# tbepler/topaz

Hardware: AMD Instinct MI355X
Metric: micrographs/sec (4096x4096 fp32) denoise+score, NMS parity (higher is better)
Workload: dtype f32 (convs: fp32 operands carried as two f16 halves on the f16 MFMA, three exact products per multiply-add accumulated in f32 -- fp32-level error, fp32-MFMA re-run on f16-range overflow; NMS in fp32; the exact-fp32-multiply rate is reported as exact_fp32)

## Files before the change

### topaz_amd/csrc/conv_split.h

```cpp
#pragma once
#include <hip/hip_runtime.h>
#include <stdint.h>
#include <vector>

#include "conv_mfma.h"
#include "split_fmt.h"

namespace tpz {

struct SplitArgs {
    const uint4* in;
    const uint4* in2;
    const uint4* wpk;
    const float* wscale;
    const float* bias;
    uint4* out;
    float* out_f32;
    const uint4* res;
    const float* post_scale;
    const float* post_shift;
    const float* head_w;
    float* head_out;
    const void* zeros;
    unsigned* flag;
    float head_b, slope;
    int cells_in, Hin, Win;
    int cells_in1, H1, W1;
    int Cout, cells_out, Hout, Wout;
    int pad_x, pad_y;
    int os, ooy, oox, Hfull, Wfull;
    int Hres, Wres, res_crop;
    int KZ, pad_z, Din, Dout, ooz, Dfull, Dres;
    int ncz;
    int nphase, phase_k, ws_phase_stride;
    size_t w_phase_bytes;
    int subpix_cout;
    int issuer_half;
    int n_chunks;
    int cog_inner;
    int tiles_x, tiles_y;
    int n_tiles;
    int vol_srcmajor;
    int xcd_swizzle;
    int wy0, wx0, wy1, wx1;
    int wz0, Dlat;
    int fold_cells, fold_tap, in2_H, in2_W, in2_oy, in2_ox;
    const struct SplitStep* plan;
};

struct SplitStep {
    uint16_t bofs[4];
    uint32_t dma;
    uint32_t cidx;
    uint32_t cell[4];
};
enum : uint32_t {
    SPLIT_DMA_ROUNDS = 0xffu,
    SPLIT_DMA_BUF = 1u << 8,
    SPLIT_DMA_NCELL_SHIFT = 9,
    SPLIT_DMA_SWITCH = 1u << 12,
    SPLIT_DMA_SRC2 = 1u << 13,
    SPLIT_DMA_NEXT = 1u << 14,
    SPLIT_DMA_ANY = 1u << 31,
};

struct SplitSlot {
    int ky, kx, c;
};

template <int K_, int D_, int MT_, int TH_, int TW_, int CC_, int WAVES_ = 8, int KX_ = K_, int SPS_ = 1>
struct SplitCfg {
    static constexpr int K = K_, KX = KX_, D = D_, MT = MT_, TH = TH_, TW = TW_, CC = CC_;
    static constexpr int WAVES = WAVES_, THREADS = 64 * WAVES_, WGS_PER_CU = WAVES_ == 8 ? 1 : 2;
    static constexpr bool UNIFORM_DMA = (MT_ >= 128 && WAVES_ == 8);
    static constexpr bool ISSUER_HALF = (MT_ >= 96 && WAVES_ == 8);
    static constexpr int MW = MT / 16;
    static constexpr int RPW = TH / WAVES;
    static constexpr int NFC = TW / 16;
    static constexpr int NW = RPW * NFC;
    static constexpr int ITH = TH + K - 1;
    static constexpr int ITW = (CC == 1) ? (TW + (KX - 1) * D + 15) / 16 * 16 : TW + (KX - 1) * D;
    static constexpr int CELL_STRIDE = (ITH * ITW + 15) / 16 * 16;
    static constexpr int NPC = CC * CELL_STRIDE;
    static constexpr int PLANE_BYTES = NPC * 16;
    static constexpr int IN_BUF = 2 * PLANE_BYTES;
    static constexpr int NR = (NPC + THREADS - 1) / THREADS;
    static constexpr bool ROWPAIR = (K == 5) && (KX == 5) && ((4 * D) % 16 == 0);
    static constexpr int PV = KX * (K / 2);
    static constexpr int PAIRS1 = PV + ((K % 2) ? (ROWPAIR ? KX - 1 : KX) : 0);
    static constexpr int NSTEP = (CC == 1) ? (PAIRS1 + 1) / 2 : (K * KX * CC + 3) / 4;
    static constexpr bool CONT = (CC % 2 == 0);
    static constexpr int Q = K * KX * CC;
    static constexpr int TAPS = K * KX;
    __host__ __device__ static constexpr int cont_slots(int cells) { return TAPS * cells; }
    __host__ __device__ static constexpr int cont_stages(int cells) { return (TAPS * cells + 3) / 4; }
    __host__ __device__ static constexpr SplitSlot cont_slot(int q) { return SplitSlot{(q / CC) / KX, (q / CC) % KX, q % CC}; }
    __host__ __device__ static constexpr SplitSlot slot(int step, int kb) {
        if (CC != 1) {
            const int q = step * 4 + kb, t = q / CC;
            return t < K * KX ? SplitSlot{t / KX, t % KX, q % CC} : SplitSlot{-1, 0, 0};
        }
        const int p = step * 2 + (kb >> 1), j = kb & 1;
        if (p < PV) return SplitSlot{2 * (p % (K / 2)) + j, p / (K / 2), 0};
        const int e = p - PV;
        if (K % 2 == 0) return SplitSlot{-1, 0, 0};
        if (ROWPAIR) {
            if (e == 0) return SplitSlot{K - 1, j ? 4 : 0, 0};
            return (e < KX - 1 && j == 0) ? SplitSlot{K - 1, e, 0} : SplitSlot{-1, 0, 0};
        }
        return (e < KX && j == 0) ? SplitSlot{K - 1, e, 0} : SplitSlot{-1, 0, 0};
    }
    __host__ __device__ static constexpr int slot_lds_off(int step, int kb) {
        SplitSlot s = slot(step, kb);
        if (s.ky < 0) s = slot(step, kb & ~1);
        if (s.ky < 0) return 0;
        return (s.c * CELL_STRIDE + s.ky * ITW + s.kx * D) * 16;
    }
    static constexpr int W_STEP_BYTES = 2 * MW * 1024;
    static constexpr int SPS = SPS_;
    static constexpr int W_STAGE_BYTES = SPS * W_STEP_BYTES;
    static constexpr int WR = (W_STAGE_BYTES + THREADS * 16 - 1) / (THREADS * 16);
    static constexpr int OFF_W = 2 * IN_BUF;
    static constexpr int OFF_TAB = OFF_W + 2 * W_STAGE_BYTES;
    static constexpr int LDS_BYTES = OFF_TAB + (NPC * 4 + 15) / 16 * 16;
    static_assert(NR <= 8, "the plan carries the DMA rounds of a step as a byte mask");
    static_assert(TH % WAVES == 0 && TW % 16 == 0 && MT % 16 == 0, "tile shape");
    static_assert(PLANE_BYTES + (RPW * ITW + TW) * 16 < 65536, "ds_read immediates are 16 bit");
    static_assert(LDS_BYTES <= 160 * 1024 / WGS_PER_CU, "LDS per workgroup");
    static_assert(WAVES == 8 || WAVES == 4, "waves per workgroup");
    static_assert(SPS == 1 || (CONT && Q >= 8 * SPS), "multi-step stages: continuous slot stream, chunks of >= 2 * SPS steps");
};

struct SplitPlanKey {
    int cells_in, cells_in1, n_chunks, has_in2, vol, KZ, fold_cells, fold_tap, srcmajor;
};

template <class C>
void split_make_plan(const SplitPlanKey& k, std::vector<SplitStep>& out) {
    const bool vol = k.vol != 0;
    const bool folded = C::CONT && C::SPS == 1 && k.fold_cells > 0;
    const int vcells = (folded ? k.cells_in1 : k.cells_in) * (vol ? k.KZ : 1);
    const int n_full = vcells / C::CC, n_rem = vcells - n_full * C::CC;
    const int n_stages_a = C::CONT ? C::cont_stages(vcells) : k.n_chunks * C::NSTEP;
    const int n_stages = n_stages_a + (folded ? k.fold_cells / C::CC : 0);
    const int chunks1 = (k.has_in2 && !vol) ? k.cells_in1 / C::CC : k.n_chunks;
    auto cont_off = [](int q) {
        const SplitSlot sl = C::cont_slot(q);
        return (sl.c * C::CELL_STRIDE + sl.ky * C::ITW + sl.kx * C::D) * 16;
    };
    auto fetch = [&](SplitStep& e, int pf, unsigned rmask, bool sw) {
        e.dma = SPLIT_DMA_ANY | (rmask & SPLIT_DMA_ROUNDS) | ((pf & 1) ? SPLIT_DMA_BUF : 0u) | (sw ? SPLIT_DMA_SWITCH : 0u);
        if (!vol) {
            const bool second = pf >= chunks1;
            if (second) e.dma |= SPLIT_DMA_SRC2;
            e.cidx = (uint32_t)(second ? pf - chunks1 : pf);
            const int have = k.cells_in - pf * C::CC;
            if (have < C::CC) e.dma |= (uint32_t)(have > 1 ? have : 1) << SPLIT_DMA_NCELL_SHIFT;
        } else {
            bool any2 = false, any1 = false;
            for (int j = 0; j < C::CC && j < 4; ++j) {
                const int v = pf * C::CC + j;
                int kz, c;
                if (!k.srcmajor) {
                    kz = v / k.cells_in; c = v - kz * k.cells_in;
                } else if (v < k.KZ * k.cells_in1) {
                    kz = v / k.cells_in1; c = v - kz * k.cells_in1;
                } else {
                    const int vv = v - k.KZ * k.cells_in1, c2n = k.cells_in - k.cells_in1;
                    kz = vv / c2n; c = k.cells_in1 + (vv - kz * c2n);
                }
                if (kz >= k.KZ) { e.cell[j] = 0; continue; }
                const bool l2 = c >= k.cells_in1;
                (l2 ? any2 : any1) = true;
                e.cell[j] = 1u | (l2 ? 2u : 0u) | (uint32_t)kz << 2 | (uint32_t)(l2 ? c - k.cells_in1 : c) << 8;
            }
            if (k.srcmajor && any2 && !any1) e.dma |= SPLIT_DMA_SRC2;
        }
    };
    out.assign((size_t)n_stages + 1, SplitStep{});
    fetch(out[0], 0, (1u << C::NR) - 1, false);
    unsigned next_rounds = 0;
    for (int s = 0; s < n_stages; ++s) {
        SplitStep& e = out[(size_t)s + 1];
        for (int l4 = 0; l4 < 4; ++l4) {
            int off;
            if (C::CONT) {
                if (folded && s >= n_stages_a) {
                    off = ((chunks1 + s - n_stages_a) & 1) * C::IN_BUF + cont_off(k.fold_tap * C::CC + l4);
                } else {
                    int G = 4 * s + l4, cg = G / C::Q, q = G - cg * C::Q;
                    if (cg >= n_full) {
                        const int q2 = G - n_full * C::Q;
                        cg = n_full < k.n_chunks ? n_full : k.n_chunks - 1;
                        q = (n_rem > 0 && q2 < C::TAPS * n_rem) ? (q2 / n_rem) * C::CC + (q2 % n_rem) : 0;
                    }
                    off = (cg & 1) * C::IN_BUF + cont_off(q);
                }
            } else {
                const int ch = s / C::NSTEP;
                off = (ch & 1) * C::IN_BUF + C::slot_lds_off(s - ch * C::NSTEP, l4);
            }
            e.bofs[l4] = (uint16_t)(off / 16);
        }
        const int stage = s / C::SPS;
        if (s % C::SPS != 0) continue;
        int pf, r0, rstride;
        if (C::CONT) {
            const int ch = (4 * s) / C::Q;
            pf = ch + 1;
            const int ws = pf >= 2 ? (C::Q * (pf - 1) - 1) / 4 + 1 : 0;
            const int we = (C::Q * pf) / 4 - 1;
            const int gs = (ws + C::SPS - 1) / C::SPS, ge = (we + 1) / C::SPS - 1;
            r0 = (stage >= gs && stage <= ge) ? stage - gs : C::NR;
            rstride = ge - gs + 1;
            if (folded && s >= n_stages_a) {
                pf = chunks1 + (s - n_stages_a) + 1;
                r0 = 0;
                rstride = 1;
            }
        } else {
            const int ch = s / C::NSTEP;
            pf = ch + 1;
            r0 = s - ch * C::NSTEP;
            rstride = C::NSTEP;
        }
        if (pf < k.n_chunks) {
            if (r0 >= C::NR) continue;
            unsigned rmask = 0;
            for (int r = r0; r < C::NR; r += rstride) rmask |= 1u << r;
            fetch(e, pf, rmask, r0 == 0 && pf == chunks1);
        } else if (pf == k.n_chunks && !folded && !vol && !k.has_in2) {
            if (C::CONT) {
                const int ws = pf >= 2 ? (C::Q * (pf - 1) - 1) / 4 + 1 : 0;
                const int we = n_stages - 1;
                const int gs = (ws + C::SPS - 1) / C::SPS, ge = (we + 1) / C::SPS - 1;
                if (stage < gs || stage > ge) continue;
                r0 = stage - gs;
                rstride = ge - gs + 1;
            }
            if (r0 >= C::NR) continue;
            unsigned rmask = 0;
            for (int r = r0; r < C::NR; r += rstride) rmask |= 1u << r;
            fetch(e, 0, rmask, r0 == 0);
            e.dma |= SPLIT_DMA_NEXT;
            if (k.n_chunks & 1) e.dma |= SPLIT_DMA_BUF;
            next_rounds |= rmask;
        }
    }
    if (next_rounds == (1u << C::NR) - 1u) out[0].dma |= SPLIT_DMA_NEXT;
    const size_t n = out.size();
    out.resize(2 * n);
    for (size_t i = 0; i < n; ++i) {
        SplitStep e = out[i];
        for (int l4 = 0; l4 < 4; ++l4) {
            const int off = e.bofs[l4] * 16;
            e.bofs[l4] = (uint16_t)((off >= C::IN_BUF ? off - C::IN_BUF : off + C::IN_BUF) / 16);
        }
        if (e.dma & SPLIT_DMA_ANY) e.dma ^= SPLIT_DMA_BUF;
        out[n + i] = e;
    }
}

enum { EPI_PLAIN_F32 = 5, EPI_POOL = 6 };
template <class C, int EPI, int ABL, int MODE>
__device__ __forceinline__ void conv_split_body(const SplitArgs& a, const unsigned bid_x, const unsigned bid_y, const unsigned bid_z,
                                                const unsigned grid_x, const unsigned grid_y) {
    constexpr int D = C::D, MW = C::MW, NW = C::NW, NFC = C::NFC;
    constexpr bool HAS2 = (MODE & 1) != 0, VOLM = (MODE & 2) != 0;
    constexpr bool UNI2 = (MODE & 8) != 0;
    static_assert(!UNI2 || (HAS2 && VOLM), "MODE 11 = two sources, plane-stacked, chunk-uniform");
    constexpr bool PERSIST = (MODE & 4) != 0;
    static_assert(!PERSIST || (MODE == 4 && EPI != EPI_HEAD), "persistent tiles: plain single-source layers");
    const uint4* const in2 = HAS2 ? a.in2 : nullptr;
    const int fold_cells = HAS2 ? a.fold_cells : 0;
    extern __shared__ __attribute__((aligned(16))) unsigned char lds[];
    unsigned* lds_tab = reinterpret_cast<unsigned*>(lds + C::OFF_TAB);

    const int tid = threadIdx.x;
    unsigned long long probe_c0 = 0, probe_r0 = 0, probe_pro = 0, probe_loop = 0;
    unsigned long long seg[4] = {0, 0, 0, 0}, seg_t = 0;
    auto seg_mark = [&](int i) {
        if constexpr ((ABL & 4096) != 0) {
            const unsigned long long t = __builtin_readcyclecounter();
            if (i >= 0) seg[i] += t - seg_t;
            seg_t = t;
        }
    };
    if constexpr ((ABL & 2048) != 0) {
        probe_c0 = __builtin_readcyclecounter();
        probe_r0 = __builtin_amdgcn_s_memrealtime();
    }
    const int lane = tid & 63;
    const int wave = __builtin_amdgcn_readfirstlane(tid >> 6);
    const int l15 = lane & 15, l4 = lane >> 4;

    int y0, x0, cogz, oz, pad_x, pad_y, pad_z, oox, ooy, ooz, phase, ybase, xbase;
    auto set_tile = [&](int bx, int by, int bz) {
        y0 = a.wy0 + (by / D) * (C::TH * D) + (by % D);
        x0 = a.wx0 + bx * C::TW;
        cogz = bz % a.ncz;
        oz = bz / a.ncz;
        pad_x = a.pad_x; pad_y = a.pad_y; pad_z = a.pad_z; oox = a.oox; ooy = a.ooy; ooz = a.ooz; phase = 0;
        if (a.nphase > 0) {
            phase = oz % a.nphase;
            oz /= a.nphase;
            oox = phase & 1; ooy = (phase >> 1) & 1; ooz = (phase >> 2) & 1;
            pad_x = (a.phase_k / 2 - oox + 1) / 2;
            pad_y = (a.phase_k / 2 - ooy + 1) / 2;
            pad_z = (a.phase_k / 2 - ooz + 1) / 2;
        }
        oz += a.wz0;
        ybase = y0 - pad_y; xbase = x0 - pad_x;
    };
    auto set_tile_linear = [&](unsigned L) {
        const unsigned txy = (unsigned)(a.tiles_x * a.tiles_y);
        const unsigned bz = L / txy, rem = L - bz * txy, by = rem / (unsigned)a.tiles_x;
        set_tile((int)(rem - by * (unsigned)a.tiles_x), (int)by, (int)bz);
    };
    unsigned tile_L = 0, tile_end = 0, tile_stride = 1;
    if constexpr (PERSIST) {
        const unsigned nt = (unsigned)a.n_tiles;
        const unsigned xcd = bid_x & 7u, j = bid_x >> 3, q = nt / 8, r = nt % 8;
        const unsigned start = xcd < r ? xcd * (q + 1) : r * (q + 1) + (xcd - r) * q;
        tile_end = start + q + (xcd < r ? 1u : 0u);
        tile_stride = grid_x >> 3;
        tile_L = start + j;
        if (tile_L >= tile_end) return;
        set_tile_linear(tile_L);
    } else {
        int bx = (int)bid_x, by = (int)bid_y;
        if (a.xcd_swizzle) {
            const unsigned nwg = grid_x * grid_y, orig = bid_x + grid_x * bid_y;
            const unsigned q = nwg / 8, r = nwg % 8, xcd = orig % 8;
            const unsigned wgid = (xcd < r ? xcd * (q + 1) : r * (q + 1) + (xcd - r) * q) + orig / 8;
            if (a.xcd_swizzle == 2) {
                const unsigned blk = wgid >> 5, in = wgid & 31u, nbx = grid_x >> 3;
                const unsigned byb = blk / nbx, tr = byb * 4 + (in >> 3), bands = (unsigned)a.tiles_y / (unsigned)D;
                bx = (int)((blk - byb * nbx) * 8 + (in & 7u));
                if (bx >= a.tiles_x || tr >= (unsigned)a.tiles_y) return;
                const unsigned ph = tr / bands;
                by = (int)((tr - ph * bands) * (unsigned)D + ph);
            } else {
                bx = (int)(wgid % grid_x);
                by = (int)(wgid / grid_x);
            }
        }
        set_tile(bx, by, (int)bid_z);
    }
    const bool vol = VOLM && (a.KZ > 1 || a.Din > 1);

    constexpr unsigned OOB = 0xfffffff0u;
    constexpr bool BUFDMA = (ABL & 65536) == 0;
    const bool ups = (a.H1 != a.Hin) || (a.W1 != a.Win);
    auto compute_offsets = [&](bool second, int tid, int H1, int W1, int Hup, int Wup, int ybase, int xbase) {
        const bool fold2 = second && fold_cells > 0;
        const int Hs = fold2 ? a.in2_H : second ? a.Hin : H1, Ws = fold2 ? a.in2_W : second ? a.Win : W1;
        const int Hv = fold2 ? a.in2_H : a.Hin, Wv = fold2 ? a.in2_W : a.Win;
#pragma unroll 1
        for (int i = 0; i < C::NR; ++i) {
            const int g = i * C::THREADS + tid;
            if (g < C::NPC) {
                const int c = g / C::CELL_STRIDE;
                const int rem = g - c * C::CELL_STRIDE;
                const int r = rem / C::ITW, x = rem - r * C::ITW;
                const int gy = ybase + r * D + (fold2 ? a.in2_oy : 0), gx = xbase + x + (fold2 ? a.in2_ox : 0);
                unsigned off = OOB;
                if ((unsigned)gy < (unsigned)Hv && (unsigned)gx < (unsigned)Wv) {
                    int sy = gy, sx = gx;
                    if (!second && ups) { sy = nearest_src(gy, H1, Hup); sx = nearest_src(gx, W1, Wup); }
                    off = vol ? (unsigned)(((size_t)sy * Ws + sx) * 16) : (unsigned)((((size_t)c * Hs + sy) * Ws + sx) * 16);
                }
                lds_tab[g] = off;
            }
        }
    };
    const size_t plane1 = (size_t)a.cells_in1 * a.H1 * a.W1 * (vol ? a.Din : 1);
    const size_t hw2 = fold_cells > 0 ? (size_t)a.in2_H * a.in2_W : (size_t)a.Hin * a.Win;
    const size_t plane2 = (size_t)(a.cells_in - a.cells_in1) * hw2 * (vol ? a.Din : 1);
    const unsigned lds_base = (unsigned)(size_t)(lptr_t)lds;
    const void* zsrc = uniform_ptr(a.zeros);
    typedef uint32_t StepW __attribute__((ext_vector_type(8)));
    typedef const __attribute__((address_space(4))) StepW* plan_ptr_t;
    const plan_ptr_t plan0 = (plan_ptr_t)a.plan;

    auto glds16 = [&](const void* src, unsigned lds_addr) {
        __builtin_amdgcn_global_load_lds((__attribute__((address_space(1))) const void*)src,
                                         (__attribute__((address_space(3))) void*)(size_t)lds_addr, 16, 0, 0);
    };
    auto make_srd = [&](const void* base, size_t bytes) {
        return __builtin_amdgcn_make_buffer_rsrc(const_cast<void*>(uniform_ptr(base)), 0,
                                                 (int)__builtin_amdgcn_readfirstlane((unsigned)bytes), 0x00020000);
    };
    auto bdma16 = [&](__amdgpu_buffer_rsrc_t srd, unsigned voff, unsigned soff, unsigned lds_addr) {
        __builtin_amdgcn_raw_ptr_buffer_load_lds(srd, (__attribute__((address_space(3))) void*)(size_t)lds_addr, 16, voff, soff, 0, 0);
    };
    auto fetch = [&](const StepW& P, unsigned rounds, int tid, int wave) {
        const unsigned d = P[2];
        const int buf = (d & SPLIT_DMA_BUF) ? 1 : 0;
        const bool second = HAS2 && (d & SPLIT_DMA_SRC2) != 0;
        const unsigned ncell = (d >> SPLIT_DMA_NCELL_SHIFT) & 7u;
        const uint4* chunk = second ? in2 + (size_t)P[3] * (C::CC * hw2) : a.in + (size_t)P[3] * (C::CC * (size_t)a.H1 * a.W1);
        const unsigned char* bhi = reinterpret_cast<const unsigned char*>(uniform_ptr(vol ? ((UNI2 && second) ? in2 : a.in) : chunk));
        const size_t lo_delta0 = ((second && (!vol || UNI2)) ? plane2 : plane1) * 16;
        const size_t ext = vol ? ((UNI2 && second) ? plane2 : plane1) * 16 : (second ? (size_t)C::CC * hw2 : (size_t)C::CC * a.H1 * a.W1) * 16;
        const __amdgpu_buffer_rsrc_t srd_hi = make_srd(bhi, ext), srd_lo = make_srd(bhi + lo_delta0, ext);
        constexpr int CCV = C::CC < 4 ? C::CC : 4;
        unsigned coff[CCV], cflag[CCV];
        if (vol) {
#pragma unroll
            for (int j = 0; j < CCV; ++j) {
                const unsigned cv = P[4 + j];
                const int iz = oz + (int)((cv >> 2) & 63u) * D - pad_z;
                const bool ok = (cv & 1u) && (unsigned)iz < (unsigned)a.Din;
                coff[j] = (unsigned)((((size_t)(cv >> 8) * a.Din + iz) * a.Hin) * a.Win * 16);
                cflag[j] = (ok ? 1u : 0u) | ((HAS2 && !UNI2) ? (cv & 2u) : 0u);
            }
        }
#pragma unroll
        for (int r = 0; r < C::NR; ++r) {
            if (!((rounds >> r) & 1u)) continue;
            const int g = r * C::THREADS + tid;
            if ((r + 1) * C::THREADS <= C::NPC || g < C::NPC) {
                unsigned off = lds_tab[g];
                size_t lo_delta = lo_delta0;
                bool lane2 = false;
                if (!vol) {
                    if (ncell != 0 && g >= (int)ncell * C::CELL_STRIDE) off = OOB;
                } else {
                    unsigned co = coff[0], cf = cflag[0];
#pragma unroll
                    for (int j = 1; j < CCV; ++j)
                        if (g >= j * C::CELL_STRIDE) { co = coff[j]; cf = cflag[j]; }
                    if (!(cf & 1u)) off = OOB;
                    else if (off != OOB) { off += co; lane2 = HAS2 && !UNI2 && (cf & 2u) != 0; }
                }
                const unsigned dst = __builtin_amdgcn_readfirstlane(lds_base + (unsigned)(buf * C::IN_BUF + (r * C::THREADS + wave * 64) * 16));
                if constexpr (BUFDMA) {
                    if (VOLM && HAS2 && !UNI2 && __any(lane2)) {
                        if (lane2) {
                            const __amdgpu_buffer_rsrc_t s2h = make_srd(in2, plane2 * 16), s2l = make_srd(in2 + plane2, plane2 * 16);
                            bdma16(s2h, off, 0, dst);
                            bdma16(s2l, off, 0, dst + C::PLANE_BYTES);
                        } else {
                            bdma16(srd_hi, off, 0, dst);
                            bdma16(srd_lo, off, 0, dst + C::PLANE_BYTES);
                        }
                    } else {
                        bdma16(srd_hi, off, 0, dst);
                        bdma16(srd_lo, off, 0, dst + C::PLANE_BYTES);
                    }
                } else if constexpr (C::UNIFORM_DMA) {
                    const void* blo = bhi + lo_delta;
                    if (!__any(off == OOB || lane2)) {
                        glds_b128(off, bhi, dst);
                        glds_b128(off, blo, dst + C::PLANE_BYTES);
                    } else {
                        if (off == OOB) {
                            glds_b128(0u, zsrc, dst);
                            glds_b128(0u, zsrc, dst + C::PLANE_BYTES);
                        } else if (lane2) {
                            const void* b2 = uniform_ptr(in2);
                            const void* b2lo = uniform_ptr(in2 + plane2);
                            glds_b128(off, b2, dst);
                            glds_b128(off, b2lo, dst + C::PLANE_BYTES);
                        } else {
                            glds_b128(off, bhi, dst);
                            glds_b128(off, blo, dst + C::PLANE_BYTES);
                        }
                    }
                } else {
                    const unsigned char* src = bhi;
                    if (lane2) { src = reinterpret_cast<const unsigned char*>(in2); lo_delta = plane2 * 16; }
                    const bool oob = off == OOB;
                    const unsigned char* shi = oob ? reinterpret_cast<const unsigned char*>(zsrc) : src + off;
                    const unsigned char* slo = oob ? reinterpret_cast<const unsigned char*>(zsrc) : src + off + lo_delta;
                    glds16(shi, dst);
                    glds16(slo, dst + C::PLANE_BYTES);
                }
            }
        }
    };
    auto issue_weights = [&](const unsigned char* wcog, int stg, int bytes, int buf, int tid, int wave) {
        const unsigned char* base = reinterpret_cast<const unsigned char*>(uniform_ptr(wcog + (size_t)stg * C::W_STAGE_BYTES));
        const unsigned dst = __builtin_amdgcn_readfirstlane(lds_base + (unsigned)(C::OFF_W + buf * C::W_STAGE_BYTES + wave * 1024));
        if constexpr (BUFDMA) {
            const __amdgpu_buffer_rsrc_t srd = make_srd(base, (size_t)bytes);
#pragma unroll
            for (int i = 0; i < C::WR; ++i)
                if ((i * C::WAVES + wave) * 1024 < bytes) bdma16(srd, (unsigned)tid * 16u, (unsigned)(i * C::THREADS * 16), dst + i * C::THREADS * 16);
            return;
        }
#pragma unroll
        for (int i = 0; i < C::WR; ++i)
            if ((i * C::WAVES + wave) * 1024 < bytes) {
                if constexpr (C::UNIFORM_DMA) glds_b128((unsigned)(i * C::THREADS + tid) * 16u, base, dst + i * C::THREADS * 16);
                else glds16(base + (unsigned)(i * C::THREADS + tid) * 16u, dst + i * C::THREADS * 16);
            }
    };

    const unsigned b_lane = (unsigned)(((wave * C::RPW) * C::ITW + l15) * 16);
    const unsigned a_lane = (unsigned)(C::OFF_W + lane * 16);
    auto b_frag_base = [&](const StepW& P, int l4) -> const unsigned char* {
        const unsigned w = (l4 & 2) ? P[1] : P[0];
        return lds + b_lane + (((w >> ((l4 & 1) * 16)) & 0xffffu) << 4);
    };

    float hsum[NW];
#pragma unroll
    for (int n = 0; n < NW; ++n) hsum[n] = 0.f;
    bool big = false;

    const bool folded = C::CONT && C::SPS == 1 && fold_cells > 0;
    const int vcells = (folded ? a.cells_in1 : a.cells_in) * (vol ? a.KZ : 1);
    const int n_stages_a = C::CONT ? C::cont_stages(vcells) : a.n_chunks * C::NSTEP;
    const int n_stages = n_stages_a + (folded ? fold_cells / C::CC : 0);
    const size_t w_cog_bytes = (size_t)n_stages * C::W_STEP_BYTES;

    const int n_wstages = (n_stages + C::SPS - 1) / C::SPS;
    int par_in = 0, par_w = 0;
    bool prefetched = false;
    auto wcog_of = [&](int phase, int cog) {
        return reinterpret_cast<const unsigned char*>(a.wpk) + (size_t)phase * a.w_phase_bytes + (size_t)cog * w_cog_bytes;
    };
    for (;;) {
    const bool has_next = PERSIST && tile_L + tile_stride < tile_end;
    int n_ybase = 0, n_xbase = 0, n_phase = 0, n_cog = 0;
    if (PERSIST && has_next) {
        const int sy0 = y0, sx0 = x0, scogz = cogz, soz = oz, spx = pad_x, spy = pad_y, spz = pad_z, sox = oox, soy = ooy,
                  soz2 = ooz, sph = phase, syb = ybase, sxb = xbase;
        set_tile_linear(tile_L + tile_stride);
        n_ybase = ybase; n_xbase = xbase; n_phase = phase; n_cog = cogz;
        y0 = sy0; x0 = sx0; cogz = scogz; oz = soz; pad_x = spx; pad_y = spy; pad_z = spz; oox = sox; ooy = soy; ooz = soz2;
        phase = sph; ybase = syb; xbase = sxb;
    }
    const plan_ptr_t plan = plan0 + (PERSIST && par_in ? n_stages + 1 : 0);
    for (int cg = 0; cg < a.cog_inner; ++cg) {
        const int cog = cogz * a.cog_inner + cg;
        const unsigned char* wcog = wcog_of(phase, cog);
        const float* wscale = a.wscale + (size_t)phase * a.ws_phase_stride;
        f32x4 acc[MW][NW];
#pragma unroll
        for (int m = 0; m < MW; ++m)
#pragma unroll
            for (int n = 0; n < NW; ++n) acc[m][n] = (f32x4){0.f, 0.f, 0.f, 0.f};

        unsigned long long probe_t0 = 0;
        if constexpr ((ABL & 2048) != 0) probe_t0 = (cg == 0 && !prefetched) ? probe_c0 : __builtin_readcyclecounter();
        __syncthreads();
        int tid_p = tid, H1_p = a.H1, W1_p = a.W1, Hup_p = a.Hin, Wup_p = a.Win;
        asm volatile("" : "+v"(tid_p), "+s"(H1_p), "+s"(W1_p), "+s"(Hup_p), "+s"(Wup_p));
        const int wave_p = __builtin_amdgcn_readfirstlane(tid_p >> 6), l4_p = (tid_p & 63) >> 4;
        StepW P = plan[1];
        if (!(PERSIST && prefetched)) {
            const StepW P0 = plan0[0];
            compute_offsets((P0[2] & SPLIT_DMA_SRC2) != 0, tid_p, H1_p, W1_p, Hup_p, Wup_p, ybase, xbase);
            fetch(P0, (1u << C::NR) - 1u, tid_p, wave_p);
            issue_weights(wcog, 0, (n_stages < C::SPS ? n_stages : C::SPS) * C::W_STEP_BYTES, 0, tid_p, wave_p);
            asm volatile("s_waitcnt vmcnt(0)" ::: "memory");
            __syncthreads();
        }

        f16x8 bh[NW], bo[NW], ah[2], ao[2];
        auto b_off = [&](int n) { return ((n / NFC) * C::ITW + (n % NFC) * 16) * 16; };
        {
            const unsigned char* bl = b_frag_base(P, l4_p);
#pragma unroll
            for (int n = 0; n < NW; ++n) {
                bh[n] = *reinterpret_cast<const f16x8*>(bl + b_off(n));
                bo[n] = *reinterpret_cast<const f16x8*>(bl + b_off(n) + C::PLANE_BYTES);
            }
            const unsigned a_lane_p = (unsigned)(C::OFF_W + (tid_p & 63) * 16 + (PERSIST ? par_w * C::W_STAGE_BYTES : 0));
            ah[0] = *reinterpret_cast<const f16x8*>(lds + a_lane_p);
            ao[0] = *reinterpret_cast<const f16x8*>(lds + a_lane_p + MW * 1024);
        }

        unsigned long long probe_t1 = 0;
        if constexpr ((ABL & 2048) != 0) probe_t1 = __builtin_readcyclecounter();
        if constexpr ((ABL & 524288) != 0) { if (C::WAVES == 8 && wave >= 4) __builtin_amdgcn_s_setprio(1); }
        if constexpr ((ABL & 1048576) != 0) { if (C::WAVES == 8 && wave < 4) __builtin_amdgcn_s_setprio(1); }
#pragma unroll 1
        for (int s = 0; s < n_stages; ++s) {
            const int stage = s / C::SPS, sub = s - stage * C::SPS;
            const bool stage_end = sub == C::SPS - 1 || s == n_stages - 1;
            const StepW Pn = plan[1 + (s + 1 < n_stages ? s + 1 : s)];
            auto step_dma = [&]() {
            if (!(ABL & 2) && sub == 0) {
                const bool iss = C::ISSUER_HALF && a.issuer_half && (!in2 || folded);
                const int reps = iss ? (wave >= 4 ? 2 : 0) : 1;
                if constexpr (!(ABL & 128)) {
                    for (int rep = 0; rep < reps; ++rep) {
                        const int vw = iss ? wave - 4 * (1 - rep) : wave, vt = iss ? tid - 256 * (1 - rep) : tid;
                        const int left = n_stages - (stage + 1) * C::SPS;
                        const int wb = PERSIST ? (stage + 1 + par_w) & 1 : (stage + 1) & 1;
                        if (left > 0) issue_weights(wcog, stage + 1, (left < C::SPS ? left : C::SPS) * C::W_STEP_BYTES, wb, vt, vw);
                        else if (PERSIST && has_next)
                            issue_weights(wcog_of(n_phase, n_cog), 0, (n_stages < C::SPS ? n_stages : C::SPS) * C::W_STEP_BYTES, wb, vt, vw);
                    }
                }
                const bool next_fetch = (P[2] & SPLIT_DMA_NEXT) != 0;
                if (!(ABL & 256) && (P[2] & SPLIT_DMA_ANY) && (!next_fetch || (PERSIST && has_next))) {
                    if (HAS2 && (P[2] & SPLIT_DMA_SWITCH)) {
                        compute_offsets(true, tid, a.H1, a.W1, a.Hin, a.Win, ybase, xbase);
                        if (iss) __syncthreads();
                    }
                    if (PERSIST && next_fetch && (P[2] & SPLIT_DMA_SWITCH)) {
                        compute_offsets(false, tid, a.H1, a.W1, a.Hin, a.Win, n_ybase, n_xbase);
                        if (iss) __syncthreads();
                    }
                    for (int rep = 0; rep < reps; ++rep) {
                        const int vw = iss ? wave - 4 * (1 - rep) : wave, vt = iss ? tid - 256 * (1 - rep) : tid;
                        fetch(P, P[2] & SPLIT_DMA_ROUNDS, vt, vw);
                    }
                }
            }
            };
            seg_mark(s == 0 ? -1 : 3);
            step_dma();
            seg_mark(0);
            constexpr bool MFMA_FIRST = (ABL & 131072) == 0;
            const int wpar = PERSIST ? par_w : 0;
            const unsigned char* al = lds + a_lane + ((stage + wpar) & 1) * C::W_STAGE_BYTES + sub * C::W_STEP_BYTES;
            const int stage_n = (s + 1) / C::SPS;
            const unsigned char* al_next = lds + a_lane + ((stage_n + wpar) & 1) * C::W_STAGE_BYTES + (s + 1 - stage_n * C::SPS) * C::W_STEP_BYTES;
            const unsigned char* bl_next = nullptr;
            constexpr bool A0_EARLY = (MW % 2 == 0);
#pragma unroll
            for (int m = 0; m < MW; ++m) {
                const int t = m & 1;
                if (m + 1 < MW) {
                    if constexpr (!(ABL & 8)) {
                        ah[t ^ 1] = *reinterpret_cast<const f16x8*>(al + (m + 1) * 1024);
                        ao[t ^ 1] = *reinterpret_cast<const f16x8*>(al + (MW + m + 1) * 1024);
                    } else {
                        ah[t ^ 1] = ah[t];
                        ao[t ^ 1] = ao[t];
                    }
                } else {
                    if constexpr (!(ABL & 16) && !(ABL & 8)) {
#pragma unroll
                        for (int mm = 0; mm + 1 < MW; ++mm) {
                            if (mm == 0 && MFMA_FIRST) {
                                __builtin_amdgcn_sched_group_barrier(0x008, NW, 0);
                                __builtin_amdgcn_sched_group_barrier(0x100, 2, 0);
                                __builtin_amdgcn_sched_group_barrier(0x008, 2 * NW, 0);
                            } else {
                                __builtin_amdgcn_sched_group_barrier(0x100, 2, 0);
                                __builtin_amdgcn_sched_group_barrier(0x008, 3 * NW, 0);
                            }
                        }
                    }
                    __builtin_amdgcn_sched_barrier(0);
                    seg_mark(1);
                    if (C::SPS == 1 || stage_end) {
                        if constexpr (!(ABL & 16384))
                            asm volatile("s_waitcnt vmcnt(0)" ::: "memory");
                        if constexpr (!(ABL & 4)) __syncthreads();
                    }
                    seg_mark(2);
                    bl_next = b_frag_base(Pn, l4);
                    __builtin_amdgcn_sched_barrier(0);
                }
                const bool last = m + 1 == MW;
                f16x8 a_hi = ah[t], a_lo = ao[t];
                if (last && A0_EARLY) {
                    ah[0] = *reinterpret_cast<const f16x8*>(al_next);
                    ao[0] = *reinterpret_cast<const f16x8*>(al_next + MW * 1024);
                }
                if constexpr (!(ABL & 16)) {
#pragma unroll
                    for (int n = 0; n < NW; ++n)
                        acc[m][n] = __builtin_amdgcn_mfma_f32_16x16x32_f16(a_hi, bo[n], acc[m][n], 0, 0, 0);
                    if (last) {
#pragma unroll
                        for (int n = 0; n < NW; ++n) bo[n] = *reinterpret_cast<const f16x8*>(bl_next + b_off(n) + C::PLANE_BYTES);
                    }
#pragma unroll
                    for (int n = 0; n < NW; ++n)
                        acc[m][n] = __builtin_amdgcn_mfma_f32_16x16x32_f16(a_hi, bh[n], acc[m][n], 0, 0, 0);
#pragma unroll
                    for (int n = 0; n < NW; ++n)
                        acc[m][n] = __builtin_amdgcn_mfma_f32_16x16x32_f16(a_lo, bh[n], acc[m][n], 0, 0, 0);
                } else {
#pragma unroll
                    for (int n = 0; n < NW; ++n) acc[m][n][0] += (float)a_hi[0] * (float)bh[n][0] + (float)a_lo[1] * (float)bo[n][1];
                    if (last) {
#pragma unroll
                        for (int n = 0; n < NW; ++n) bo[n] = *reinterpret_cast<const f16x8*>(bl_next + b_off(n) + C::PLANE_BYTES);
                    }
                }
                if (last) {
#pragma unroll
                    for (int n = 0; n < NW; ++n) bh[n] = *reinterpret_cast<const f16x8*>(bl_next + b_off(n));
                    if (!A0_EARLY) {
                        ah[0] = *reinterpret_cast<const f16x8*>(al_next);
                        ao[0] = *reinterpret_cast<const f16x8*>(al_next + MW * 1024);
                    }
                    if constexpr (!(ABL & 16) && !(ABL & 8)) {
                        if (A0_EARLY) __builtin_amdgcn_sched_group_barrier(0x100, 2, 1);
                        __builtin_amdgcn_sched_group_barrier(0x008, NW, 1);
                        __builtin_amdgcn_sched_group_barrier(0x100, NW, 1);
                        __builtin_amdgcn_sched_group_barrier(0x008, 2 * NW, 1);
                        __builtin_amdgcn_sched_group_barrier(0x100, A0_EARLY ? NW : NW + 2, 1);
                    }
                    __builtin_amdgcn_sched_barrier(0);
                }
            }
            P = Pn;
        }
        if constexpr ((ABL & 2048) != 0) {
            probe_loop += __builtin_readcyclecounter() - probe_t1;
            probe_pro += probe_t1 - probe_t0;
        }

        if constexpr ((ABL & (524288 | 1048576)) != 0) __builtin_amdgcn_s_setprio(0);
        int tid_e = threadIdx.x;
        asm volatile("" : "+v"(tid_e));
        const int l15 = tid_e & 15, l4 = (tid_e >> 4) & 3;
        const int wave = __builtin_amdgcn_readfirstlane(tid_e >> 6);
        const int fz = oz * a.os + ooz;
        const size_t cplane_out = (size_t)a.Dfull * a.Hfull * a.Wfull, cplane_res = (size_t)a.Dres * a.Hres * a.Wres;
        const size_t plane_out = (size_t)a.cells_out * cplane_out;
        const size_t plane_res = (size_t)a.cells_out * cplane_res;
        const size_t zoff_out = (size_t)fz * a.Hfull * a.Wfull;
        const size_t zoff_res = (size_t)(fz + (a.Dres > 1 ? a.res_crop : 0)) * a.Hres * a.Wres;
        const bool has_bias = a.bias != nullptr;
        unsigned opix[NW], rpix[NW], ovo[NW], rvo[NW];
        bool okv[NW];
        if constexpr (EPI != EPI_HEAD) {
#pragma unroll
            for (int n = 0; n < NW; ++n) {
                const int oy = y0 + (wave * C::RPW + n / NFC) * D;
                const int ox = x0 + (n % NFC) * 16 + l15;
                okv[n] = oy < a.wy1 && ox < a.wx1;
                if constexpr ((ABL & 1) != 0 || (ABL & 64) != 0) okv[n] = okv[n] && (a.slope == 12345.f);
                const int cy = oy < a.Hout ? oy : a.Hout - 1, cx = ox < a.Wout ? ox : a.Wout - 1;
                const int fy = cy * a.os + ooy, fx = cx * a.os + oox;
                if constexpr (EPI == EPI_POOL) opix[n] = (unsigned)((cy >> 1) * a.Wfull + (cx >> 1));
                else opix[n] = (unsigned)(fy * a.Wfull + fx);
                rpix[n] = (unsigned)((fy + a.res_crop) * a.Wres + fx + a.res_crop);
                if constexpr (EPI == EPI_POOL) {
                    okv[n] = (l15 & 1) == 0 && oy < a.wy1 && ox < a.wx1 && oy + 1 < a.Hout && ox + 1 < a.Wout;
                }
                const unsigned lane_o = (unsigned)(l4 >> 1) * (unsigned)(cplane_out * 16) + (unsigned)(l4 & 1) * 8u;
                const unsigned lane_r = (unsigned)(l4 >> 1) * (unsigned)(cplane_res * 16) + (unsigned)(l4 & 1) * 8u;
                ovo[n] = okv[n] ? opix[n] * 16u + lane_o : OOB;
                rvo[n] = rpix[n] * 16u + lane_r;
            }
        }
        const unsigned cp16_o = (unsigned)(cplane_out * 16), cp16_r = (unsigned)(cplane_res * 16);
        constexpr bool WIDE = (NW % 2 == 0) && EPI != EPI_HEAD && EPI != EPI_PLAIN_F32 && EPI != EPI_POOL && (ABL & 262144) == 0;
        constexpr int NP = WIDE ? NW / 2 : 1;
        unsigned ovw[NP], rvw[NP];
        if constexpr (WIDE) {
            const int odd = l4 & 1;
#pragma unroll
            for (int q = 0; q < NP; ++q) {
                const int fr = odd ? (2 * q + 1) / NFC : (2 * q) / NFC, fc = odd ? (2 * q + 1) % NFC : (2 * q) % NFC;
                const int oy = y0 + (wave * C::RPW + fr) * D;
                const int ox = x0 + fc * 16 + l15;
                bool ok = oy < a.wy1 && ox < a.wx1;
                if constexpr ((ABL & 1) != 0 || (ABL & 64) != 0) ok = ok && (a.slope == 12345.f);
                const int cy = oy < a.Hout ? oy : a.Hout - 1, cx = ox < a.Wout ? ox : a.Wout - 1;
                const int fy = cy * a.os + ooy, fx = cx * a.os + oox;
                const unsigned po = (unsigned)(fy * a.Wfull + fx), pr = (unsigned)((fy + a.res_crop) * a.Wres + fx + a.res_crop);
                ovw[q] = ok ? po * 16u + (unsigned)(l4 >> 1) * (unsigned)(cplane_out * 16) : OOB;
                rvw[q] = pr * 16u + (unsigned)(l4 >> 1) * (unsigned)(cplane_res * 16);
            }
        }
        const unsigned zo16 = (unsigned)(zoff_out * 16), zr16 = (unsigned)(zoff_res * 16);
        const size_t pl16_o = plane_out * 16, pl16_r = plane_res * 16;
        const unsigned char* const out8 = reinterpret_cast<const unsigned char*>(a.out);
        const unsigned char* const res8 = reinterpret_cast<const unsigned char*>(a.res);
        const float slope = a.slope;
        u16x2 bigacc = {0, 0};
        unsigned okmask[NW];
#pragma unroll
        for (int n = 0; n < NW; ++n) okmask[n] = (EPI != EPI_HEAD && okv[n]) ? 0x7fff7fffu : 0u;
        struct Frag { int cb, sy, sx, cell0, ncell; bool ok; };
        auto frag_of = [&](int m) {
            Frag f;
            const int covb = cog * C::MT + m * 16;
            f.cb = covb; f.sy = 0; f.sx = 0; f.ok = true;
            if (a.subpix_cout > 0) {
                const int par = covb / a.subpix_cout;
                f.cb = covb - par * a.subpix_cout;
                f.sx = par & 1; f.sy = (par >> 1) & 1;
                f.ok = par <= 3;
            }
            f.cell0 = f.cb >> 3;
            const int nc = f.ok ? a.cells_out - f.cell0 : 0;
            f.ncell = nc < 0 ? 0 : nc > 2 ? 2 : nc;
            return f;
        };
        constexpr bool RESID = (EPI == EPI_RES || EPI == EPI_RES_POST) && !(ABL & 1) && !(ABL & 32);
        u32x2 rhb[2][NW], rlb[2][NW];
        auto load_res = [&](int m, u32x2 (&rh)[NW], u32x2 (&rl)[NW]) {
            const Frag f = frag_of(m);
            const unsigned ex16 = zr16 + (unsigned)(f.sy * a.Wres + f.sx) * 16u;
            const unsigned nrec = f.ncell > 0 ? (unsigned)f.ncell * cp16_r - ex16 : 0u;
            const unsigned char* rb8 = res8 + ((size_t)((unsigned)f.cell0 * (unsigned long long)cp16_r) + ex16);
            const __amdgpu_buffer_rsrc_t srd_rh = make_srd(rb8, nrec);
            const __amdgpu_buffer_rsrc_t srd_rl = make_srd(rb8 + pl16_r, nrec);
            if constexpr (WIDE) {
#pragma unroll
                for (int q = 0; q < NP; ++q) {
                    const u32x4 ch = __builtin_amdgcn_raw_buffer_load_b128(srd_rh, (int)rvw[q], 0, 0);
                    const u32x4 cl = __builtin_amdgcn_raw_buffer_load_b128(srd_rl, (int)rvw[q], 0, 0);
                    rh[2 * q] = (u32x2){ch[0], ch[1]}; rh[2 * q + 1] = (u32x2){ch[2], ch[3]};
                    rl[2 * q] = (u32x2){cl[0], cl[1]}; rl[2 * q + 1] = (u32x2){cl[2], cl[3]};
                }
            } else {
#pragma unroll
                for (int n = 0; n < NW; ++n) {
                    rh[n] = __builtin_amdgcn_raw_buffer_load_b64(srd_rh, (int)rvo[n], 0, 0);
                    rl[n] = __builtin_amdgcn_raw_buffer_load_b64(srd_rl, (int)rvo[n], 0, 0);
                }
            }
        };
        auto unswap_res = [&](u32x2 (&r)[NW], int q) {
            const auto s0 = __builtin_amdgcn_permlane16_swap(r[2 * q].x, r[2 * q + 1].x, false, false);
            const auto s1 = __builtin_amdgcn_permlane16_swap(r[2 * q].y, r[2 * q + 1].y, false, false);
            r[2 * q] = (u32x2){s0[0], s1[0]};
            r[2 * q + 1] = (u32x2){s0[1], s1[1]};
        };
        if constexpr (RESID) load_res(0, rhb[0], rlb[0]);
#pragma unroll
        for (int m = 0; m < MW; ++m) {
            const Frag f = frag_of(m);
            const int cov0 = cog * C::MT + m * 16 + l4 * 4;
            const int sy = f.sy, sx = f.sx, cell0 = f.cell0, ncell = f.ncell;
            const int co0 = f.ok ? f.cb + l4 * 4 : a.Cout;
            if constexpr (RESID) { if (m + 1 < MW) load_res(m + 1, rhb[(m + 1) & 1], rlb[(m + 1) & 1]); }
            u32x2 (&rh)[NW] = rhb[m & 1];
            u32x2 (&rl)[NW] = rlb[m & 1];
            f32x2 sc[2], bi[2], psc[2], psh[2], hw[2];
            {
                const float4 s4 = *reinterpret_cast<const float4*>(wscale + cov0);
                sc[0] = (f32x2){s4.x, s4.y}; sc[1] = (f32x2){s4.z, s4.w};
                float4 b4 = make_float4(0.f, 0.f, 0.f, 0.f);
                if (has_bias) b4 = *reinterpret_cast<const float4*>(a.bias + co0);
                bi[0] = (f32x2){b4.x, b4.y}; bi[1] = (f32x2){b4.z, b4.w};
                if constexpr (EPI == EPI_RES_POST) {
                    const float4 p4 = *reinterpret_cast<const float4*>(a.post_scale + co0);
                    const float4 q4 = *reinterpret_cast<const float4*>(a.post_shift + co0);
                    psc[0] = (f32x2){p4.x, p4.y}; psc[1] = (f32x2){p4.z, p4.w};
                    psh[0] = (f32x2){q4.x, q4.y}; psh[1] = (f32x2){q4.z, q4.w};
                }
                if constexpr (EPI == EPI_HEAD) {
                    const float4 h4 = *reinterpret_cast<const float4*>(a.head_w + co0);
                    hw[0] = (f32x2){h4.x, h4.y}; hw[1] = (f32x2){h4.z, h4.w};
                }
            }
            const f32x2 slope2 = {slope, slope};
            __amdgpu_buffer_rsrc_t srd_oh, srd_ol;
            if constexpr (EPI != EPI_HEAD && EPI != EPI_PLAIN_F32) {
                const unsigned ex16 = zo16 + (unsigned)(sy * a.Wfull + sx) * 16u;
                const unsigned nrec = ncell > 0 ? (unsigned)ncell * cp16_o - ex16 : 0u;
                const unsigned char* ob8 = out8 + ((size_t)((unsigned)cell0 * (unsigned long long)cp16_o) + ex16);
                srd_oh = make_srd(ob8, nrec);
                srd_ol = make_srd(ob8 + pl16_o, nrec);
            }
            if constexpr (EPI == EPI_POOL) {
                static_assert(EPI != EPI_POOL || (C::RPW % 2 == 0 && C::D == 1), "pooling pairs tile rows inside a wave");
#pragma unroll
                for (int n = 0; n < NW; ++n) {
                    if ((n / NFC) % 2 != 0) continue;
                    f32x2 v[2];
#pragma unroll
                    for (int h = 0; h < 2; ++h) {
                        f32x2 t0 = (f32x2){acc[m][n][2 * h], acc[m][n][2 * h + 1]} * sc[h] + bi[h];
                        f32x2 t1 = (f32x2){acc[m][n + NFC][2 * h], acc[m][n + NFC][2 * h + 1]} * sc[h] + bi[h];
                        t0 = __builtin_elementwise_max(t0, t0 * slope2);
                        t1 = __builtin_elementwise_max(t1, t1 * slope2);
                        const f32x2 t = __builtin_elementwise_max(t0, t1);
                        v[h] = __builtin_elementwise_max(t, (f32x2){__shfl_xor(t[0], 1, 64), __shfl_xor(t[1], 1, 64)});
                    }
                    unsigned h0, l0, h1, l1;
                    split2m(v[0], h0, l0);
                    split2m(v[1], h1, l1);
                    const u32x2 hi = {h0, h1}, lo = {l0, l1};
                    bigacc = __builtin_elementwise_max(bigacc, __builtin_bit_cast(u16x2, h0 & okmask[n]));
                    bigacc = __builtin_elementwise_max(bigacc, __builtin_bit_cast(u16x2, h1 & okmask[n]));
                    __builtin_amdgcn_raw_buffer_store_b64(hi, srd_oh, (int)ovo[n], 0, 0);
                    __builtin_amdgcn_raw_buffer_store_b64(lo, srd_ol, (int)ovo[n], 0, 0);
                }
                continue;
            }
            unsigned keep_h[2] = {0u, 0u}, keep_l[2] = {0u, 0u};
#pragma unroll
            for (int n = 0; n < NW; ++n) {
                if constexpr (WIDE && RESID) {
                    if ((n & 1) == 0) { unswap_res(rh, n >> 1); unswap_res(rl, n >> 1); }
                }
                f32x2 v[2];
#pragma unroll
                for (int h = 0; h < 2; ++h) {
                    f32x2 addend = bi[h];
                    if constexpr (RESID)
                        addend = add_halves(add_halves(addend, h ? rl[n].y : rl[n].x), h ? rh[n].y : rh[n].x);
                    v[h] = (f32x2){acc[m][n][2 * h], acc[m][n][2 * h + 1]} * sc[h] + addend;
                    if constexpr (EPI == EPI_RES_POST) v[h] = v[h] * psc[h] + psh[h];
                    v[h] = __builtin_elementwise_max(v[h], v[h] * slope2);
                    if constexpr (EPI == EPI_HEAD) v[h] *= hw[h];
                }
                if constexpr (EPI == EPI_HEAD) {
                    const f32x2 t = v[0] + v[1];
                    hsum[n] += t[0] + t[1];
                } else if constexpr (EPI == EPI_PLAIN_F32) {
                    const size_t cs = cplane_out;
                    float* const fb = a.out_f32 + ((size_t)co0 * cplane_out + zoff_out + (unsigned)(sy * a.Wfull + sx)) + opix[n];
#pragma unroll
                    for (int r = 0; r < 4; ++r)
                        if (okv[n] && co0 + r < a.Cout) fb[r * cs] = v[r >> 1][r & 1];
                } else {
                    unsigned h0, l0, h1, l1;
                    split2m(v[0], h0, l0);
                    split2m(v[1], h1, l1);
                    const u32x2 hi = {h0, h1}, lo = {l0, l1};
                    bigacc = __builtin_elementwise_max(bigacc, __builtin_bit_cast(u16x2, h0 & okmask[n]));
                    bigacc = __builtin_elementwise_max(bigacc, __builtin_bit_cast(u16x2, h1 & okmask[n]));
                    if constexpr (WIDE) {
                        if ((n & 1) == 0) {
                            keep_h[0] = h0; keep_h[1] = h1; keep_l[0] = l0; keep_l[1] = l1;
                        } else {
                            const auto sh0 = __builtin_amdgcn_permlane16_swap(keep_h[0], h0, false, false);
                            const auto sh1 = __builtin_amdgcn_permlane16_swap(keep_h[1], h1, false, false);
                            const auto sl0 = __builtin_amdgcn_permlane16_swap(keep_l[0], l0, false, false);
                            const auto sl1 = __builtin_amdgcn_permlane16_swap(keep_l[1], l1, false, false);
                            const u32x4 chi = {sh0[0], sh1[0], sh0[1], sh1[1]}, clo = {sl0[0], sl1[0], sl0[1], sl1[1]};
                            __builtin_amdgcn_raw_buffer_store_b128(chi, srd_oh, (int)ovw[n >> 1], 0, 0);
                            __builtin_amdgcn_raw_buffer_store_b128(clo, srd_ol, (int)ovw[n >> 1], 0, 0);
                        }
                    } else {
                        __builtin_amdgcn_raw_buffer_store_b64(hi, srd_oh, (int)ovo[n], 0, 0);
                        __builtin_amdgcn_raw_buffer_store_b64(lo, srd_ol, (int)ovo[n], 0, 0);
                    }
                }
            }
        }
        big = big || bigacc[0] >= 0x7c00 || bigacc[1] >= 0x7c00;
    }
    if (!(PERSIST && has_next)) break;
    tile_L += tile_stride;
    set_tile_linear(tile_L);
    par_in ^= a.n_chunks & 1;
    par_w ^= n_wstages & 1;
    prefetched = true;
    }

    if constexpr ((ABL & 2048) != 0) {
        if (threadIdx.x == 0) {
            unsigned long long* ctr = reinterpret_cast<unsigned long long*>(a.flag) + 1;
            atomicAdd(ctr, __builtin_readcyclecounter() - probe_c0);
            atomicAdd(ctr + 1, __builtin_amdgcn_s_memrealtime() - probe_r0);
            atomicAdd(ctr + 2, probe_pro);
            atomicAdd(ctr + 3, probe_loop);
        }
        if constexpr ((ABL & 4096) != 0) {
            if ((threadIdx.x & 63) == 0 && (wave == 0 || wave == C::WAVES / 2)) {
                unsigned long long* ctr = reinterpret_cast<unsigned long long*>(a.flag) + 5 + (wave == 0 ? 0 : 4);
                for (int i = 0; i < 4; ++i) atomicAdd(ctr + i, seg[i]);
            }
        }
    }
    if constexpr (EPI == EPI_HEAD) {
        int tid_e = threadIdx.x;
        asm volatile("" : "+v"(tid_e));
        const int l15 = tid_e & 15, l4 = (tid_e >> 4) & 3;
        const int wave = __builtin_amdgcn_readfirstlane(tid_e >> 6);
#pragma unroll
        for (int n = 0; n < NW; ++n) {
            const int trow = wave * C::RPW + n / NFC;
            const int oy = y0 + trow * D;
            const int ox = x0 + (n % NFC) * 16 + l15;
            float h = hsum[n];
            h += __shfl_xor(h, 16, 64);
            h += __shfl_xor(h, 32, 64);
            if (l4 == 0 && oy < a.wy1 && ox < a.wx1) a.head_out[((size_t)oz * a.Hout + oy) * a.Wout + ox] = h + a.head_b;
        }
    } else if constexpr (EPI != EPI_PLAIN_F32) {
        if (__any(big) && lane == 0) atomicOr(a.flag, 1u);
    }
}

template <class C, int EPI, int ABL = 0, int MODE = 3>
__global__ __launch_bounds__(C::THREADS, C::WGS_PER_CU) void conv_split_kernel(const SplitArgs a) {
    conv_split_body<C, EPI, ABL, MODE>(a, blockIdx.x, blockIdx.y, blockIdx.z, gridDim.x, gridDim.y);
}

enum { SPLIT_MULTI_MAX = 8 };
struct SplitMulti {
    unsigned n, first[SPLIT_MULTI_MAX + 1];
    unsigned pad_[6];
    SplitArgs a[SPLIT_MULTI_MAX];
};
static_assert(sizeof(SplitMulti) <= 4096, "kernel-argument segment");

template <class C, int EPI, int MODE>
__global__ __launch_bounds__(C::THREADS, C::WGS_PER_CU) void conv_split_multi_kernel(const SplitMulti) {
    typedef const __attribute__((address_space(4))) SplitMulti* multi_ptr_t;
    const multi_ptr_t m = (multi_ptr_t)__builtin_amdgcn_kernarg_segment_ptr();
    const unsigned b = blockIdx.x;
    unsigned j = 0;
#pragma unroll
    for (unsigned i = 1; i < SPLIT_MULTI_MAX; ++i) j += b >= m->first[i] ? 1u : 0u;
    const unsigned l = b - m->first[j];
    const SplitArgs& a = *(const SplitArgs*)&m->a[j];
    const unsigned gx = (unsigned)a.tiles_x, gy = (unsigned)a.tiles_y, gxy = gx * gy;
    const unsigned bz = l / gxy, rem = l - bz * gxy, by = rem / gx;
    if (l >= (unsigned)a.n_tiles) return;
    conv_split_body<C, EPI, 0, MODE>(a, rem - by * gx, by, bz, gx, gy);
}

}
```

### topaz_amd/csrc/conv_split_registry.h

```cpp
#pragma once
#include <hip/hip_runtime.h>
#include "conv_split.h"
#include "conv_registry.h"

namespace tpz {

struct SplitKernelInfo {
    int K, D, MT, epi;
    int KX, TH, TW, CC, WAVES, NSTEP, W_STEP_BYTES, lds_bytes, SPS;
    int cont, Q;
    SplitSlot (*slot)(int step, int kb);
    SplitSlot (*cont_slot)(int q);
    int stages(int cells) const { return cont ? ((Q / CC) * cells + 3) / 4 : (cells + CC - 1) / CC * NSTEP; }
    hipError_t (*launch)(const SplitArgs&, dim3 grid, hipStream_t);
    hipError_t (*launch_multi)(const SplitArgs* const* list, int n, hipStream_t);
    void (*make_plan)(const SplitPlanKey&, std::vector<SplitStep>&);
    char name[160];
};

void register_split(const SplitKernelInfo& info);
const SplitKernelInfo* find_split(int K, int D, int MT, int epi, int KX = 0, int sps = 0);

template <class C, int EPI>
hipError_t launch_split_cfg(const SplitArgs& a, dim3 grid, hipStream_t s) {
    static bool attr_set = false;
    if (!attr_set) {
        hipError_t e = hipFuncSetAttribute(reinterpret_cast<const void*>(&conv_split_kernel<C, EPI, 0, 0>),
                                           hipFuncAttributeMaxDynamicSharedMemorySize, C::LDS_BYTES);
        if (e == hipSuccess)
            e = hipFuncSetAttribute(reinterpret_cast<const void*>(&conv_split_kernel<C, EPI, 0, 1>),
                                    hipFuncAttributeMaxDynamicSharedMemorySize, C::LDS_BYTES);
        if (e == hipSuccess)
            e = hipFuncSetAttribute(reinterpret_cast<const void*>(&conv_split_kernel<C, EPI, 0, 2>),
                                    hipFuncAttributeMaxDynamicSharedMemorySize, C::LDS_BYTES);
        if (e == hipSuccess)
            e = hipFuncSetAttribute(reinterpret_cast<const void*>(&conv_split_kernel<C, EPI, 0, 11>),
                                    hipFuncAttributeMaxDynamicSharedMemorySize, C::LDS_BYTES);
        if (e == hipSuccess)
            e = hipFuncSetAttribute(reinterpret_cast<const void*>(&conv_split_kernel<C, EPI, 0, 3>),
                                    hipFuncAttributeMaxDynamicSharedMemorySize, C::LDS_BYTES);
        if constexpr (EPI != EPI_HEAD)
            if (e == hipSuccess)
                e = hipFuncSetAttribute(reinterpret_cast<const void*>(&conv_split_kernel<C, EPI, 0, 4>),
                                        hipFuncAttributeMaxDynamicSharedMemorySize, C::LDS_BYTES);
        if (e != hipSuccess) return e;
        attr_set = true;
    }
    const bool plain = !a.in2 && a.KZ <= 1 && a.Din <= 1;
    if (a.n_tiles > 0) {
        if constexpr (EPI != EPI_HEAD) {
            if (!plain) return hipErrorInvalidValue;
            hipLaunchKernelGGL((conv_split_kernel<C, EPI, 0, 4>), grid, dim3(C::THREADS), C::LDS_BYTES, s, a);
        } else {
            return hipErrorInvalidValue;
        }
    } else if (plain) {
        hipLaunchKernelGGL((conv_split_kernel<C, EPI, 0, 0>), grid, dim3(C::THREADS), C::LDS_BYTES, s, a);
    } else if (a.KZ <= 1 && a.Din <= 1) {
        hipLaunchKernelGGL((conv_split_kernel<C, EPI, 0, 1>), grid, dim3(C::THREADS), C::LDS_BYTES, s, a);
    } else if (!a.in2) {
        hipLaunchKernelGGL((conv_split_kernel<C, EPI, 0, 2>), grid, dim3(C::THREADS), C::LDS_BYTES, s, a);
    } else if (a.vol_srcmajor) {
        hipLaunchKernelGGL((conv_split_kernel<C, EPI, 0, 11>), grid, dim3(C::THREADS), C::LDS_BYTES, s, a);
    } else {
        hipLaunchKernelGGL((conv_split_kernel<C, EPI, 0, 3>), grid, dim3(C::THREADS), C::LDS_BYTES, s, a);
    }
    return hipGetLastError();
}

inline int split_mode_of(const SplitArgs& a) {
    if (!a.in2 && a.KZ <= 1 && a.Din <= 1) return 0;
    if (a.KZ <= 1 && a.Din <= 1) return 1;
    if (!a.in2) return 2;
    return a.vol_srcmajor ? 11 : 3;
}

template <class C, int EPI>
hipError_t launch_split_multi_cfg(const SplitArgs* const* list, int n, hipStream_t s) {
    static bool attr_set = false;
    if (!attr_set) {
        hipError_t e = hipFuncSetAttribute(reinterpret_cast<const void*>(&conv_split_multi_kernel<C, EPI, 0>),
                                           hipFuncAttributeMaxDynamicSharedMemorySize, C::LDS_BYTES);
        if (e == hipSuccess)
            e = hipFuncSetAttribute(reinterpret_cast<const void*>(&conv_split_multi_kernel<C, EPI, 1>),
                                    hipFuncAttributeMaxDynamicSharedMemorySize, C::LDS_BYTES);
        if (e == hipSuccess)
            e = hipFuncSetAttribute(reinterpret_cast<const void*>(&conv_split_multi_kernel<C, EPI, 2>),
                                    hipFuncAttributeMaxDynamicSharedMemorySize, C::LDS_BYTES);
        if (e == hipSuccess)
            e = hipFuncSetAttribute(reinterpret_cast<const void*>(&conv_split_multi_kernel<C, EPI, 11>),
                                    hipFuncAttributeMaxDynamicSharedMemorySize, C::LDS_BYTES);
        if (e != hipSuccess) return e;
        attr_set = true;
    }
    if (n < 1 || n > SPLIT_MULTI_MAX) return hipErrorInvalidValue;
    SplitMulti m;
    m.n = (unsigned)n;
    unsigned total = 0;
    const int mode = split_mode_of(*list[0]);
    for (int i = 0; i < n; ++i) {
        if (split_mode_of(*list[i]) != mode || list[i]->n_tiles < 1) return hipErrorInvalidValue;
        m.first[i] = total;
        m.a[i] = *list[i];
        total = (total + (unsigned)list[i]->n_tiles + 7u) & ~7u;
    }
    for (int i = n; i <= SPLIT_MULTI_MAX; ++i) m.first[i] = total;
    const dim3 grid(total, 1, 1);
    if (mode == 0) hipLaunchKernelGGL((conv_split_multi_kernel<C, EPI, 0>), grid, dim3(C::THREADS), C::LDS_BYTES, s, m);
    else if (mode == 1) hipLaunchKernelGGL((conv_split_multi_kernel<C, EPI, 1>), grid, dim3(C::THREADS), C::LDS_BYTES, s, m);
    else if (mode == 2) hipLaunchKernelGGL((conv_split_multi_kernel<C, EPI, 2>), grid, dim3(C::THREADS), C::LDS_BYTES, s, m);
    else if (mode == 11) hipLaunchKernelGGL((conv_split_multi_kernel<C, EPI, 11>), grid, dim3(C::THREADS), C::LDS_BYTES, s, m);
    else return hipErrorInvalidValue;
    return hipGetLastError();
}

template <class C>
SplitSlot split_slot_of(int step, int kb) { return C::slot(step, kb); }
template <class C>
SplitSlot split_cont_slot_of(int q) { return C::cont_slot(q); }

template <class C, int EPI>
struct SplitRegistrar {
    SplitRegistrar() {
        SplitKernelInfo i;
        i.K = C::K; i.KX = C::KX; i.D = C::D; i.MT = C::MT; i.epi = EPI;
        i.TH = C::TH; i.TW = C::TW; i.CC = C::CC; i.WAVES = C::WAVES; i.NSTEP = C::NSTEP; i.W_STEP_BYTES = C::W_STEP_BYTES;
        i.lds_bytes = C::LDS_BYTES;
        i.SPS = C::SPS;
        i.slot = &split_slot_of<C>;
        i.cont = C::CONT ? 1 : 0; i.Q = C::Q;
        i.cont_slot = &split_cont_slot_of<C>;
        i.launch = &launch_split_cfg<C, EPI>;
        i.launch_multi = nullptr;
        if constexpr (C::WAVES == 4 && EPI != EPI_HEAD) i.launch_multi = &launch_split_multi_cfg<C, EPI>;
        i.make_plan = &split_make_plan<C>;
        if (C::SPS == 1)
            snprintf(i.name, sizeof i.name, "conv_split_kernel<K=%dx%d,D=%d,MT=%d,TH=%d,TW=%d,CC=%d,W=%d,EPI=%d>", i.K, i.KX,
                     i.D, i.MT, i.TH, i.TW, i.CC, i.WAVES, i.epi);
        else
            snprintf(i.name, sizeof i.name, "conv_split_kernel<K=%dx%d,D=%d,MT=%d,TH=%d,TW=%d,CC=%d,W=%d,S=%d,EPI=%d>", i.K,
                     i.KX, i.D, i.MT, i.TH, i.TW, i.CC, i.WAVES, i.SPS, i.epi);
        register_split(i);
    }
};

#define TPZ_SPLIT(K, D, MT, TH, TW, CC, EPI) \
    static ::tpz::SplitRegistrar<::tpz::SplitCfg<K, D, MT, TH, TW, CC>, EPI> TPZ_CAT(tpz_sreg_, __COUNTER__);
#define TPZ_SPLIT_S(K, D, MT, TH, TW, CC, S, EPI) \
    static ::tpz::SplitRegistrar<::tpz::SplitCfg<K, D, MT, TH, TW, CC, 8, K, S>, EPI> TPZ_CAT(tpz_sreg_, __COUNTER__);
#define TPZ_SPLIT4_S(K, D, MT, TH, TW, CC, S, EPI) \
    static ::tpz::SplitRegistrar<::tpz::SplitCfg<K, D, MT, TH, TW, CC, 4, K, S>, EPI> TPZ_CAT(tpz_sreg_, __COUNTER__);
#define TPZ_SPLIT4_COL(K, D, MT, TH, TW, CC, EPI) \
    static ::tpz::SplitRegistrar<::tpz::SplitCfg<K, D, MT, TH, TW, CC, 4, 1>, EPI> TPZ_CAT(tpz_sreg_, __COUNTER__);
#define TPZ_SPLIT4(K, D, MT, TH, TW, CC, EPI) \
    static ::tpz::SplitRegistrar<::tpz::SplitCfg<K, D, MT, TH, TW, CC, 4>, EPI> TPZ_CAT(tpz_sreg_, __COUNTER__);
#define TPZ_SPLIT_RESID_S(K, D, MT, TH, TW, CC, S)        \
    TPZ_SPLIT_S(K, D, MT, TH, TW, CC, S, ::tpz::EPI_PLAIN) \
    TPZ_SPLIT_S(K, D, MT, TH, TW, CC, S, ::tpz::EPI_RES)   \
    TPZ_SPLIT_S(K, D, MT, TH, TW, CC, S, ::tpz::EPI_RES_POST)
#define TPZ_SPLIT4_RESID(K, D, MT, TH, TW, CC)        \
    TPZ_SPLIT4(K, D, MT, TH, TW, CC, ::tpz::EPI_PLAIN) \
    TPZ_SPLIT4(K, D, MT, TH, TW, CC, ::tpz::EPI_RES)   \
    TPZ_SPLIT4(K, D, MT, TH, TW, CC, ::tpz::EPI_RES_POST)
#define TPZ_SPLIT4_RESID_S(K, D, MT, TH, TW, CC, S)        \
    TPZ_SPLIT4_S(K, D, MT, TH, TW, CC, S, ::tpz::EPI_PLAIN) \
    TPZ_SPLIT4_S(K, D, MT, TH, TW, CC, S, ::tpz::EPI_RES)   \
    TPZ_SPLIT4_S(K, D, MT, TH, TW, CC, S, ::tpz::EPI_RES_POST)
#define TPZ_SPLIT_RESID(K, D, MT, TH, TW, CC)        \
    TPZ_SPLIT(K, D, MT, TH, TW, CC, ::tpz::EPI_PLAIN) \
    TPZ_SPLIT(K, D, MT, TH, TW, CC, ::tpz::EPI_RES)   \
    TPZ_SPLIT(K, D, MT, TH, TW, CC, ::tpz::EPI_RES_POST)

}
```

### topaz_amd/csrc/rt_core.hip

```cpp
#include "rt_internal.h"

namespace tpz {
namespace {
std::vector<ConvKernelInfo>& registry() {
    static std::vector<ConvKernelInfo> r;
    return r;
}
std::vector<SplitKernelInfo>& split_registry() {
    static std::vector<SplitKernelInfo> r;
    return r;
}
}
void register_conv(const ConvKernelInfo& info) { registry().push_back(info); }
const ConvKernelInfo* find_conv(int dims, int K, int D, int MT, bool cin1, int epi) {
    for (const auto& k : registry())
        if (k.dims == dims && k.K == K && k.D == D && k.MT == MT && k.cin1 == (cin1 ? 1 : 0) && k.epi == epi) return &k;
    return nullptr;
}
void register_split(const SplitKernelInfo& info) { split_registry().push_back(info); }
const SplitKernelInfo* find_split(int K, int D, int MT, int epi, int KX, int sps) {
    if (KX <= 0) KX = K;
    const SplitKernelInfo* best = nullptr;
    for (const auto& k : split_registry())
        if (k.K == K && k.KX == KX && k.D == D && k.MT == MT && k.epi == epi && (sps <= 0 || k.SPS == sps) &&
            (!best || k.SPS > best->SPS)) best = &k;
    return best;
}
}

namespace tpz::rt {
namespace {
std::string g_last_error;
}
const std::string& last_global_error() { return g_last_error; }
void restore_errors(tpz_ctx* ctx, const std::string& ctx_err, const std::string& global_err) {
    if (ctx) ctx->err = ctx_err;
    g_last_error = global_err;
}

DebugEnv debug_env() {
    DebugEnv d;
    const char* on = getenv("TPZ_DEBUG");
    if (!on || !*on || !strcmp(on, "0")) return d;
    d.on = true;
    auto flag = [](const char* name) { const char* e = getenv(name); return e != nullptr && *e && strcmp(e, "0") != 0; };
    d.no_phase = flag("TPZ_NO_PHASE");
    d.exact_fp32 = flag("TPZ_EXACT_FP32");
    d.no_issuer = flag("TPZ_NO_ISSUER");
    d.no_lanes = flag("TPZ_NO_LANES");
    d.no_roi = flag("TPZ_NO_ROI");
    d.no_persist = flag("TPZ_NO_PERSIST");
    d.trace_host = flag("TPZ_TRACE_HOST");
    d.no_range = flag("TPZ_NO_RANGE");
    d.no_raster = flag("TPZ_NO_RASTER");
    d.no_srcmajor = flag("TPZ_NO_SRCMAJOR");
    d.no_valu_last = flag("TPZ_NO_VALU_LAST");
    d.no_rw = flag("TPZ_NO_RW");
    d.no_pool3d = flag("TPZ_NO_POOL3D");
    d.no_fold = flag("TPZ_NO_FOLD");
    d.no_widen = flag("TPZ_NO_WIDEN");
    if (flag("TPZ_NO_BATCH")) d.batch = 0;
    else if (const char* e = getenv("TPZ_BATCH")) {
        const int n = atoi(e);
        d.batch = n < 0 ? 0 : n > (int)tpz::SPLIT_MULTI_MAX ? (int)tpz::SPLIT_MULTI_MAX : n;
    }
    if (const char* e = getenv("TPZ_LANES")) d.lanes = atoi(e);
    return d;
}

int fail(tpz_ctx* ctx, const char* fmt, ...) {
    char buf[1024];
    va_list ap;
    va_start(ap, fmt);
    vsnprintf(buf, sizeof buf, fmt, ap);
    va_end(ap);
    g_last_error = buf;
    if (ctx) ctx->err = buf;
    return 1;
}

void* pool_alloc(tpz_ctx* ctx, size_t bytes) {
    if (bytes == 0) bytes = 16;
    std::vector<tpz_ctx::Buf>& pool = *ctx->pool_cur;
    int best = -1;
    for (int i = 0; i < (int)pool.size(); ++i) {
        auto& b = pool[i];
        if (!b.used && b.bytes >= bytes && (best < 0 || b.bytes < pool[best].bytes)) best = i;
    }
    if (best >= 0) {
        pool[best].used = true;
        return pool[best].p;
    }
    void* p = nullptr;
    size_t rounded = (bytes + (1u << 20) - 1) & ~((size_t)(1u << 20) - 1);
    if (hipMalloc(&p, rounded) != hipSuccess) {
        auto trim = [](std::vector<tpz_ctx::Buf>& pl) {
            for (auto it = pl.begin(); it != pl.end();) {
                if (!it->used) { (void)hipFree(it->p); it = pl.erase(it); }
                else ++it;
            }
        };
        auto recording = [&](const std::vector<tpz_ctx::Buf>* pl) {
            if (!ctx->rec_on) return false;
            for (const auto& rp : ctx->rec_pools[ctx->rec_lane])
                if (&rp == pl) return true;
            return false;
        };
        (void)hipGetLastError();
        if (!recording(&pool)) trim(pool);
        if (recording(&pool) || hipMalloc(&p, rounded) != hipSuccess) {
            (void)hipGetLastError();
            (void)hipDeviceSynchronize();
            trim(ctx->pool);
            for (auto& ln : ctx->lanes) trim(ln.pool);
            for (auto& lane_pools : ctx->rec_pools)
                for (auto& pl : lane_pools)
                    if (!recording(&pl)) trim(pl);
            if (hipMalloc(&p, rounded) != hipSuccess) { (void)hipGetLastError(); return nullptr; }
        }
    }
    pool.push_back({p, rounded, true});
    return p;
}
void pool_release(tpz_ctx* ctx, void* p) {
    for (auto& b : *ctx->pool_cur)
        if (b.p == p) { b.used = false; return; }
}

hipError_t flag_clear(tpz_ctx* ctx) { return hipMemsetAsync(ctx->d_flag, 0, sizeof(unsigned), ctx->stream); }
hipError_t flag_read(tpz_ctx* ctx, unsigned* flag, bool check_copy) {
    const hipError_t copied = hipMemcpyAsync(ctx->h_flag, ctx->d_flag, sizeof(unsigned), hipMemcpyDeviceToHost, ctx->stream);
    const hipError_t drained = hipStreamSynchronize(ctx->stream);
    *flag = *ctx->h_flag;
    return check_copy && copied != hipSuccess ? copied : drained;
}

float* next_nrm(tpz_ctx* ctx) {
    if (ctx->nrm_next >= NRM_RING) {
        if (ctx->lanes_on) (void)hipDeviceSynchronize();
        else (void)hipStreamSynchronize(ctx->stream);
        ctx->nrm_next = 0;
    }
    return ctx->d_nrm + 4 * (ctx->nrm_next++);
}

int lanes_begin(tpz_ctx* ctx) {
    if (!ctx->lanes_enabled || ctx->lanes_on) return 0;
    if (!ctx->lanes_fork) {
        if (hipEventCreateWithFlags(&ctx->lanes_fork, hipEventDisableTiming) != hipSuccess) return fail(ctx, "hipEventCreate failed");
        for (auto& ln : ctx->lanes) {
            if (hipStreamCreateWithFlags(&ln.stream, hipStreamNonBlocking) != hipSuccess ||
                hipEventCreateWithFlags(&ln.done, hipEventDisableTiming) != hipSuccess ||
                hipMalloc((void**)&ln.d_part, 2 * PART_BLOCKS * sizeof(double)) != hipSuccess)
                return fail(ctx, "patch lanes: stream / event / scratch creation failed");
        }
    }
    HIPCHK(ctx, hipEventRecord(ctx->lanes_fork, ctx->stream));
    for (auto& ln : ctx->lanes) HIPCHK(ctx, hipStreamWaitEvent(ln.stream, ctx->lanes_fork, 0));
    ctx->lanes_saved_stream = ctx->stream;
    ctx->lanes_saved_part = ctx->d_part;
    ctx->lanes_on = true;
    ctx->lanes_live = ctx->n_lanes;
    return 0;
}
void lane_enter(tpz_ctx* ctx, int k) {
    if (!ctx->lanes_on) return;
    tpz_ctx::Lane& ln = ctx->lanes[k % ctx->lanes_live];
    ctx->stream = ln.stream;
    ctx->pool_cur = &ln.pool;
    ctx->d_part = ln.d_part;
}
int lanes_end(tpz_ctx* ctx) {
    if (!ctx->lanes_on) return 0;
    ctx->stream = ctx->lanes_saved_stream;
    ctx->pool_cur = &ctx->pool;
    ctx->d_part = ctx->lanes_saved_part;
    ctx->lanes_on = false;
    for (auto& ln : ctx->lanes) {
        HIPCHK(ctx, hipEventRecord(ln.done, ln.stream));
        HIPCHK(ctx, hipStreamWaitEvent(ctx->stream, ln.done, 0));
    }
    return 0;
}

void prof_begin(tpz_ctx* ctx, int cls, double flops, const void* key, double bytes) {
    ctx->prof_open = false;
    if (!ctx->prof) return;
    if (ctx->prof == 2 && (cls != 0 || flops < 2e10)) return;
    ctx->prof_open = true;
    ProfRec r;
    r.cls = cls;
    r.flops = flops;
    r.bytes = bytes;
    r.key = key;
    auto get = [&]() {
        hipEvent_t e;
        if (!ctx->free_events.empty()) { e = ctx->free_events.back(); ctx->free_events.pop_back(); }
        else (void)hipEventCreate(&e);
        return e;
    };
    r.e0 = get();
    r.e1 = get();
    (void)hipEventRecord(r.e0, ctx->stream);
    ctx->recs.push_back(r);
}
void prof_end(tpz_ctx* ctx) {
    if (!ctx->prof_open || ctx->recs.empty()) return;
    ctx->prof_open = false;
    (void)hipEventRecord(ctx->recs.back().e1, ctx->stream);
}
void prof_flush(tpz_ctx* ctx) {
    if (ctx->recs.empty()) return;
    (void)hipStreamSynchronize(ctx->stream);
    for (auto& r : ctx->recs) {
        float ms = 0.f;
        (void)hipEventElapsedTime(&ms, r.e0, r.e1);
        ctx->acc_ms[r.cls] += ms;
        ctx->acc_n[r.cls] += 1;
        ctx->acc_flops[r.cls] += r.flops;
        if (r.key) {
            ProfAcc* a = nullptr;
            for (auto& kv : ctx->per_kernel)
                if (kv.first == r.key) a = &kv.second;
            if (!a) { ctx->per_kernel.push_back({r.key, ProfAcc()}); a = &ctx->per_kernel.back().second; }
            a->ms += ms; a->flops += r.flops; a->bytes += r.bytes; a->n += 1;
        }
        ctx->free_events.push_back(r.e0);
        ctx->free_events.push_back(r.e1);
    }
    ctx->recs.clear();
}

int rec_begin(tpz_ctx* ctx, int batch_no) {
    if (ctx->dbg.trace_host) ctx->rec_t0 = host_now_ms();
    for (auto& r : ctx->rec) r.clear();
    lane_enter(ctx, batch_no);
    ctx->rec_lane = ctx->lanes_on ? batch_no % ctx->lanes_live : 0;
    ctx->rec_on = true;
    ctx->rec_cur = 0;
    ctx->pool_cur = &ctx->rec_pools[ctx->rec_lane][0];
    return 0;
}
void rec_select(tpz_ctx* ctx, int i) {
    ctx->rec_cur = i;
    ctx->pool_cur = &ctx->rec_pools[ctx->rec_lane][i];
}
void rec_abort(tpz_ctx* ctx) {
    ctx->rec_on = false;
    ctx->pool_cur = &ctx->pool;
    for (auto& r : ctx->rec) r.clear();
}
int rec_flush(tpz_ctx* ctx) {
    ctx->rec_on = false;
    ctx->pool_cur = &ctx->pool;
    const double t_flush0 = ctx->dbg.trace_host ? host_now_ms() : 0.0;
    long long n_issued = 0;
    const int n = (int)tpz::SPLIT_MULTI_MAX;
    size_t cur[tpz::SPLIT_MULTI_MAX] = {};
    int rc = 0;
    for (;;) {
        bool any = false;
        for (int i = 0; i < n && !rc; ++i) {
            auto& L = ctx->rec[i];
            while (cur[i] < L.size() && !L[cur[i]].ks && !rc) {
                RecOp& op = L[cur[i]++];
                prof_begin(ctx, op.cls, op.flops, op.key, op.bytes);
                const hipError_t e = op.fn(ctx->stream);
                prof_end(ctx);
                ++ctx->n_launches;
                ++n_issued;
                if (e != hipSuccess) rc = fail(ctx, "launch failed: %s", hipGetErrorString(e));
            }
            if (cur[i] < L.size()) any = true;
        }
        if (rc || !any) break;
        int lead = -1;
        for (int i = 0; i < n; ++i)
            if (cur[i] < ctx->rec[i].size()) { lead = i; break; }
        const RecOp& o0 = ctx->rec[lead][cur[lead]];
        const SplitArgs* list[tpz::SPLIT_MULTI_MAX];
        int who[tpz::SPLIT_MULTI_MAX], m = 0;
        double flops = 0, bytes = 0;
        for (int i = lead; i < n; ++i) {
            if (cur[i] >= ctx->rec[i].size()) continue;
            const RecOp& o = ctx->rec[i][cur[i]];
            if (o.ks != o0.ks || o.a.plan != o0.a.plan || split_mode_of(o.a) != split_mode_of(o0.a)) continue;
            if (i != lead && (!o0.ks->launch_multi || split_mode_of(o0.a) == 3)) continue;
            list[m] = &o.a; who[m++] = i;
            flops += o.flops; bytes += o.bytes;
        }
        prof_begin(ctx, 0, flops, o0.ks->name, bytes);
        hipError_t e;
        if (m == 1) {
            SplitArgs a1 = o0.a;
            a1.n_tiles = 0;
            e = o0.ks->launch(a1, o0.grid, ctx->stream);
        } else {
            e = o0.ks->launch_multi(list, m, ctx->stream);
        }
        prof_end(ctx);
        ++ctx->n_launches;
        ++n_issued;
        if (e != hipSuccess) rc = fail(ctx, "conv_split launch failed: %s", hipGetErrorString(e));
        for (int k = 0; k < m; ++k) ++cur[who[k]];
    }
    if (ctx->dbg.trace_host) {
        size_t n_ops = 0;
        int n_img = 0;
        for (auto& r : ctx->rec) { n_ops += r.size(); n_img += r.empty() ? 0 : 1; }
        fprintf(stderr, "[tpz host] batch of %d images: %zu launches recorded in %.3f ms, issued as %lld in %.3f ms\n", n_img, n_ops,
                t_flush0 - ctx->rec_t0, n_issued, host_now_ms() - t_flush0);
    }
    for (auto& r : ctx->rec) r.clear();
    return rc;
}

}

using namespace tpz;
using namespace tpz::rt;

int tpz_debug_switches(char* buf, int buf_len) {
    const DebugEnv d = debug_env();
    std::string s;
    int n = 0;
    auto add = [&](bool on, const char* name) { if (on) { if (!s.empty()) s += ' '; s += name; ++n; } };
    add(d.no_phase, "no_phase"); add(d.exact_fp32, "exact_fp32"); add(d.no_issuer, "no_issuer"); add(d.no_lanes, "no_lanes");
    add(d.no_roi, "no_roi"); add(d.no_persist, "no_persist"); add(d.trace_host, "trace_host"); add(d.no_range, "no_range");
    add(d.no_raster, "no_raster"); add(d.no_srcmajor, "no_srcmajor"); add(d.no_valu_last, "no_valu_last"); add(d.no_rw, "no_rw");
    add(d.no_pool3d, "no_pool3d"); add(d.no_fold, "no_fold"); add(d.no_widen, "no_widen"); add(d.batch >= 0, "batch");
    add(d.lanes != 0, "lanes");
    if (buf && buf_len > 0) snprintf(buf, (size_t)buf_len, "%s", s.c_str());
    return n;
}

const char* tpz_version(void) { return "topaz_hip 0.1 (gfx950)"; }

const char* tpz_last_error(tpz_ctx* ctx) { return ctx ? ctx->err.c_str() : g_last_error.c_str(); }

int tpz_ctx_create(int device_id, tpz_ctx** out) {
    if (!out) return fail(nullptr, "tpz_ctx_create: out is NULL");
    *out = nullptr;
    int ndev = 0;
    if (hipGetDeviceCount(&ndev) != hipSuccess || ndev == 0)
        return fail(nullptr, "tpz_ctx_create: no HIP device visible (this library has no CPU fallback)");
    if (device_id < 0 || device_id >= ndev) return fail(nullptr, "tpz_ctx_create: device %d of %d", device_id, ndev);
    tpz_ctx* ctx = new tpz_ctx();
    ctx->device = device_id;
    if (hipSetDevice(device_id) != hipSuccess) { delete ctx; return fail(nullptr, "hipSetDevice(%d) failed", device_id); }
    hipDeviceProp_t prop;
    if (hipGetDeviceProperties(&prop, device_id) == hipSuccess) {
        if (strncmp(prop.gcnArchName, "gfx950", 6) != 0) {
            delete ctx;
            return fail(nullptr, "device %d is %s; this library is built for gfx950 (MI355X) only", device_id,
                        prop.gcnArchName);
        }
        if (prop.multiProcessorCount > 0) ctx->n_cus = prop.multiProcessorCount;
    }
    ctx->dbg = debug_env();
    ctx->lanes_enabled = !ctx->dbg.no_lanes;
    ctx->roi_enabled = !ctx->dbg.no_roi;
    ctx->persist_mode = ctx->dbg.no_persist ? 0 : 1;
    ctx->range_scaling = !ctx->dbg.no_range;
    ctx->raster = !ctx->dbg.no_raster;
    ctx->exact = ctx->dbg.exact_fp32;
    if (ctx->dbg.batch >= 0) ctx->batch = ctx->dbg.batch;
    if (ctx->dbg.lanes >= 2 && ctx->dbg.lanes <= N_LANES) ctx->n_lanes = ctx->dbg.lanes;
    if (hipStreamCreate(&ctx->own_stream) != hipSuccess) { delete ctx; return fail(nullptr, "hipStreamCreate failed"); }
    ctx->stream = ctx->own_stream;
    if (hipMalloc((void**)&ctx->d_part, 2 * PART_BLOCKS * sizeof(double)) != hipSuccess ||
        hipMalloc((void**)&ctx->d_nrm, 4 * NRM_RING * sizeof(float)) != hipSuccess ||
        hipMalloc((void**)&ctx->d_counters, NMS_COUNTERS * sizeof(unsigned int)) != hipSuccess ||
        hipMalloc((void**)&ctx->d_flag, 16) != hipSuccess || hipHostMalloc((void**)&ctx->h_flag, 16) != hipSuccess ||
        hipMalloc((void**)&ctx->d_absmax, 1024) != hipSuccess || hipMemset(ctx->d_absmax, 0, 1024) != hipSuccess ||
        hipMalloc((void**)&ctx->d_zeros, 256) != hipSuccess || hipMemset(ctx->d_zeros, 0, 256) != hipSuccess) {
        delete ctx;
        return fail(nullptr, "tpz_ctx_create: hipMalloc failed");
    }
    *out = ctx;
    return 0;
}

void tpz_ctx_destroy(tpz_ctx* ctx) {
    if (!ctx) return;
    (void)hipSetDevice(ctx->device);
    (void)hipStreamSynchronize(ctx->stream);
    (void)hipDeviceSynchronize();
    if (ctx->io_stage) tpz_stage_free(ctx->io_stage);
    for (auto& b : ctx->pool) (void)hipFree(b.p);
    for (auto& lane_pools : ctx->rec_pools)
        for (auto& rp : lane_pools)
            for (auto& b : rp) (void)hipFree(b.p);
    for (auto& ln : ctx->lanes) {
        for (auto& b : ln.pool) (void)hipFree(b.p);
        if (ln.d_part) (void)hipFree(ln.d_part);
        if (ln.done) (void)hipEventDestroy(ln.done);
        if (ln.stream) (void)hipStreamDestroy(ln.stream);
    }
    if (ctx->lanes_fork) (void)hipEventDestroy(ctx->lanes_fork);
    (void)hipFree(ctx->d_part);
    (void)hipFree(ctx->d_nrm);
    (void)hipFree(ctx->d_counters);
    (void)hipFree(ctx->d_zeros);
    (void)hipFree(ctx->d_flag);
    (void)hipFree(ctx->d_absmax);
    (void)hipHostFree(ctx->h_flag);
    for (auto& e : ctx->split_plans) (void)hipFree(e.d);
    for (auto e : ctx->free_events) (void)hipEventDestroy(e);
    if (ctx->own_stream) (void)hipStreamDestroy(ctx->own_stream);
    delete ctx;
}

int tpz_ctx_set_stream(tpz_ctx* ctx, void* hip_stream) {
    if (!ctx) return fail(nullptr, "ctx is NULL");
    (void)hipStreamSynchronize(ctx->stream);
    ctx->stream = hip_stream ? (hipStream_t)hip_stream : ctx->own_stream;
    return 0;
}

int tpz_ctx_sync(tpz_ctx* ctx) {
    if (!ctx) return fail(nullptr, "ctx is NULL");
    HIPCHK(ctx, hipStreamSynchronize(ctx->stream));
    return 0;
}

int tpz_ctx_set_lanes(tpz_ctx* ctx, int on) {
    if (!ctx) return fail(nullptr, "ctx is NULL");
    if (on < 0 || on > N_LANES) return fail(ctx, "tpz_ctx_set_lanes: 0 (off), 1 (on, two lanes) or a lane count up to %d", (int)N_LANES);
    ctx->lanes_enabled = on != 0;
    if (on >= 1) ctx->n_lanes = on == 1 ? 2 : on;
    return 0;
}

int tpz_ctx_set_batch(tpz_ctx* ctx, int n) {
    if (!ctx) return fail(nullptr, "ctx is NULL");
    if (n < 0 || n > (int)SPLIT_MULTI_MAX) return fail(ctx, "tpz_ctx_set_batch: 0 (off) or up to %d images per launch", (int)SPLIT_MULTI_MAX);
    ctx->batch = n == 1 ? 0 : n;
    return 0;
}
int tpz_ctx_set_batch_memory(tpz_ctx* ctx, long long bytes) {
    if (!ctx || bytes < 0) return fail(ctx, "tpz_ctx_set_batch_memory: bytes >= 0 (0: 90 %% of the free device memory)");
    ctx->batch_mem = bytes;
    return 0;
}
long long tpz_prof_launches(tpz_ctx* ctx) { return ctx ? ctx->n_launches : 0; }

int tpz_ctx_set_persist(tpz_ctx* ctx, int mode, int workgroups) {
    if (!ctx || mode < 0 || mode > 2 || workgroups < 0) return fail(ctx, "tpz_ctx_set_persist: bad arguments");
    ctx->persist_mode = mode;
    ctx->persist_wgs = workgroups;
    return 0;
}
int tpz_ctx_set_roi(tpz_ctx* ctx, int on) {
    if (!ctx) return 1;
    ctx->roi_enabled = on != 0;
    return 0;
}

int tpz_ctx_set_tiling(tpz_ctx* ctx, long long limit_px, int tile) {
    if (!ctx || limit_px < 1 || tile < 16) return fail(ctx, "tpz_ctx_set_tiling: limit_px >= 1, tile >= 16");
    ctx->tile_limit_px = limit_px;
    ctx->tile_size = tile;
    return 0;
}

int tpz_ctx_set_raster(tpz_ctx* ctx, int on) {
    if (!ctx) return fail(nullptr, "ctx is NULL");
    ctx->raster = on != 0;
    return 0;
}

int tpz_ctx_set_rw(tpz_ctx* ctx, int on) {
    if (!ctx) return fail(nullptr, "ctx is NULL");
    ctx->rw_enabled = on != 0;
    return 0;
}
int tpz_ctx_set_range(tpz_ctx* ctx, int on) {
    if (!ctx) return fail(nullptr, "ctx is NULL");
    ctx->range_scaling = on != 0;
    return 0;
}

int tpz_ctx_set_exact(tpz_ctx* ctx, int on) {
// ... 128 lines not shown
```

### topaz_amd/csrc/rt_forward.hip

```cpp
#include "rt_internal.h"

namespace tpz::rt {
namespace {

bool split_volume_fits(const tpz_model* m, int D, int H, int W) {
    if (D <= 1) return true;
    size_t cmax = 1;
    for (const LayerRT& rt : m->layers)
        if (rt.L.op == TPZ_OP_CONV) cmax = std::max(cmax, (size_t)std::max(rt.L.cin, rt.L.cout));
    return split_cells((int)cmax) * (size_t)D * H * W * 16 < ((size_t)1 << 32) - 16;
}

int model_halo(const tpz_model* m) {
    int h = 0;
    for (const LayerRT& rt : m->layers) {
        const tpz_layer& L = rt.L;
        if (L.op != TPZ_OP_CONV && L.op != TPZ_OP_MAXPOOL && L.op != TPZ_OP_AVGPOOL) return -1;
        h += std::max(L.pad, L.dil * (L.k - 1) - L.pad);
    }
    return (h + 1) & ~1;
}

bool has_padded_pool(const tpz_model* m) {
    for (const LayerRT& rt : m->layers)
// ... 35 lines not shown
            if (!rc) {
                const float* src = ot + (size_t)(ty - y0) * ww + (tx - x0);
                float* dst = out + (size_t)ty * W + tx;
                const hipError_t e = enqueue(ctx, [=](hipStream_t st) {
                    return launch_copy_box(src, (long long)wh * ww, ww, dst, (long long)H * W, W, Co, th, tw, st);
                });
                if (e != hipSuccess) rc = fail(ctx, "copy_box failed: %s", hipGetErrorString(e));
            }
            if (xt) pool_release(ctx, xt);
            if (ot) pool_release(ctx, ot);
            if (rc) return rc;
        }
    return 0;
}

enum PassMode {
    PASS_DEFAULT,
    PASS_SPLIT,
    PASS_FP32,
};

bool split_path_open(const tpz_model* m, int D, int H, int W) { return m->split_ok && split_volume_fits(m, D, H, W); }

int forward_image(tpz_model* m, float* x, int D, int H, int W, float* out_b, int Co, int Do, int Ho, int Wo, PassMode mode,
                  unsigned* overflow_out = nullptr) {
    tpz_ctx* ctx = m->ctx;
    bool done = false;
    if (mode == PASS_SPLIT || (mode == PASS_DEFAULT && !ctx->exact && !m->exact && split_path_open(m, D, H, W))) {
        HIPCHK(ctx, flag_clear(ctx));
        float* x_b = x;
        const bool scaled = ctx->range_scaling && m->layers.back().L.op == TPZ_OP_CONV && m->layers.back().L.head &&
                            m->d_bias_scaled != nullptr;
        float *xs = nullptr, *rng = nullptr;
        if (scaled) {
            const size_t n_in = (size_t)D * H * W;
            rng = next_nrm(ctx);
            xs = (float*)pool_alloc(ctx, n_in * sizeof(float));
            if (!xs) return fail(ctx, "out of device memory");
            hipError_t e = enqueue(ctx, [=](hipStream_t st) {
                return launch_range_fit(x_b, n_in, ctx->d_absmax, rng, m->d_bias_arena, m->d_bias_scaled, m->n_bias_arena, st);
            });
            if (e == hipSuccess) e = enqueue(ctx, [=](hipStream_t st) { return launch_affine_dev(x_b, D, H, W, (long long)H * W, W, rng, xs, st); });
            if (e != hipSuccess) { pool_release(ctx, xs); return fail(ctx, "range scaling failed: %s", hipGetErrorString(e)); }
            x_b = xs;
            ctx->bias_shift = m->d_bias_scaled - m->d_bias_arena;
            ctx->scaled_pass = true;
        }
        const int rc = run_image(m, x_b, D, H, W, out_b, Co, Do, Ho, Wo, true);
        ctx->bias_shift = 0;
        ctx->scaled_pass = false;
        if (xs) pool_release(ctx, xs);
        if (rc) return 1;
        if (scaled) {
            const size_t n_out = (size_t)Co * Do * Ho * Wo;
            const float hb = m->layers.back().head_b;
            HIPCHK(ctx, enqueue(ctx, [=](hipStream_t st) { return launch_unscale(out_b, n_out, rng, hb, st); }));
        }
        unsigned overflow = 0;
        HIPCHK(ctx, flag_read(ctx, &overflow));
        if (mode == PASS_SPLIT) {
            if (overflow_out) *overflow_out = overflow;
            return 0;
        }
        done = (overflow == 0);
        if (done) ++m->n_split; else ++m->n_fallback;
    }
    if (!done && run_image(m, x, D, H, W, out_b, Co, Do, Ho, Wo, false)) return 1;
    return 0;
}

}

}

using namespace tpz;
using namespace tpz::rt;

int tpz_model_forward(tpz_model* m, const float* d_in, int n, int D, int H, int W, float* d_out) {
    if (!m || !d_in || !d_out) return fail(m ? m->ctx : nullptr, "tpz_model_forward: NULL argument");
    tpz_ctx* ctx = m->ctx;
    HIPCHK(ctx, hipSetDevice(ctx->device));
    int Do, Ho, Wo;
    tpz_model_out_shape(m, D, H, W, &Do, &Ho, &Wo);
    if (Do < 1 || Ho < 1 || Wo < 1) return fail(ctx, "input %dx%dx%d too small for this model", D, H, W);
    int Co = 1;
    tpz_model_out_channels(m, &Co);
    for (int b = 0; b < n; ++b)
        if (forward_image(m, const_cast<float*>(d_in) + (size_t)b * D * H * W, D, H, W, d_out + (size_t)b * Co * Do * Ho * Wo, Co, Do,
                          Ho, Wo, PASS_DEFAULT))
            return 1;
    return 0;
}

int tpz_model_calibrate(tpz_model* m, const float* d_in, int D, int H, int W, float bar, tpz_calibration* out) {
    if (!m || !d_in || !out) return fail(m ? m->ctx : nullptr, "tpz_model_calibrate: NULL argument");
    tpz_ctx* ctx = m->ctx;
    HIPCHK(ctx, hipSetDevice(ctx->device));
    memset(out, 0, sizeof *out);
    int Do, Ho, Wo;
    tpz_model_out_shape(m, D, H, W, &Do, &Ho, &Wo);
    if (Do < 1 || Ho < 1 || Wo < 1) return fail(ctx, "tpz_model_calibrate: input %dx%dx%d too small for this model", D, H, W);
    if (!split_path_open(m, D, H, W)) return 0;
    out->eligible = 1;
    int Co = 1;
    tpz_model_out_channels(m, &Co);
    const size_t n_out = (size_t)Co * Do * Ho * Wo;
    float* x = const_cast<float*>(d_in);
    float* y_split = (float*)pool_alloc(ctx, n_out * sizeof(float));
    float* y_exact = (float*)pool_alloc(ctx, n_out * sizeof(float));
    int rc = (!y_split || !y_exact) ? fail(ctx, "out of device memory") : 0;
    unsigned overflow = 0;
    if (!rc) rc = forward_image(m, x, D, H, W, y_split, Co, Do, Ho, Wo, PASS_SPLIT, &overflow);
    if (!rc && overflow) out->overflow = 1;
    if (!rc && !overflow) rc = forward_image(m, x, D, H, W, y_exact, Co, Do, Ho, Wo, PASS_FP32);
    if (!rc && !overflow) rc = delta_stats(ctx, y_split, y_exact, n_out, &out->d);
    if (y_split) pool_release(ctx, y_split);
    if (y_exact) pool_release(ctx, y_exact);
    if (rc || overflow) return rc;
    out->rms_delta = std::sqrt(out->d.sum_sq / (double)n_out);
    if (bar > 0.f && !(out->d.max_abs_delta <= bar)) {
        m->exact = true;
        out->tripped = 1;
    }
    return 0;
}

int tpz_model_set_exact(tpz_model* m, int on) {
    if (!m) return fail(nullptr, "tpz_model_set_exact: model is NULL");
    m->exact = on != 0;
    return 0;
}

int tpz_model_get_exact(tpz_model* m, int* on) {
    if (!m || !on) return fail(m ? m->ctx : nullptr, "tpz_model_get_exact: NULL argument");
    *on = m->exact ? 1 : 0;
    return 0;
}

int tpz_conv_split_2d(tpz_ctx* ctx, const float* d_in, int cin, int H, int W, const float* h_w, const float* h_b,
                      int cout, int k, int dil, int pad, float slope, const float* d_res, int res_crop,
                      const float* h_post_scale, const float* h_post_shift, const float* h_head_w, float head_b,
                      float* d_out, int* overflow) {
    if (!ctx || !d_in || !h_w || !d_out) return fail(ctx, "tpz_conv_split_2d: NULL argument");
    if (slope > 1.f) return fail(ctx, "tpz_conv_split_2d: the 2xf16 epilogue applies max(v, slope * v): slope must be <= 1 (%g)", slope);
    HIPCHK(ctx, hipSetDevice(ctx->device));
    int epi = EPI_PLAIN;
    if (h_head_w) epi = EPI_HEAD;
    else if (d_res) epi = h_post_scale ? EPI_RES_POST : EPI_RES;
    LayerRT rt;
    tpz_layer& L = rt.L;
    memset(&L, 0, sizeof L);
    L.op = TPZ_OP_CONV; L.dims = 2; L.cin = cin; L.cout = cout; L.k = k; L.dil = dil; L.pad = pad; L.slope = slope;
    L.res = d_res ? 1 : -1; L.res_crop = res_crop; L.head = h_head_w ? 1 : 0; L.src2 = -1;
    rt.ks = pick_split(k, dil, cout, epi);
    if (!rt.ks) return fail(ctx, "tpz_conv_split_2d: no 2xf16 kernel for k=%d dil=%d cout=%d epi=%d", k, dil, cout, epi);
    const int span = dil * (k - 1);
    const int Ho = H + 2 * pad - span, Wo = W + 2 * pad - span;
    if (Ho < 1 || Wo < 1) return fail(ctx, "tpz_conv_split_2d: input too small");
    tpz_model tmp;
    tmp.ctx = ctx;
    rt.s_n_cog = (cout + rt.ks->MT - 1) / rt.ks->MT;
    rt.s_n_chunks = (int)((split_cells(cin) + rt.ks->CC - 1) / rt.ks->CC);
    std::vector<uint16_t> packed;
    std::vector<float> inv;
    pack_weights_split(*rt.ks, h_w, cout, cin, rt.s_n_cog, rt.s_n_chunks, packed, inv);
    int rc = upload_halfs(ctx, &tmp, packed, &rt.d_wsplit);
    if (!rc) rc = upload_chan(ctx, &tmp, inv.data(), inv.size(), &rt.d_wscale);
    if (!rc && h_b) rc = upload_chan(ctx, &tmp, h_b, cout, &rt.d_bias);
    if (!rc && h_post_scale) rc = upload_chan(ctx, &tmp, h_post_scale, cout, &rt.d_post_scale);
    if (!rc && h_post_shift) rc = upload_chan(ctx, &tmp, h_post_shift, cout, &rt.d_post_shift);
    if (!rc && h_head_w) { rc = upload_chan(ctx, &tmp, h_head_w, cout, &rt.d_head_w); rt.head_b = head_b; }
    Slot s1, sres, dst;
    float *x_s = nullptr, *r_s = nullptr, *y_s = nullptr;
    const int Hr = Ho + 2 * res_crop, Wr = Wo + 2 * res_crop;
    if (!rc) {
        x_s = (float*)pool_alloc(ctx, split_cells(cin) * 8 * (size_t)H * W * 4);
        y_s = (float*)pool_alloc(ctx, split_cells(cout) * 8 * (size_t)Ho * Wo * 4);
        if (d_res) r_s = (float*)pool_alloc(ctx, split_cells(cout) * 8 * (size_t)Hr * Wr * 4);
        if (!x_s || !y_s || (d_res && !r_s)) rc = fail(ctx, "out of device memory");
    }
    if (!rc) {
        (void)flag_clear(ctx);
        (void)launch_to_split(d_in, x_s, cin, H, W, ctx->d_flag, ctx->stream);
        set_dense(s1, x_s, cin, 1, H, W); s1.split = true;
        if (d_res) { (void)launch_to_split(d_res, r_s, cout, Hr, Wr, ctx->d_flag, ctx->stream); set_dense(sres, r_s, cout, 1, Hr, Wr); sres.split = true; }
        set_dense(dst, L.head ? d_out : y_s, L.head ? 1 : cout, 1, Ho, Wo);
        rc = run_conv_split(ctx, rt, s1, d_res ? &sres : nullptr, dst);
        if (!rc && !L.head) (void)launch_from_split(y_s, d_out, cout, Ho, Wo, ctx->stream);
        unsigned flag = 0;
        if (flag_read(ctx, &flag, false) != hipSuccess) rc = fail(ctx, "tpz_conv_split_2d: kernel failed");
        if (overflow) *overflow = (int)flag;
    }
    if (x_s) pool_release(ctx, x_s);
    if (y_s) pool_release(ctx, y_s);
    if (r_s) pool_release(ctx, r_s);
    for (void* p_ : tmp.dev_allocs) (void)hipFree(p_);
    return rc;
}

int tpz_conv(tpz_ctx* ctx, int dims, const float* d_in, int cin1, int D1, int H1, int W1, const float* d_in2, int cin,
             int D, int H, int W, const float* h_w, const float* h_b, int cout, int k, int dil, int pad, float slope,
             const float* d_res, int res_crop, const float* h_post_scale, const float* h_post_shift,
             const float* h_head_w, float head_b, float* d_out) {
    if (!ctx || !d_in || !h_w || !d_out) return fail(ctx, "tpz_conv: NULL argument");
    HIPCHK(ctx, hipSetDevice(ctx->device));
    const size_t taps = dims == 3 ? (size_t)k * k * k : (size_t)k * k;
    std::vector<float> blob;
    tpz_layer L;
    memset(&L, 0, sizeof L);
    L.op = TPZ_OP_CONV; L.dims = dims; L.src = 0; L.src2 = d_in2 ? 1 : -1; L.dst = 3;
    L.cin = cin; L.cout = cout; L.k = k; L.dil = dil; L.pad = pad; L.slope = slope;
    L.res = d_res ? 2 : -1; L.res_crop = res_crop;
    L.w_off = 0;
    blob.insert(blob.end(), h_w, h_w + (size_t)cout * cin * taps);
    L.b_off = -1;
    if (h_b) { L.b_off = (int64_t)blob.size(); blob.insert(blob.end(), h_b, h_b + cout); }
    L.post_scale_off = L.post_shift_off = -1;
    if (h_post_scale && h_post_shift) {
        L.post_scale_off = (int64_t)blob.size(); blob.insert(blob.end(), h_post_scale, h_post_scale + cout);
        L.post_shift_off = (int64_t)blob.size(); blob.insert(blob.end(), h_post_shift, h_post_shift + cout);
    }
    L.head = h_head_w ? 1 : 0;
    if (h_head_w) {
        L.head_w_off = (int64_t)blob.size(); blob.insert(blob.end(), h_head_w, h_head_w + cout);
        L.head_b_off = (int64_t)blob.size(); blob.push_back(head_b);
    }
    tpz_model* m = nullptr;
    if (model_load(ctx, &L, 1, blob.data(), blob.size(), {cin1, d_in2 ? cin - cin1 : 0, cout}, &m)) return 1;
    std::vector<Slot> slots(4);
    set_dense(slots[0], const_cast<float*>(d_in), cin1, D1, H1, W1);
    if (d_in2) set_dense(slots[1], const_cast<float*>(d_in2), cin - cin1, D, H, W);
    if (d_res) {
        const int span = dil * (k - 1);
        const int Ho = H + 2 * pad - span, Wo = W + 2 * pad - span, Do = dims == 3 ? D + 2 * pad - span : 1;
        set_dense(slots[2], const_cast<float*>(d_res), cout, dims == 3 ? Do + 2 * res_crop : 1, Ho + 2 * res_crop,
                  Wo + 2 * res_crop);
    }
    m->n_slots = 4;
    m->last_use.assign(4, 0);
    int rc = run_program(m, slots, d_out, nullptr);
    if (rc == 0 && hipStreamSynchronize(ctx->stream) != hipSuccess) rc = fail(ctx, "tpz_conv: kernel failed");
    tpz_model_free(m);
    return rc;
}

int tpz_maxpool2(tpz_ctx* ctx, int dims, const float* d_in, int C, int D, int H, int W, float* d_out) {
    if (!ctx || !d_in || !d_out) return fail(ctx, "tpz_maxpool2: NULL argument");
    HIPCHK(ctx, hipSetDevice(ctx->device));
    HIPCHK(ctx, launch_maxpool2(d_in, d_out, C, D, H, W, dims, ctx->stream));
    return 0;
}

int tpz_pool(tpz_ctx* ctx, int op, int dims, const float* d_in, int C, int D, int H, int W, int dil, int pad, int split,
             float* d_out, int* overflow) {
    if (!ctx || !d_in || !d_out) return fail(ctx, "tpz_pool: NULL argument");
    if (overflow) *overflow = 0;
    if (op != TPZ_OP_MAXPOOL && op != TPZ_OP_AVGPOOL) return fail(ctx, "tpz_pool: op must be TPZ_OP_MAXPOOL or TPZ_OP_AVGPOOL");
    if ((dims != 2 && dims != 3) || C < 1 || H < 1 || W < 1 || (dims == 3 && D < 1)) return fail(ctx, "tpz_pool: bad shape");
    if (dil < 1 || pad < 0 || pad > dil) return fail(ctx, "tpz_pool: needs 0 <= pad <= dil");
    if (op == TPZ_OP_AVGPOOL && (dil != 1 || pad != 1)) return fail(ctx, "tpz_pool: the mean takes dil = 1, pad = 1");
    if (dims == 2) D = 1;
    const int grow = 2 * pad - 2 * dil;
    const int Do = dims == 3 ? D + grow : 1, Ho = H + grow, Wo = W + grow;
    if (Do < 1 || Ho < 1 || Wo < 1) return fail(ctx, "tpz_pool: input too small");
    HIPCHK(ctx, hipSetDevice(ctx->device));
    const bool mean = op == TPZ_OP_AVGPOOL;
    int rc = 0;
    if (!split) {
        HIPCHK(ctx, launch_pool_pad(d_in, d_out, C, D, H, W, dil, pad, dims, mean, false, ctx->stream));
    } else {
        float* x_s = (float*)pool_alloc(ctx, split_cells(C) * 8 * (size_t)D * H * W * 4);
        float* y_s = (float*)pool_alloc(ctx, split_cells(C) * 8 * (size_t)Do * Ho * Wo * 4);
        if (!x_s || !y_s) rc = fail(ctx, "out of device memory");
        if (!rc) {
            hipError_t e = flag_clear(ctx);
            if (e == hipSuccess) e = launch_to_split(d_in, x_s, C, D * H, W, ctx->d_flag, ctx->stream);
            if (e == hipSuccess) e = launch_pool_pad(x_s, y_s, C, D, H, W, dil, pad, dims, mean, true, ctx->stream);
            if (e == hipSuccess) e = launch_from_split(y_s, d_out, C, Do * Ho, Wo, ctx->stream);
            if (e != hipSuccess) rc = fail(ctx, "tpz_pool: launch failed: %s", hipGetErrorString(e));
        }
        unsigned flag = 0;
        if (flag_read(ctx, &flag) != hipSuccess) rc = fail(ctx, "tpz_pool: kernel failed");
        if (!rc && overflow) *overflow = (int)flag;
        if (x_s) pool_release(ctx, x_s);
        if (y_s) pool_release(ctx, y_s);
        return rc;
    }
    if (hipStreamSynchronize(ctx->stream) != hipSuccess) rc = fail(ctx, "tpz_pool: kernel failed");
    return rc;
}

int tpz_transpose_2d(tpz_ctx* ctx, const float* d_in, int rows, int cols, float* d_out) {
    if (!ctx || !d_in || !d_out) return fail(ctx, "tpz_transpose_2d: NULL argument");
    HIPCHK(ctx, hipSetDevice(ctx->device));
    prof_begin(ctx, 2, 0);
    hipError_t e = launch_transpose(d_in, d_out, rows, cols, ctx->stream);
    prof_end(ctx);
    HIPCHK(ctx, e);
    return 0;
}

int tpz_filter_2d(tpz_ctx* ctx, const float* d_in, int H, int W, const float* h_w, int k, float bias, float* d_out) {
    if (!ctx || !d_in || !h_w || !d_out || k < 1 || (k & 1) == 0) return fail(ctx, "tpz_filter_2d: bad arguments");
    return tpz_conv(ctx, 2, d_in, 1, 1, H, W, nullptr, 1, 1, H, W, h_w, &bias, 1, k, 1, k / 2, 1.0f, nullptr, 0, nullptr,
                    nullptr, nullptr, 0.f, d_out);
}
```

### topaz_amd/csrc/rt_internal.h

```cpp
#pragma once
#include <hip/hip_runtime.h>
#include <stdarg.h>
#include <stdio.h>
#include <string.h>
#include <algorithm>
#include <chrono>
#include <cmath>
#include <functional>
#include <string>
#include <vector>

#include "../../include/topaz_hip.h"
#include "conv_registry.h"
#include "conv_split_registry.h"
#include "conv_rw.h"
#include "kernels_misc.h"

namespace tpz::rt {

struct DebugEnv {
    bool on = false;
    bool no_phase = false;
    bool exact_fp32 = false;
    bool no_issuer = false;
    bool no_lanes = false;
    bool no_roi = false;
    bool no_persist = false;
    bool trace_host = false;
    bool no_range = false;
    bool no_raster = false;
    bool no_srcmajor = false;
    bool no_valu_last = false;
    bool no_rw = false;
    bool no_pool3d = false;
    bool no_fold = false;
    bool no_widen = false;
    int batch = -1;
    int lanes = 0;
};
DebugEnv debug_env();

static inline double host_now_ms() {
    return std::chrono::duration<double, std::milli>(std::chrono::steady_clock::now().time_since_epoch()).count();
}

#ifndef TPZ_N_LANES
#define TPZ_N_LANES 4
#endif
enum { N_LANES = TPZ_N_LANES };
enum { NMS_BATCH = 4, NMS_VER = 5, NMS_SNAP = 9, NMS_PICKS = 15, NMS_COUNTERS = 16 };

struct ProfRec {
    int cls;
    hipEvent_t e0, e1;
    double flops, bytes;
    const void* key;
};
struct ProfAcc {
    double ms = 0, flops = 0, bytes = 0;
    long long n = 0;
};

struct RecOp {
    const SplitKernelInfo* ks = nullptr;
    SplitArgs a;
    dim3 grid;
    std::function<hipError_t(hipStream_t)> fn;
    int cls = 2;
    double flops = 0, bytes = 0;
    const void* key = nullptr;
};

}

struct tpz_ctx {
    int device = 0;
    tpz::rt::DebugEnv dbg;
    int n_cus = 256;
    hipStream_t own_stream = nullptr;
    hipStream_t stream = nullptr;
    std::string err;
    struct Buf {
        void* p;
        size_t bytes;
        bool used;
    };
    std::vector<Buf> pool;
    std::vector<Buf>* pool_cur = &pool;
    struct Lane {
        hipStream_t stream = nullptr;
        hipEvent_t done = nullptr;
        std::vector<Buf> pool;
        double* d_part = nullptr;
    };
    Lane lanes[tpz::rt::N_LANES];
    struct tpz_stage* io_stage = nullptr;
    hipEvent_t lanes_fork = nullptr;
    hipStream_t lanes_saved_stream = nullptr;
    double* lanes_saved_part = nullptr;
    bool lanes_on = false;
    int lanes_live = 2;
    int n_lanes = 2;
    bool lanes_enabled = true;
    bool roi_enabled = true;
    int persist_mode = 1;
    int persist_wgs = 0;
    int batch = (int)tpz::SPLIT_MULTI_MAX;
    bool rec_on = false;
    double rec_t0 = 0;
    int rec_cur = 0;
    std::vector<tpz::rt::RecOp> rec[tpz::SPLIT_MULTI_MAX];
    std::vector<Buf> rec_pools[TPZ_N_LANES][tpz::SPLIT_MULTI_MAX];
    int rec_lane = 0;
    long long batch_mem = 0;
    long long n_launches = 0;
    long long resample_upload_bytes = 0;
    double* d_part = nullptr;
    float* d_nrm = nullptr;
    int nrm_next = 0;
    unsigned int* d_counters = nullptr;
    float* d_zeros = nullptr;
    ptrdiff_t bias_shift = 0;
    bool scaled_pass = false;
    unsigned* d_absmax = nullptr;
    bool range_scaling = true;
    bool raster = true;
    bool rw_enabled = true;
    long long tile_limit_px = 40LL << 20;
    int tile_size = 4096;
    unsigned* d_flag = nullptr;
    unsigned* h_flag = nullptr;
    bool exact = false;
    struct SplitPlan {
        const tpz::SplitKernelInfo* ks;
        tpz::SplitPlanKey key;
        tpz::SplitStep* d;
        bool next_ok;
    };
    std::vector<SplitPlan> split_plans;
    int prof = 0;
    bool prof_open = false;
    std::vector<tpz::rt::ProfRec> recs;
    std::vector<hipEvent_t> free_events;
    std::vector<std::pair<const void*, tpz::rt::ProfAcc>> per_kernel;
    double acc_ms[4] = {0, 0, 0, 0};
    long long acc_n[4] = {0, 0, 0, 0};
    double acc_flops[4] = {0, 0, 0, 0};
};

namespace tpz::rt {

static const int PART_BLOCKS = 1024;
static const int NRM_RING = 4096;

int fail(tpz_ctx* ctx, const char* fmt, ...);

#define HIPCHK(ctx, expr)                                                                        \
    do {                                                                                         \
        hipError_t e__ = (expr);                                                                 \
        if (e__ != hipSuccess)                                                                   \
            return ::tpz::rt::fail(ctx, "%s failed: %s (%s:%d)", #expr, hipGetErrorString(e__), __FILE__, __LINE__); \
    } while (0)

void* pool_alloc(tpz_ctx* ctx, size_t bytes);
void pool_release(tpz_ctx* ctx, void* p);
hipError_t flag_clear(tpz_ctx* ctx);
hipError_t flag_read(tpz_ctx* ctx, unsigned* flag, bool check_copy = true);
float* next_nrm(tpz_ctx* ctx);
int lanes_begin(tpz_ctx* ctx);
void lane_enter(tpz_ctx* ctx, int k);
int lanes_end(tpz_ctx* ctx);
void prof_begin(tpz_ctx* ctx, int cls, double flops, const void* key = nullptr, double bytes = 0);
void prof_end(tpz_ctx* ctx);
void prof_flush(tpz_ctx* ctx);
int rec_begin(tpz_ctx* ctx, int batch_no = 0);
void rec_select(tpz_ctx* ctx, int i);
void rec_abort(tpz_ctx* ctx);
int rec_flush(tpz_ctx* ctx);
const std::string& last_global_error();
void restore_errors(tpz_ctx* ctx, const std::string& ctx_err, const std::string& global_err);

template <class F>
static hipError_t enqueue(tpz_ctx* ctx, int cls, double flops, const void* key, double bytes, F&& fn) {
    if (ctx->rec_on) {
        RecOp op;
        op.fn = std::forward<F>(fn);
        op.cls = cls; op.flops = flops; op.key = key; op.bytes = bytes;
        ctx->rec[ctx->rec_cur].push_back(std::move(op));
        return hipSuccess;
// ... 1 lines not shown
    prof_begin(ctx, cls, flops, key, bytes);
    const hipError_t e = fn(ctx->stream);
    prof_end(ctx);
    ++ctx->n_launches;
    return e;
}
template <class F>
static hipError_t enqueue(tpz_ctx* ctx, F&& fn) { return enqueue(ctx, 2, 0.0, nullptr, 0.0, std::forward<F>(fn)); }

struct LayerRT {
    tpz_layer L;
    const ConvKernelInfo* ki = nullptr;
    int n_cog = 1, n_chunks = 1, cog_inner = 1;
    int c1 = 0, c2 = 0;
    float* d_wpk = nullptr;
    float* d_bias = nullptr;
    float* d_post_scale = nullptr;
    float* d_post_shift = nullptr;
    float* d_head_w = nullptr;
    float head_b = 0.f;
    float bias0 = 0.f;
    const SplitKernelInfo* ks = nullptr;
    const ConvKernelInfo* ki_stem_split = nullptr;
    void* d_wsplit = nullptr;
    float* d_wscale = nullptr;
    int s_n_cog = 1, s_n_chunks = 1;
    const SplitKernelInfo* ks_stem = nullptr;
    const SplitKernelInfo* ks_last = nullptr;
    float* d_wlast = nullptr;
    void* d_w_rw = nullptr;
    float* d_ws_rw = nullptr;
    const SplitKernelInfo* ks_pool = nullptr;
    int folded_into = -1;
    int fold_src = -1, fold_cells = 0, f_n_cog = 1, f_n_chunks = 1;
    const SplitKernelInfo* ks_fold = nullptr;
    void* d_wfold = nullptr;
    float* d_wscale_fold = nullptr;
    float* d_bias_fold = nullptr;
    struct SplitPhase {
        bool valid = false;
        const SplitKernelInfo* ks_low = nullptr;
        const SplitKernelInfo* ks_skip = nullptr;
        const ConvKernelInfo* ki_skip_stem = nullptr;
        int n_cog_low = 1, n_chunks_low = 1, n_cog_skip = 1, n_chunks_skip = 1;
        const SplitKernelInfo* ks_sub = nullptr;
        int n_cog_sub = 1;
        bool sub_with_skip = false;
        bool low_with_skip = false;
        bool srcmajor = false;
        const SplitKernelInfo* ks_low_plain = nullptr;
        void* d_w_low = nullptr;
        float* d_ws_low = nullptr;
        size_t w_phase_bytes = 0;
        void* d_w_skip = nullptr;
        float* d_ws_skip = nullptr;
    } sphase;
    struct Phase {
        bool valid = false;
        int c1 = 0, c2 = 0, k1 = 0;
        const ConvKernelInfo* ki_low = nullptr;
        const ConvKernelInfo* ki_skip = nullptr;
        int n_cog_low = 1, n_chunks_low = 1, n_cog_skip = 1, n_chunks_skip = 1;
        float* d_w_low[8] = {nullptr, nullptr, nullptr, nullptr, nullptr, nullptr, nullptr, nullptr};
        float* d_w_skip = nullptr;
    } phase;
};

}

struct tpz_model {
    tpz_ctx* ctx = nullptr;
    tpz::rt::DebugEnv dbg;
    std::vector<tpz::rt::LayerRT> layers;
    int n_slots = 0;
    std::vector<int> last_use;
    std::vector<void*> dev_allocs;
    float* d_bias_arena = nullptr;
    float* d_bias_scaled = nullptr;
    size_t n_bias_arena = 0;
    int n_conv = 0, n_conv_split = 0;
    std::string off_path;
    bool split_ok = false;
    bool widened = false;
    long long n_split = 0, n_fallback = 0;
    bool exact = false;
};

namespace tpz::rt {

struct Rect {
    int y0 = 0, x0 = 0, y1 = 0, x1 = 0;
    bool on = false;
    int z0 = 0, z1 = 1;
    void unite(const Rect& r) {
        if (!r.on) return;
        if (!on) { *this = r; return; }
        y0 = std::min(y0, r.y0); x0 = std::min(x0, r.x0); y1 = std::max(y1, r.y1); x1 = std::max(x1, r.x1);
        z0 = std::min(z0, r.z0); z1 = std::max(z1, r.z1);
    }
    long long area() const { return (long long)(y1 - y0) * (x1 - x0); }
};

struct Slot {
    Rect need;
    float* p = nullptr;
    int C = 0, D = 1, H = 0, W = 0;
    long long cs = 0, ps = 0;
    int pitch = 0;
    bool owned = false;
    bool set = false;
    bool split = false;
    bool pooled = false;
    float* alt = nullptr;
};

static void set_dense(Slot& s, float* p, int C, int D, int H, int W) {
    s.p = p; s.C = C; s.D = D; s.H = H; s.W = W;
    s.pitch = W; s.ps = (long long)H * W; s.cs = s.ps * D;
    s.set = true;
}

static inline const float* bias_view(const tpz_ctx* ctx, const float* p) { return p ? p + ctx->bias_shift : nullptr; }

enum ConvForm {
    FORM_FP32,
    FORM_FP32_STEM_SPLIT,
    FORM_SPLIT,
    FORM_SPLIT_FOLD,
    FORM_STEM,
    FORM_LAST,
    FORM_PARITY,
    FORM_FOLDED_AWAY,
};
struct ConvPlan {
    ConvForm form = FORM_FP32;
    bool fuse_pool = false;
    bool split_dst = false;
    bool split1 = false, split2 = false, split_res = false;
};
struct Dhw { int D = 1, H = 0, W = 0; };

static inline Dhw layer_out_dhw(const tpz_layer& L, const Dhw& g) {
    if (L.op == TPZ_OP_MAXPOOL2) return {L.dims == 3 ? g.D / 2 : 1, g.H / 2, g.W / 2};
    const int grow = 2 * L.pad - L.dil * (L.k - 1);
    return {L.dims == 3 ? g.D + grow : 1, g.H + grow, g.W + grow};
}
static inline bool is_padded_pool(const tpz_layer& L) { return L.op == TPZ_OP_AVGPOOL || (L.op == TPZ_OP_MAXPOOL && L.pad > 0); }

static inline size_t chan_pad(size_t n) { return (n + 127) / 128 * 128 + 128; }
static inline int phase_pad(int k, int p) { return (k / 2 - p + 1) / 2; }
int upload(tpz_ctx* ctx, tpz_model* m, const float* h, size_t n, float** out);
int upload_chan(tpz_ctx* ctx, tpz_model* m, const float* h, size_t n, float** out);
int upload_halfs(tpz_ctx* ctx, tpz_model* m, const std::vector<uint16_t>& h, void** out);
void pack_weights_split(const SplitKernelInfo& ki, const float* w, int cout, int cin, int n_cog, int n_chunks,
                        std::vector<uint16_t>& out, std::vector<float>& wscale_inv, const float* wp = nullptr, int cin_b = 0,
                        const float* mul = nullptr);
const SplitKernelInfo* pick_split(int k, int dil, int cout, int epi, int kx = 0);
int model_load(tpz_ctx* ctx, const tpz_layer* layers, int n_layers, const float* h_blob, size_t n_floats,
               const std::vector<int>& preset_chan, tpz_model** out);
unsigned split_forms(const tpz_model* m, int i);
ConvPlan conv_plan(const tpz_model* m, int i, bool split, const Dhw& g1, const Dhw* g2, bool split1, bool fold_set);
int run_conv_split(tpz_ctx* ctx, const LayerRT& rt, const Slot& s1, const Slot* sres, Slot& dst, const Slot* s2 = nullptr,
                   bool pooled = false, const Slot* fold = nullptr);
int run_program(tpz_model* m, std::vector<Slot>& slots, float* d_out, const float* d_nrm, bool split = false,
                const Rect* keep = nullptr);
tpz_ctx* resample_ctx(tpz_resample* plan);
int delta_stats(tpz_ctx* ctx, const float* d_a, const float* d_b, size_t n, tpz_delta* out);
static inline double beta_logpdf(double x, double a, double b) {
    const double t1 = (b - 1.0) == 0.0 ? 0.0 : (b - 1.0) * std::log1p(-x);
    const double t2 = (a - 1.0) == 0.0 ? 0.0 : (a - 1.0) * std::log(x);
    return t1 + t2 - (std::lgamma(a) + std::lgamma(b) - std::lgamma(a + b));
}
struct GmmMoments { double mu_all, var_unbiased; };
static inline GmmMoments gmm_moments(const double* S, double N) {
    const double mu_all = S[3] / N;
    return {mu_all, (S[5] - 2.0 * mu_all * S[3] + mu_all * mu_all * N) / (N - 1.0)};
}
static inline void gmm_single_component(const GmmMoments& M, double N, double alpha, double beta, double scale, double& logp,
                                        double& mu, double& sd, double& pi) {
    const double pdf1 = beta == 1.0 ? std::exp(-(std::lgamma(alpha) + std::lgamma(beta) - std::lgamma(alpha + beta)))
                                    : (beta > 1.0 ? 0.0 : INFINITY);
    logp = scale * (-(N - 1.0) / 2.0 - N * 0.5 * std::log(2.0 * M_PI * M.var_unbiased)) + pdf1;
    mu = M.mu_all;
    sd = std::sqrt(M.var_unbiased);
    pi = 1.0;
}
static inline void gmm_m_step(const double* T, double N, double mu_all, double& mu0, double& mu1, double& var) {
    mu0 = T[1] > 0 ? T[3] / T[1] : mu_all;
    mu1 = T[2] > 0 ? T[4] / T[2] : mu_all;
    var = ((T[5] - 2.0 * mu0 * T[3] + mu0 * mu0 * T[1]) + (T[6] - 2.0 * mu1 * T[4] + mu1 * mu1 * T[2])) / N;
}
static inline double gmm_map_pi(const double* S, double N, double alpha, double beta) {
    const double a_ = alpha + S[2], b_ = beta + N - S[2];
    return (a_ - 1.0) / (a_ + b_ - 2.0);
}
static inline void gmm_e_step_par(double mu0, double mu1, double var, double pi, double (&par)[6]) {
    par[0] = mu0; par[1] = mu1; par[2] = var; par[3] = var; par[4] = std::log1p(-pi); par[5] = std::log(pi);
}

hipError_t launch_mfma_spin(const void* src, float* out, int n_wg, int iters, unsigned long long* ticks, hipStream_t s);

}
```

### topaz_amd/csrc/rt_load.hip

```cpp
#include "rt_internal.h"

namespace tpz::rt {

int upload(tpz_ctx* ctx, tpz_model* m, const float* h, size_t n, float** out) {
    float* d = nullptr;
    HIPCHK(ctx, hipMalloc((void**)&d, std::max<size_t>(n, 4) * sizeof(float)));
    HIPCHK(ctx, hipMemcpy(d, h, n * sizeof(float), hipMemcpyHostToDevice));
    if (m) m->dev_allocs.push_back(d);
    *out = d;
    return 0;
}

int upload_chan(tpz_ctx* ctx, tpz_model* m, const float* h, size_t n, float** out) {
    std::vector<float> padded(chan_pad(n), 0.f);
    memcpy(padded.data(), h, n * sizeof(float));
    return upload(ctx, m, padded.data(), padded.size(), out);
}

namespace {

template <class Find>
auto pick_by_padded_width(int cout, Find find) -> decltype(find(0)) {
    decltype(find(0)) best = nullptr;
    int best_padded = 1 << 30;
// ... 14 lines not shown
}

const ConvKernelInfo* choose_kernel(const tpz_layer& L) {
    if (L.cout == 1 && !L.head) return nullptr;
    const bool cin1 = (L.cin == 1 && L.src2 < 0);
    int epi = EPI_PLAIN;
    if (L.head) epi = EPI_HEAD;
    else if (L.res >= 0) epi = L.post_scale_off >= 0 ? EPI_RES_POST : EPI_RES;
    if ((L.head && (L.res >= 0 || L.post_scale_off >= 0)) || (L.res < 0 && L.post_scale_off >= 0)) return nullptr;
    return pick_conv(L.dims, L.k, L.dil, L.cout, cin1, epi);
}

void pack_weights(const ConvKernelInfo& ki, const float* w, int cout, int cin, int n_cog, int n_chunks,
                  std::vector<float>& out) {
    const int K = ki.K, KZ = ki.dims == 3 ? K : 1, MW = ki.MT / 16;
    out.assign((size_t)n_cog * n_chunks * ki.W_CHUNK, 0.f);
    const size_t taps = (size_t)KZ * K * K;
    for (int cog = 0; cog < n_cog; ++cog)
        for (int ch = 0; ch < n_chunks; ++ch)
            for (int j = 0; j < ki.SPG; ++j) {
                float* blk = out.data() + ((size_t)cog * n_chunks + ch) * ki.W_CHUNK + (size_t)j * ki.W_STAGE;
                for (int step = 0; step < ki.STEPS; ++step)
                    for (int mf = 0; mf < MW; ++mf)
                        for (int k = 0; k < 4; ++k)
                            for (int i = 0; i < 16; ++i) {
                                const int co = cog * ki.MT + mf * 16 + i;
                                int ci, kx, row;
                                if (ki.cin1) {
                                    row = j * ki.RPS + step / ki.KXG;
                                    kx = (step % ki.KXG) * 4 + k;
                                    ci = 0;
                                } else {
                                    const int kg = step / (ki.RPS * K);
                                    row = j * ki.RPS + (step / K) % ki.RPS;
                                    kx = step % K;
                                    ci = ch * ki.NCH + kg * 4 + k;
                                }
                                const int kz = row / K, ky = row % K;
                                float v = 0.f;
                                if (co < cout && ci < cin && kx < K)
                                    v = w[((size_t)co * cin + ci) * taps + ((size_t)kz * K + ky) * K + kx];
                                blk[((size_t)step * MW + mf) * 64 + k * 16 + i] = v;
                            }
            }
}

int phase_tap(int k, int p, int ky) {
    const int v = p + ky - k / 2;
    return (v >= 0 ? v / 2 : -((-v + 1) / 2)) + phase_pad(k, p);
}

void phase_weights(const tpz_layer& L, const float* w, int c1, int p, std::vector<double>& acc) {
    const int k = L.k, k1 = k / 2 + 1, kz_n = L.dims == 3 ? k : 1;
    const size_t taps = (size_t)kz_n * k * k, taps1 = (size_t)(L.dims == 3 ? k1 : 1) * k1 * k1;
    const int px = p & 1, py = (p >> 1) & 1, pz = L.dims == 3 ? (p >> 2) & 1 : 0;
    acc.assign((size_t)L.cout * c1 * taps1, 0.0);
    for (int co = 0; co < L.cout; ++co)
        for (int ci = 0; ci < c1; ++ci)
            for (int kz = 0; kz < kz_n; ++kz)
                for (int ky = 0; ky < k; ++ky)
                    for (int kx = 0; kx < k; ++kx) {
                        const int tz = L.dims == 3 ? phase_tap(k, pz, kz) : 0;
                        acc[((size_t)co * c1 + ci) * taps1 + ((size_t)tz * k1 + phase_tap(k, py, ky)) * k1 + phase_tap(k, px, kx)] +=
                            (double)w[((size_t)co * L.cin + ci) * taps + ((size_t)kz * k + ky) * k + kx];
                    }
}

void skip_weights(const tpz_layer& L, const float* w, int c1, int c2, std::vector<float>& eff) {
    const size_t taps = L.dims == 3 ? (size_t)L.k * L.k * L.k : (size_t)L.k * L.k;
    eff.resize((size_t)L.cout * c2 * taps);
    for (int co = 0; co < L.cout; ++co)
        for (int ci = 0; ci < c2; ++ci)
            memcpy(&eff[((size_t)co * c2 + ci) * taps], &w[((size_t)co * L.cin + c1 + ci) * taps], taps * sizeof(float));
}

int prepare_phases(tpz_ctx* ctx, tpz_model* m, const tpz_layer& L, const float* w, int c1, int c2, LayerRT& rt) {
    LayerRT::Phase& ph = rt.phase;
    if (L.src2 < 0 || L.dil != 1 || (L.k != 3 && L.k != 5) || L.pad != L.k / 2 || L.res >= 0 || L.head ||
        L.post_scale_off >= 0 || c1 + c2 != L.cin || c1 < 1 || c2 < 1)
        return 0;
    const int k = L.k, k1 = k / 2 + 1, dims = L.dims;
    ph.ki_low = pick_conv(dims, k1, 1, L.cout, false, EPI_PLAIN);
    ph.ki_skip = pick_conv(dims, k, 1, L.cout, c2 == 1, EPI_RES);
    if (!ph.ki_low || !ph.ki_skip) return 0;
    ph.c1 = c1; ph.c2 = c2; ph.k1 = k1;
    ph.n_cog_low = (L.cout + ph.ki_low->MT - 1) / ph.ki_low->MT;
    ph.n_chunks_low = (c1 + ph.ki_low->NCH - 1) / ph.ki_low->NCH;
    ph.n_cog_skip = (L.cout + ph.ki_skip->MT - 1) / ph.ki_skip->MT;
    ph.n_chunks_skip = ph.ki_skip->cin1 ? 1 : (c2 + ph.ki_skip->NCH - 1) / ph.ki_skip->NCH;
    std::vector<double> acc;
    std::vector<float> eff, packed;
    for (int p = 0; p < (1 << dims); ++p) {
        phase_weights(L, w, c1, p, acc);
        eff.assign(acc.begin(), acc.end());
        pack_weights(*ph.ki_low, eff.data(), L.cout, c1, ph.n_cog_low, ph.n_chunks_low, packed);
        if (upload(ctx, m, packed.data(), packed.size(), &ph.d_w_low[p])) return 1;
    }
    skip_weights(L, w, c1, c2, eff);
    pack_weights(*ph.ki_skip, eff.data(), L.cout, c2, ph.n_cog_skip, ph.n_chunks_skip, packed);
    if (upload(ctx, m, packed.data(), packed.size(), &ph.d_w_skip)) return 1;
    ph.valid = true;
    return 0;
}

int prepare_layer(tpz_ctx* ctx, tpz_model* m, const tpz_layer& L, const float* blob, size_t n_floats, LayerRT& rt,
                  int c1 = 0, int c2 = 0) {
    rt.L = L;
    rt.c1 = c1; rt.c2 = c2;
    if (L.op == TPZ_OP_MAXPOOL && (L.pad < 0 || L.pad > L.dil || (L.pad > 0 && L.k != 3) || L.dil < 1 || L.k < 1))
        return fail(ctx, "maxpool: pad %d needs k = 3 and pad <= dil (k %d, dil %d)", L.pad, L.k, L.dil);
    if (L.op == TPZ_OP_AVGPOOL && (L.k != 3 || L.dil != 1 || L.pad != 1)) return fail(ctx, "avgpool: only k = 3, dil = 1, pad = 1");
    if (L.op != TPZ_OP_CONV && L.op != TPZ_OP_MAXPOOL2 && L.op != TPZ_OP_MAXPOOL && L.op != TPZ_OP_AVGPOOL) return fail(ctx, "unknown op %d", L.op);
    if (L.op != TPZ_OP_CONV && L.dims != 2 && L.dims != 3) return fail(ctx, "pool: dims must be 2 or 3");
    if (L.op != TPZ_OP_CONV) return 0;
    if (L.dims != 2 && L.dims != 3) return fail(ctx, "conv: dims must be 2 or 3");
    const size_t taps = (L.dims == 3 ? (size_t)L.k * L.k * L.k : (size_t)L.k * L.k);
    const size_t wn = (size_t)L.cout * L.cin * taps;
    if (L.w_off < 0 || (size_t)L.w_off + wn > n_floats) return fail(ctx, "conv: weight offset out of range");
    const float* w = blob + L.w_off;
    rt.ki = choose_kernel(L);
    if (rt.ki) {
        const ConvKernelInfo& ki = *rt.ki;
        rt.n_cog = (L.cout + ki.MT - 1) / ki.MT;
        rt.n_chunks = ki.cin1 ? 1 : (L.cin + ki.NCH - 1) / ki.NCH;
        rt.cog_inner = L.head ? rt.n_cog : 1;
        std::vector<float> packed;
        pack_weights(ki, w, L.cout, L.cin, rt.n_cog, rt.n_chunks, packed);
        if (upload(ctx, m, packed.data(), packed.size(), &rt.d_wpk)) return 1;
        if (!m->dbg.no_phase && prepare_phases(ctx, m, L, w, c1, c2, rt)) return 1;
    } else {
        if (L.src2 >= 0 || L.head || L.post_scale_off >= 0)
            return fail(ctx, "conv k=%d dil=%d cin=%d cout=%d dims=%d: no MFMA kernel compiled and the direct "
                        "kernel has no concat/head/affine epilogue", L.k, L.dil, L.cin, L.cout, L.dims);
        if (upload(ctx, m, w, wn, &rt.d_wpk)) return 1;
    }
    if (L.b_off >= 0) {
        if ((size_t)L.b_off + L.cout > n_floats) return fail(ctx, "conv: bias offset out of range");
        rt.bias0 = blob[L.b_off];
        if (upload_chan(ctx, m, blob + L.b_off, L.cout, &rt.d_bias)) return 1;
    }
    if (L.post_scale_off >= 0) {
        if (upload_chan(ctx, m, blob + L.post_scale_off, L.cout, &rt.d_post_scale)) return 1;
        if (upload_chan(ctx, m, blob + L.post_shift_off, L.cout, &rt.d_post_shift)) return 1;
    }
    if (L.head) {
        if (upload_chan(ctx, m, blob + L.head_w_off, L.cout, &rt.d_head_w)) return 1;
        rt.head_b = blob[L.head_b_off];
    }
    return 0;
}

}

void pack_weights_split(const SplitKernelInfo& ki, const float* w, int cout, int cin, int n_cog, int n_chunks,
                        std::vector<uint16_t>& out, std::vector<float>& wscale_inv, const float* wp, int cin_b, const float* mul) {
    const int K = ki.K, KX = ki.KX, MW = ki.MT / 16;
    const size_t taps = (size_t)K * KX;
    std::vector<float> scale(cout, 1.f);
    wscale_inv.assign(cout, 1.f);
    for (int co = 0; co < cout; ++co) {
        float mx = 0.f;
        const float f = mul ? std::fabs(mul[co]) : 1.f;
        for (size_t i = 0; i < (size_t)cin * taps; ++i) mx = std::max(mx, f * std::fabs(w[(size_t)co * cin * taps + i]));
        for (int i = 0; wp && i < cin_b; ++i) mx = std::max(mx, f * std::fabs(wp[(size_t)co * cin_b + i]));
        int e = 0;
        if (mx > 0.f && std::isfinite(mx)) e = std::min(60, std::max(-60, (int)std::floor(std::log2(16384.0 / mx))));
        scale[co] = std::ldexp(1.f, e);
        wscale_inv[co] = std::ldexp(1.f, -e);
    }
    const size_t step_halfs = (size_t)ki.W_STEP_BYTES / 2;
    const int cells = (int)split_cells(cin);
    const int n_stages_a = ki.stages(cells);
    const int n_stages = n_stages_a + (wp ? (int)split_cells(cin_b) / ki.CC : 0);
    const int n_full = cells / ki.CC, n_rem = cells - n_full * ki.CC, taps_n = ki.cont ? ki.Q / ki.CC : 0;
    out.assign((size_t)n_cog * n_stages * step_halfs, 0);
    auto put = [&](uint16_t* blk, int m, int kb, int i, int j, float v) {
        const _Float16 hi = (_Float16)v;
        const _Float16 lo = (_Float16)(v - (float)hi);
        uint16_t hb, lb;
        memcpy(&hb, &hi, 2);
        memcpy(&lb, &lo, 2);
        const size_t lane = (size_t)kb * 16 + i;
        blk[((size_t)(0 * MW + m) * 64 + lane) * 8 + j] = hb;
        blk[((size_t)(1 * MW + m) * 64 + lane) * 8 + j] = lb;
    };
    for (int cog = 0; cog < n_cog; ++cog)
        for (int st = 0; st < n_stages; ++st) {
            uint16_t* blk = out.data() + ((size_t)cog * n_stages + st) * step_halfs;
            if (st >= n_stages_a) {
                const int cb = st - n_stages_a;
                for (int kb = 0; kb < ki.CC; ++kb)
                    for (int m = 0; m < MW; ++m)
                        for (int i = 0; i < 16; ++i) {
                            const int co = cog * ki.MT + m * 16 + i;
                            if (co >= cout) continue;
                            for (int j = 0; j < 8; ++j) {
                                const int ci = (cb * ki.CC + kb) * 8 + j;
                                if (ci < cin_b) put(blk, m, kb, i, j, wp[(size_t)co * cin_b + ci] * scale[co] * (mul ? mul[co] : 1.f));
                            }
                        }
                continue;
            }
            for (int kb = 0; kb < 4; ++kb) {
                int ch;
                SplitSlot sl;
                if (ki.cont) {
                    const int G = 4 * st + kb;
                    ch = G / ki.Q;
                    if (ch < n_full) {
                        sl = ki.cont_slot(G % ki.Q);
                    } else {
                        const int q2 = G - n_full * ki.Q;
                        if (n_rem == 0 || q2 >= taps_n * n_rem) continue;
                        ch = n_full;
                        sl = ki.cont_slot((q2 / n_rem) * ki.CC + (q2 % n_rem));
                    }
                } else {
                    ch = st / ki.NSTEP;
                    sl = ki.slot(st % ki.NSTEP, kb);
                    if (sl.ky < 0) continue;
                }
                for (int m = 0; m < MW; ++m)
                    for (int i = 0; i < 16; ++i) {
                        const int co = cog * ki.MT + m * 16 + i;
                        if (co >= cout) continue;
                        for (int j = 0; j < 8; ++j) {
                            const int ci = (ch * ki.CC + sl.c) * 8 + j;
                            if (ci >= cin) continue;
                            put(blk, m, kb, i, j, w[((size_t)co * cin + ci) * taps + (size_t)sl.ky * KX + sl.kx] * scale[co] * (mul ? mul[co] : 1.f));
                        }
                    }
            }
        }
}

const SplitKernelInfo* pick_split(int k, int dil, int cout, int epi, int kx) {
    return pick_by_padded_width(cout, [&](int mt) { return find_split(k, dil, mt, epi, kx); });
}

int upload_halfs(tpz_ctx* ctx, tpz_model* m, const std::vector<uint16_t>& h, void** out) {
    float* d = nullptr;
    if (upload(ctx, m, reinterpret_cast<const float*>(h.data()), (h.size() + 1) / 2, &d)) return 1;
    *out = d;
    return 0;
}

namespace {

void pack_weights_split_stacked(const SplitKernelInfo& ks, const float* w, int cout, int cin, int* n_cog, int* n_chunks,
                                std::vector<uint16_t>& packed, std::vector<float>& inv, int kz_n = 1, int c1_major = 0) {
    std::vector<float> stacked;
    if (kz_n > 1) {
        const int c8 = (int)split_cells(cin) * 8, k = ks.K;
        const size_t taps2 = (size_t)k * ks.KX;
        stacked.assign((size_t)cout * kz_n * c8 * taps2, 0.f);
        for (int co = 0; co < cout; ++co)
            for (int ci = 0; ci < cin; ++ci)
                for (int kz = 0; kz < kz_n; ++kz) {
                    size_t vch = (size_t)kz * c8 + ci;
                    if (c1_major > 0)
                        vch = ci < c1_major ? (size_t)kz * c1_major + ci
                                            : (size_t)kz_n * c1_major + (size_t)kz * (c8 - c1_major) + (ci - c1_major);
                    memcpy(&stacked[((size_t)co * kz_n * c8 + vch) * taps2],
                           &w[(((size_t)co * cin + ci) * kz_n + kz) * taps2], taps2 * sizeof(float));
                }
        w = stacked.data();
        cin = kz_n * c8;
    }
    *n_cog = (cout + ks.MT - 1) / ks.MT;
    *n_chunks = (int)((split_cells(cin) + ks.CC - 1) / ks.CC);
    pack_weights_split(ks, w, cout, cin, *n_cog, *n_chunks, packed, inv);
}

int upload_split_weights(tpz_ctx* ctx, tpz_model* m, const SplitKernelInfo& ks, const float* w, int cout, int cin, int* n_cog,
                         int* n_chunks, void** d_w, float** d_ws, int kz_n = 1) {
    std::vector<uint16_t> packed;
    std::vector<float> inv;
    pack_weights_split_stacked(ks, w, cout, cin, n_cog, n_chunks, packed, inv, kz_n);
    if (upload_halfs(ctx, m, packed, d_w)) return 1;
    return upload_chan(ctx, m, inv.data(), inv.size(), d_ws);
}

int prepare_split_phases(tpz_ctx* ctx, tpz_model* m, const float* w, LayerRT& rt) {
    const tpz_layer& L = rt.L;
    const LayerRT::Phase& ph = rt.phase;
    LayerRT::SplitPhase& sp = rt.sphase;
    if (!ph.valid || ph.c1 % 8 != 0) return 0;
    const int k = L.k, k1 = ph.k1, c1 = ph.c1, c2 = ph.c2, dims = L.dims;
    const int kz_n = dims == 3 ? k : 1, k1z_n = dims == 3 ? k1 : 1;
    sp.ks_low = pick_split(k1, 1, L.cout, EPI_RES);
    if (!sp.ks_low) return 0;
    if (c2 == 1) {
        if (!ph.ki_skip->cin1) return 0;
        sp.ki_skip_stem = find_conv(dims, k, 1, ph.ki_skip->MT, true, EPI_SPLIT);
        if (!sp.ki_skip_stem || ph.n_cog_skip != 1) return 0;
    } else {
        sp.ks_skip = pick_split(k, 1, L.cout, EPI_PLAIN);
        if (!sp.ks_skip) return 0;
    }
    const size_t taps = (size_t)kz_n * k * k, taps1 = (size_t)k1z_n * k1 * k1;
    if (k == 3 && c2 == 1) {
        sp.ks_low_plain = find_split(k1, 1, sp.ks_low->MT, EPI_PLAIN);
        if (sp.ks_low_plain && sp.ks_low_plain->CC == sp.ks_low->CC && sp.ks_low_plain->WAVES == sp.ks_low->WAVES &&
            (dims == 3 || (c1 / 8) % sp.ks_low_plain->CC == 0))
            sp.low_with_skip = true;
    }
    const int c1e = sp.low_with_skip ? c1 + 8 : c1;
    std::vector<double> acc;
    std::vector<float> eff, all_s, sub_w, inv;
    std::vector<uint16_t> all_w, packed;
    for (int p = 0; p < (1 << dims); ++p) {
        const int px = p & 1, py = (p >> 1) & 1, pz = dims == 3 ? (p >> 2) & 1 : 0;
        phase_weights(L, w, c1, p, acc);
        eff.assign((size_t)L.cout * c1e * taps1, 0.f);
        for (int co = 0; co < L.cout; ++co)
            for (size_t i = 0; i < (size_t)c1 * taps1; ++i) eff[(size_t)co * c1e * taps1 + i] = (float)acc[(size_t)co * c1 * taps1 + i];
        if (sp.low_with_skip) {
            const int nq = 1 << dims;
            for (int co = 0; co < L.cout; ++co)
                for (int q = 0; q < nq; ++q) {
                    const int qx = q & 1, qy = (q >> 1) & 1, qz = dims == 3 ? (q >> 2) & 1 : 0;
                    for (int tz = 0; tz < k1z_n; ++tz)
                        for (int ty = 0; ty < k1; ++ty)
                            for (int tx = 0; tx < k1; ++tx) {
                                const int dz = dims == 3 ? 2 * (tz - phase_pad(k, pz)) + qz - pz : 0;
                                const int dy = 2 * (ty - phase_pad(k, py)) + qy - py, dx = 2 * (tx - phase_pad(k, px)) + qx - px;
                                if (dz < -1 || dz > 1 || dy < -1 || dy > 1 || dx < -1 || dx > 1) continue;
                                const int kz = dims == 3 ? dz + 1 : 0;
                                eff[((size_t)co * c1e + c1 + q) * taps1 + ((size_t)tz * k1 + ty) * k1 + tx] =
                                    w[((size_t)co * L.cin + c1) * taps + ((size_t)kz * k + (dy + 1)) * k + (dx + 1)];
                            }
                }
        }
        if (!sp.low_with_skip) sub_w.insert(sub_w.end(), eff.begin(), eff.end());
        const bool no_srcmajor = m->dbg.no_srcmajor;
        sp.srcmajor = dims == 3 && sp.low_with_skip && !no_srcmajor && (k1z_n * (c1 / 8)) % sp.ks_low_plain->CC == 0;
        pack_weights_split_stacked(sp.low_with_skip ? *sp.ks_low_plain : *sp.ks_low, eff.data(), L.cout, c1e, &sp.n_cog_low,
                                   &sp.n_chunks_low, packed, inv, k1z_n, sp.srcmajor ? c1 : 0);
        sp.w_phase_bytes = packed.size() * sizeof(uint16_t);
        all_w.insert(all_w.end(), packed.begin(), packed.end());
        inv.resize(chan_pad(L.cout), 0.f);
        all_s.insert(all_s.end(), inv.begin(), inv.end());
    }
    if (dims == 2 && k == 5 && L.cout % 16 == 0) sp.ks_sub = find_split(k1, 1, 128, EPI_RES);
    if (sp.ks_sub && c2 == 1) {
        const SplitKernelInfo* pl = find_split(k1, 1, 128, EPI_PLAIN);
        if (pl && pl->CC == sp.ks_sub->CC) {
            const int cin2 = c1 + 8;
            std::vector<float> w2((size_t)4 * L.cout * cin2 * taps1, 0.f);
            for (int p = 0; p < 4; ++p)
                for (int co = 0; co < L.cout; ++co) {
                    const size_t v = (size_t)p * L.cout + co;
                    memcpy(&w2[v * cin2 * taps1], &sub_w[v * c1 * taps1], (size_t)c1 * taps1 * sizeof(float));
                    const int px = p & 1, py = (p >> 1) & 1;
                    for (int q = 0; q < 4; ++q)
                        for (int ty = 0; ty < 3; ++ty)
                            for (int tx = 0; tx < 3; ++tx) {
                                const int ky = 2 * (ty - 1) + (q >> 1) - py + 2, kx = 2 * (tx - 1) + (q & 1) - px + 2;
                                if (ky < 0 || ky > 4 || kx < 0 || kx > 4) continue;
                                w2[(v * cin2 + c1 + q) * taps1 + (size_t)ty * 3 + tx] = w[((size_t)co * L.cin + c1) * taps + (size_t)ky * 5 + kx];
                            }
                }
            sub_w.swap(w2);
            sp.ks_sub = pl;
            sp.sub_with_skip = true;
        }
    }
    if (sp.ks_sub) {
        all_w.clear(); all_s.clear();
        if (upload_split_weights(ctx, m, *sp.ks_sub, sub_w.data(), 4 * L.cout, sp.sub_with_skip ? c1 + 8 : c1, &sp.n_cog_sub,
                                 &sp.n_chunks_low, &sp.d_w_low, &sp.d_ws_low)) return 1;
    } else {
        if (upload_halfs(ctx, m, all_w, &sp.d_w_low)) return 1;
        if (upload(ctx, m, all_s.data(), all_s.size(), &sp.d_ws_low)) return 1;
    }
    if (sp.ks_skip) {
        skip_weights(L, w, c1, c2, eff);
        if (upload_split_weights(ctx, m, *sp.ks_skip, eff.data(), L.cout, c2, &sp.n_cog_skip, &sp.n_chunks_skip,
                                 &sp.d_w_skip, &sp.d_ws_skip, kz_n)) return 1;
    }
    sp.valid = true;
    return 0;
}

int prepare_split(tpz_ctx* ctx, tpz_model* m, const float* blob) {
    const int nl = (int)m->layers.size();
    std::vector<int> reads(nl, 0);
    for (int i = 0; i < nl; ++i) {
        LayerRT& rt = m->layers[i];
        const tpz_layer& L = rt.L;
        if (L.op == TPZ_OP_CONV && L.slope > 1.f) continue;
        if (L.op == TPZ_OP_CONV && !rt.ki && L.cout == 1 && L.cin % 8 == 0 && L.src2 < 0 && (L.res < 0 || L.res_crop == 0) && !L.head &&
            L.post_scale_off < 0 && L.dil == 1 && L.pad == L.k / 2 && L.slope == 1.f && i == nl - 1) {
            rt.ks_last = find_split(L.k, 1, 16, EPI_PLAIN_F32, 1);
            reads[i] = rt.ks_last ? 1 : 0;
            continue;
        }
        if (L.op != TPZ_OP_CONV || !rt.ki || rt.ki->cin1) continue;
        if (L.src2 >= 0) {
            if (prepare_split_phases(ctx, m, blob + L.w_off, rt)) return 1;
            if (L.dims == 2 && rt.ki->epi == EPI_PLAIN && rt.c1 + rt.c2 == L.cin) {
                rt.ks = pick_split(L.k, L.dil, L.cout, EPI_PLAIN);
                if (rt.ks && rt.c1 % (8 * rt.ks->CC) != 0) rt.ks = nullptr;
            }
            reads[i] = (rt.sphase.valid || rt.ks) ? 1 : 0;
            continue;
        }
        rt.ks = pick_split(L.k, L.dil, L.cout, rt.ki->epi);
        if (!rt.ks && rt.ki->epi == EPI_PLAIN) rt.ks = pick_split(L.k, L.dil, L.cout, EPI_PLAIN_F32);
        reads[i] = rt.ks ? 1 : 0;
    }
    std::function<bool(int)> slot_read_split = [&](int slot) {
        bool any = false;
        for (int j = 0; j < nl; ++j) {
            const tpz_layer& Lj = m->layers[j].L;
            const bool uses = Lj.src == slot || Lj.src2 == slot || Lj.res == slot;
            if (!uses) continue;
            if (Lj.op == TPZ_OP_MAXPOOL2 || Lj.op == TPZ_OP_MAXPOOL || Lj.op == TPZ_OP_AVGPOOL) any |= slot_read_split(Lj.dst);
            else if (Lj.src2 == slot && m->layers[j].sphase.valid && m->layers[j].sphase.ki_skip_stem) continue;
            else any |= reads[j] != 0;
        }
        return any;
    };
    bool any_split = false;
    for (int i = 0; i < nl; ++i) {
        LayerRT& rt = m->layers[i];
        const tpz_layer& L = rt.L;
        if (L.op != TPZ_OP_CONV) continue;
        const bool wanted = slot_read_split(L.dst);
        if (rt.ki && rt.ki->cin1 && L.src2 < 0) {
            if (!(wanted && L.res < 0 && !L.head && L.post_scale_off < 0)) continue;
            if (L.dil == 1 && !(L.slope > 1.f)) rt.ks_stem = pick_split(L.k, 1, L.cout, EPI_PLAIN, 1);
            if (rt.ks_stem) {
                const int k = L.k, kz_n = L.dims == 3 ? k : 1, c8 = (k + 7) / 8 * 8;
                std::vector<float> w2((size_t)L.cout * c8 * kz_n * k, 0.f);
                const float* w = blob + L.w_off;
                for (int co = 0; co < L.cout; ++co)
                    for (int kz = 0; kz < kz_n; ++kz)
                        for (int ky = 0; ky < k; ++ky)
                            for (int kx = 0; kx < k; ++kx)
                                w2[(((size_t)co * c8 + kx) * kz_n + kz) * k + ky] = w[(((size_t)co * kz_n + kz) * k + ky) * k + kx];
                if (upload_split_weights(ctx, m, *rt.ks_stem, w2.data(), L.cout, c8, &rt.s_n_cog, &rt.s_n_chunks,
                                         &rt.d_wsplit, &rt.d_wscale, kz_n)) return 1;
                any_split = true;
            } else if (rt.n_cog == 1) {
                rt.ki_stem_split = find_conv(L.dims, L.k, L.dil, rt.ki->MT, true, EPI_SPLIT);
            }
            continue;
        }
        if (rt.ks_last) {
            const int k = L.k, kz_n = L.dims == 3 ? k : 1;
            const float* w = blob + L.w_off;
            const bool no_valu_last = m->dbg.no_valu_last;
            if (!no_valu_last && (k == 3 || k == 5) && (size_t)L.cin * k * k * kz_n <= 1024) {
                const int cells = (int)split_cells(L.cin);
                std::vector<float> wl((size_t)kz_n * cells * k * k * 8, 0.f);
                for (int ci = 0; ci < L.cin; ++ci)
                    for (int kz = 0; kz < kz_n; ++kz)
                        for (int ky = 0; ky < k; ++ky)
                            for (int kx = 0; kx < k; ++kx)
                                wl[((((size_t)kz * cells + ci / 8) * k + kx) * k + ky) * 8 + ci % 8] =
                                    w[(((size_t)ci * kz_n + kz) * k + ky) * k + kx];
                if (upload(ctx, m, wl.data(), wl.size(), &rt.d_wlast)) return 1;
            }
            std::vector<float> w2((size_t)k * L.cin * kz_n * k);
            for (int v = 0; v < k; ++v)
                for (int ci = 0; ci < L.cin; ++ci)
                    for (int kz = 0; kz < kz_n; ++kz)
                        for (int ky = 0; ky < k; ++ky)
                            w2[(((size_t)v * L.cin + ci) * kz_n + kz) * k + ky] = w[(((size_t)ci * kz_n + kz) * k + ky) * k + v];
            if (upload_split_weights(ctx, m, *rt.ks_last, w2.data(), k, L.cin, &rt.s_n_cog, &rt.s_n_chunks,
                                     &rt.d_wsplit, &rt.d_wscale, kz_n)) return 1;
            any_split = true;
            continue;
        }
        if (rt.ks) {
            if (!L.head && !wanted && rt.ks->epi == EPI_PLAIN && L.src2 < 0) {
                const SplitKernelInfo* f = find_split(L.k, L.dil, rt.ks->MT, EPI_PLAIN_F32);
                if (!f) f = pick_split(L.k, L.dil, L.cout, EPI_PLAIN_F32);
                if (f) rt.ks = f;
            }
            if (i == nl - 1 && !L.head && rt.ks->epi != EPI_PLAIN_F32) rt.ks = nullptr;
        }
        if (rt.ks) {
            if (upload_split_weights(ctx, m, *rt.ks, blob + L.w_off, L.cout, L.cin, &rt.s_n_cog, &rt.s_n_chunks,
                                     &rt.d_wsplit, &rt.d_wscale, L.dims == 3 ? L.k : 1)) return 1;
            any_split = true;
            const bool no_rw = m->dbg.no_rw;
            if (!no_rw && L.dims == 2 && L.k == 3 && L.cin == 32 && L.cout == 32 && L.src2 < 0 && !L.head &&
                (L.dil == 1 || L.dil == 2 || L.dil == 4) && rt.ks->epi <= EPI_RES_POST) {
                SplitKernelInfo rw;
                memset(&rw, 0, sizeof rw);
                rw.K = rw.KX = 3; rw.D = L.dil; rw.MT = 32; rw.CC = 4; rw.cont = 1; rw.Q = 36; rw.SPS = 1;
                rw.W_STEP_BYTES = 2 * (32 / 16) * 1024;
                rw.cont_slot = [](int q) { return SplitSlot{(q / 4) / 3, (q / 4) % 3, q % 4}; };
                int n_cog = 0, n_chunks = 0;
                if (upload_split_weights(ctx, m, rw, blob + L.w_off, L.cout, L.cin, &n_cog, &n_chunks, &rt.d_w_rw, &rt.d_ws_rw)) return 1;
            }
        }
        if (rt.sphase.valid) any_split = true;
    }
    for (int i = 0; i + 1 < nl; ++i) {
        LayerRT& rt = m->layers[i];
        const tpz_layer& L = rt.L;
        const bool no_pool3d = m->dbg.no_pool3d;
        if (L.op != TPZ_OP_CONV || L.dil != 1 || L.head || L.res >= 0 || L.post_scale_off >= 0 || (L.dims == 3 && no_pool3d)) continue;
        const SplitKernelInfo* base = rt.ks_stem ? rt.ks_stem : ((rt.ks && L.src2 < 0 && rt.ks->epi == EPI_PLAIN) ? rt.ks : nullptr);
        if (!base) continue;
        int readers = 0, pool = -1;
        for (int j = 0; j < nl; ++j) {
            const tpz_layer& Lj = m->layers[j].L;
            if (Lj.src == L.dst || Lj.src2 == L.dst || Lj.res == L.dst) { ++readers; if (Lj.op == TPZ_OP_MAXPOOL2 && Lj.src == L.dst) pool = j; }
        }
        if (readers != 1 || pool != i + 1) continue;
        const SplitKernelInfo* pk = find_split(base->K, base->D, base->MT, EPI_POOL, base->KX);
        if (pk && pk->CC == base->CC && pk->NSTEP == base->NSTEP && pk->cont == base->cont && pk->W_STEP_BYTES == base->W_STEP_BYTES) rt.ks_pool = pk;
    }
    const bool no_fold = m->dbg.no_fold;
    for (int i = 0; i < nl && !no_fold; ++i) {
        LayerRT& rt = m->layers[i];
        const tpz_layer& L = rt.L;
        if (L.op != TPZ_OP_CONV || L.dims != 2 || !rt.ks || L.res < 0 || L.src2 >= 0 || L.head || L.k % 2 == 0) continue;
        if (rt.ks->epi != EPI_RES && rt.ks->epi != EPI_RES_POST) continue;
        int j = -1, readers = 0;
        for (int t = 0; t < nl; ++t) {
            const tpz_layer& T = m->layers[t].L;
            if (T.dst == L.res && t < i) j = t;
            if (T.src == L.res || T.src2 == L.res || T.res == L.res) ++readers;
        }
        if (j < 0 || readers != 1) continue;
        LayerRT& pj = m->layers[j];
        const tpz_layer& P = pj.L;
        if (P.op != TPZ_OP_CONV || P.dims != 2 || P.k != 1 || P.pad != 0 || P.slope != 1.f || P.b_off >= 0 || P.res >= 0 ||
            P.src2 >= 0 || P.head || P.post_scale_off >= 0 || P.cout != L.cout || !pj.ks) continue;
        const SplitKernelInfo* kf = find_split(L.k, L.dil, rt.ks->MT, EPI_PLAIN, 0, 1);
        if (!kf || !kf->cont || kf->CC != 2 || L.cin % 16 != 0 || P.cin % 16 != 0) continue;
        std::vector<float> mul, bias(L.cout, 0.f);
        if (L.b_off >= 0) memcpy(bias.data(), blob + L.b_off, L.cout * sizeof(float));
        if (L.post_scale_off >= 0) {
            mul.assign(blob + L.post_scale_off, blob + L.post_scale_off + L.cout);
            for (int c = 0; c < L.cout; ++c) bias[c] = bias[c] * mul[c] + blob[L.post_shift_off + c];
        }
        rt.f_n_cog = (L.cout + kf->MT - 1) / kf->MT;
        rt.fold_cells = (int)split_cells(P.cin);
        rt.f_n_chunks = (int)split_cells(L.cin) / kf->CC + rt.fold_cells / kf->CC;
        std::vector<uint16_t> packed;
        std::vector<float> inv;
        pack_weights_split(*kf, blob + L.w_off, L.cout, L.cin, rt.f_n_cog, rt.f_n_chunks, packed, inv, blob + P.w_off, P.cin,
                           mul.empty() ? nullptr : mul.data());
        if (upload_halfs(ctx, m, packed, &rt.d_wfold)) return 1;
        if (upload_chan(ctx, m, inv.data(), inv.size(), &rt.d_wscale_fold)) return 1;
        if (upload_chan(ctx, m, bias.data(), bias.size(), &rt.d_bias_fold)) return 1;
        rt.ks_fold = kf;
        rt.fold_src = P.src;
        pj.folded_into = i;
        m->last_use[P.src] = std::max(m->last_use[P.src], i);
    }
    m->split_ok = any_split;
    m->n_conv = m->n_conv_split = 0;
    m->off_path.clear();
    for (int i = 0; i < nl; ++i) {
        const LayerRT& rt = m->layers[i];
        const tpz_layer& L = rt.L;
        if (L.op != TPZ_OP_CONV) continue;
        ++m->n_conv;
        if (split_forms(m, i)) { ++m->n_conv_split; continue; }
        char buf[96];
        snprintf(buf, sizeof buf, "%s#%d %dx%d d%d %d->%d", m->off_path.empty() ? "" : ", ", i, L.k, L.k, L.dil, L.cin, L.cout);
        if (m->off_path.size() < 400) m->off_path += buf;
    }
    return 0;
}

int build_bias_arena(tpz_ctx* ctx, tpz_model* m) {
    std::vector<std::pair<float**, size_t>> vecs;
    for (LayerRT& rt : m->layers) {
        if (rt.L.op != TPZ_OP_CONV) continue;
        const size_t n = chan_pad((size_t)rt.L.cout);
        if (rt.d_bias) vecs.push_back({&rt.d_bias, n});
        if (rt.d_post_shift) vecs.push_back({&rt.d_post_shift, n});
        if (rt.d_bias_fold) vecs.push_back({&rt.d_bias_fold, n});
    }
    size_t total = 0;
    for (auto& v : vecs) total += v.second;
    if (total == 0) return 0;
    float *arena = nullptr, *scaled = nullptr;
    HIPCHK(ctx, hipMalloc((void**)&arena, total * sizeof(float)));
    m->dev_allocs.push_back(arena);
    HIPCHK(ctx, hipMalloc((void**)&scaled, total * sizeof(float)));
    m->dev_allocs.push_back(scaled);
    size_t off = 0;
    for (auto& v : vecs) {
        HIPCHK(ctx, hipMemcpy(arena + off, *v.first, v.second * sizeof(float), hipMemcpyDeviceToDevice));
        *v.first = arena + off;
        off += v.second;
    }
    HIPCHK(ctx, hipMemcpy(scaled, arena, total * sizeof(float), hipMemcpyDeviceToDevice));
    m->d_bias_arena = arena; m->d_bias_scaled = scaled; m->n_bias_arena = total;
    return 0;
}

bool widen_program(const tpz_layer* layers, int n_layers, const float* blob, size_t n_floats, std::vector<tpz_layer>& out_l,
                   std::vector<float>& out_b) {
    int max_slot = 0;
    for (int i = 0; i < n_layers; ++i)
        max_slot = std::max(max_slot, std::max(std::max(layers[i].src, layers[i].src2), std::max(layers[i].dst, layers[i].res)));
    std::vector<int> chan(max_slot + 1, 0), pch(max_slot + 1, 0);
    chan[0] = pch[0] = 1;
    auto pad16 = [](int c) { return c <= 1 ? c : (c + 15) / 16 * 16; };
    bool any = false;
    out_l.assign(layers, layers + n_layers);
    out_b.assign(blob, blob + n_floats);
    std::vector<char> is_out(max_slot + 1, 0);
    is_out[layers[n_layers - 1].dst] = 1;
    for (int i = n_layers - 1; i >= 0 && layers[i].op != TPZ_OP_CONV; --i)
        if (layers[i].dst >= 0 && layers[i].dst <= max_slot && is_out[layers[i].dst] && layers[i].src >= 0 && layers[i].src <= max_slot)
            is_out[layers[i].src] = 1;
    for (int i = 0; i < n_layers; ++i) {
        tpz_layer& L = out_l[i];
        if (L.src < 0 || L.src > max_slot || L.dst <= 0) return false;
        const int c1 = chan[L.src], c2 = L.src2 >= 0 ? chan[L.src2] : 0;
        const int p1 = pch[L.src], p2 = L.src2 >= 0 ? pch[L.src2] : 0;
        if (L.op != TPZ_OP_CONV) { chan[L.dst] = c1; pch[L.dst] = p1; continue; }
        if (L.cin != c1 + c2 || L.w_off < 0) return false;
        const size_t taps = L.dims == 3 ? (size_t)L.k * L.k * L.k : (size_t)L.k * L.k;
        if ((size_t)L.w_off + (size_t)L.cout * L.cin * taps > n_floats) return false;
        const bool last = is_out[L.dst] != 0;
        const int pco = (last || L.cout == 1) ? L.cout : pad16(L.cout);
        chan[L.dst] = L.head ? 1 : L.cout;
        pch[L.dst] = L.head ? 1 : pco;
        if (pco == L.cout && p1 == c1 && p2 == c2) continue;
        any = true;
        const int pci = p1 + p2;
        const size_t w_new = out_b.size();
        out_b.resize(w_new + (size_t)pco * pci * taps, 0.f);
        for (int co = 0; co < L.cout; ++co) {
            memcpy(&out_b[w_new + ((size_t)co * pci) * taps], blob + L.w_off + ((size_t)co * L.cin) * taps, (size_t)c1 * taps * sizeof(float));
            if (c2 > 0)
                memcpy(&out_b[w_new + ((size_t)co * pci + p1) * taps], blob + L.w_off + ((size_t)co * L.cin + c1) * taps,
                       (size_t)c2 * taps * sizeof(float));
        }
        auto widen_vec = [&](int64_t& off) {
            if (off < 0 || pco == L.cout) return;
            const size_t o = out_b.size();
            out_b.resize(o + pco, 0.f);
            memcpy(&out_b[o], blob + off, (size_t)L.cout * sizeof(float));
            off = (int64_t)o;
        };
        widen_vec(L.b_off); widen_vec(L.post_scale_off); widen_vec(L.post_shift_off);
        if (L.head) widen_vec(L.head_w_off);
        L.w_off = (int64_t)w_new;
        L.cin = pci;
        L.cout = pco;
    }
    return any;
}

int model_load_one(tpz_ctx* ctx, const tpz_layer* layers, int n_layers, const float* h_blob, size_t n_floats,
                   const std::vector<int>& preset_chan, tpz_model** out) {
    if (!ctx || !layers || !out || n_layers < 1) return fail(ctx, "tpz_model_load: bad arguments");
    *out = nullptr;
    HIPCHK(ctx, hipSetDevice(ctx->device));
    tpz_model* m = new tpz_model();
    m->ctx = ctx;
    m->dbg = debug_env();
    int max_slot = 0;
    for (int i = 0; i < n_layers; ++i) {
        const tpz_layer& L = layers[i];
        max_slot = std::max(max_slot, std::max(std::max(L.src, L.src2), std::max(L.dst, L.res)));
// ... 87 lines not shown
```

Before: 8.861.

## Add ky-run slot ordering for 5x5 split convs to reuse B fragments across rows

Adds a KYRUN variant of the split-fp32 MFMA conv for 5x5 kernels. Each wave owns four output rows of one 16-column fragment, and the slot stream is ordered in runs over ky. Consecutive ky steps then reuse B fragments held in registers: each step loads only one new row instead of all NW fragments. This cuts LDS reads per MFMA. The cost is extra B registers (NW+K-1), a new DMA plan generator, new instantiations, and kernel selection that now prefers ky-run kernels for 2-D layers.

```diff
diff --git a/topaz_amd/csrc/conv_split.h b/topaz_amd/csrc/conv_split.h
--- a/topaz_amd/csrc/conv_split.h
+++ b/topaz_amd/csrc/conv_split.h
@@ -1,6 +1,7 @@
 #pragma once
 #include <hip/hip_runtime.h>
 #include <stdint.h>
+#include <type_traits>
 #include <vector>
 
 #include "conv_mfma.h"
@@ -67,16 +68,22 @@
 struct SplitSlot {
     int ky, kx, c;
 };
-
-template <int K_, int D_, int MT_, int TH_, int TW_, int CC_, int WAVES_ = 8, int KX_ = K_, int SPS_ = 1>
+struct SplitRunSlot {
+    int chunk;
+    SplitSlot sl;
+};
+
+template <int K_, int D_, int MT_, int TH_, int TW_, int CC_, int WAVES_ = 8, int KX_ = K_, int SPS_ = 1, bool KYRUN_ = false>
 struct SplitCfg {
     static constexpr int K = K_, KX = KX_, D = D_, MT = MT_, TH = TH_, TW = TW_, CC = CC_;
+    static constexpr bool KYRUN = KYRUN_;
     static constexpr int WAVES = WAVES_, THREADS = 64 * WAVES_, WGS_PER_CU = WAVES_ == 8 ? 1 : 2;
     static constexpr bool UNIFORM_DMA = (MT_ >= 128 && WAVES_ == 8);
     static constexpr bool ISSUER_HALF = (MT_ >= 96 && WAVES_ == 8);
     static constexpr int MW = MT / 16;
-    static constexpr int RPW = TH / WAVES;
-    static constexpr int NFC = TW / 16;
+    static constexpr int WCOLS = KYRUN ? TW / 16 : 1;
+    static constexpr int RPW = KYRUN ? 4 : TH / WAVES;
+    static constexpr int NFC = KYRUN ? 1 : TW / 16;
     static constexpr int NW = RPW * NFC;
     static constexpr int ITH = TH + K - 1;
     static constexpr int ITW = (CC == 1) ? (TW + (KX - 1) * D + 15) / 16 * 16 : TW + (KX - 1) * D;
@@ -110,6 +117,26 @@
         }
         return (e < KX && j == 0) ? SplitSlot{K - 1, e, 0} : SplitSlot{-1, 0, 0};
     }
+    __host__ __device__ static constexpr int kyrun_runs(int cells) {
+        const int pairs = cells / (2 * CC), rem = cells - pairs * 2 * CC;
+        return pairs * KX + (rem * KX + 3) / 4;
+    }
+    __host__ __device__ static constexpr int kyrun_stages(int cells) { return K * kyrun_runs(cells); }
+    __host__ __device__ static constexpr SplitRunSlot kyrun_slot(int cells, int step, int kb) {
+        const int run = step / K, ky = step - run * K;
+        const int pair = run / KX, left = cells - pair * 2 * CC;
+        const int na = left < CC ? left : CC, nb = left - na < CC ? left - na : CC;
+        const int ca = 2 * pair, cb = 2 * pair + 1;
+        int g = 4 * (run - pair * KX) + kb;
+        if (g < na * (KX - 1)) return SplitRunSlot{ca, SplitSlot{ky, g / na, g % na}};
+        g -= na * (KX - 1);
+        if (g < na) return SplitRunSlot{ca, SplitSlot{ky, KX - 1, g}};
+        g -= na;
+        if (g < nb) return SplitRunSlot{cb, SplitSlot{ky, KX - 1, g}};
+        g -= nb;
+        if (g < nb * (KX - 1)) return SplitRunSlot{cb, SplitSlot{ky, g / nb, g % nb}};
+        return SplitRunSlot{-1, SplitSlot{-1, 0, 0}};
+    }
     __host__ __device__ static constexpr int slot_lds_off(int step, int kb) {
         SplitSlot s = slot(step, kb);
         if (s.ky < 0) s = slot(step, kb & ~1);
@@ -129,6 +156,8 @@
     static_assert(LDS_BYTES <= 160 * 1024 / WGS_PER_CU, "LDS per workgroup");
     static_assert(WAVES == 8 || WAVES == 4, "waves per workgroup");
     static_assert(SPS == 1 || (CONT && Q >= 8 * SPS), "multi-step stages: continuous slot stream, chunks of >= 2 * SPS steps");
+    static_assert(!KYRUN || (K == 5 && KX == 5 && CC == 2 && TH % 4 == 0 && (TH / 4) * (TW / 16) == WAVES && 2 * K >= 2 * SPS - 1),
+                  "ky runs: 5x5 taps, chunks of two cells, four rows x one column fragment per wave");
 };
 
 struct SplitPlanKey {
@@ -136,7 +165,72 @@
 };
 
 template <class C>
+void split_plan_finish(std::vector<SplitStep>& out, unsigned next_rounds) {
+    if (next_rounds == (1u << C::NR) - 1u) out[0].dma |= SPLIT_DMA_NEXT;
+    const size_t n = out.size();
+    out.resize(2 * n);
+    for (size_t i = 0; i < n; ++i) {
+        SplitStep e = out[i];
+        for (int l4 = 0; l4 < 4; ++l4) {
+            const int off = e.bofs[l4] * 16;
+            e.bofs[l4] = (uint16_t)((off >= C::IN_BUF ? off - C::IN_BUF : off + C::IN_BUF) / 16);
+        }
+        if (e.dma & SPLIT_DMA_ANY) e.dma ^= SPLIT_DMA_BUF;
+        out[n + i] = e;
+    }
+}
+
+template <class C>
+void split_make_plan_kyrun(const SplitPlanKey& k, std::vector<SplitStep>& out) {
+    const int cells = k.cells_in, nch = k.n_chunks, n_stages = C::kyrun_stages(cells);
+    out.assign((size_t)n_stages + 1, SplitStep{});
+    std::vector<int> first((size_t)nch + 1, n_stages), last((size_t)nch + 1, -1);
+    for (int s = 0; s < n_stages; ++s)
+        for (int l4 = 0; l4 < 4; ++l4) {
+            SplitRunSlot rs = C::kyrun_slot(cells, s, l4);
+            if (rs.sl.ky < 0) rs = C::kyrun_slot(cells, s, 0);
+            out[(size_t)s + 1].bofs[l4] =
+                (uint16_t)((rs.chunk & 1) * (C::IN_BUF / 16) + rs.sl.c * C::CELL_STRIDE + rs.sl.ky * C::ITW + rs.sl.kx * C::D);
+            if (s < first[rs.chunk]) first[rs.chunk] = s;
+            if (s > last[rs.chunk]) last[rs.chunk] = s;
+        }
+    auto fetch = [&](SplitStep& e, int pf, unsigned rmask, bool sw) {
+        e.dma = SPLIT_DMA_ANY | (rmask & SPLIT_DMA_ROUNDS) | ((pf & 1) ? SPLIT_DMA_BUF : 0u) | (sw ? SPLIT_DMA_SWITCH : 0u);
+        e.cidx = (uint32_t)pf;
+        const int have = cells - pf * C::CC;
+        if (have < C::CC) e.dma |= (uint32_t)(have > 1 ? have : 1) << SPLIT_DMA_NCELL_SHIFT;
+    };
+    fetch(out[0], 0, (1u << C::NR) - 1, false);
+    unsigned next_rounds = 0;
+    for (int pf = 1; pf <= nch; ++pf) {
+        const int ws = pf >= 2 ? last[pf - 2] + 1 : 0, we = (pf < nch ? first[pf] : n_stages) - 1;
+        const int gs = (ws + C::SPS - 1) / C::SPS, ge = (we + 1) / C::SPS - 1;
+        const int rstride = ge - gs + 1;
+        for (int stage = gs; stage <= ge; ++stage) {
+            const int r0 = stage - gs;
+            if (r0 >= C::NR) break;
+            unsigned rmask = 0;
+            for (int r = r0; r < C::NR; r += rstride) rmask |= 1u << r;
+            SplitStep& e = out[(size_t)stage * C::SPS + 1];
+            if (pf < nch) {
+                fetch(e, pf, rmask, false);
+            } else {
+                fetch(e, 0, rmask, r0 == 0);
+                e.dma |= SPLIT_DMA_NEXT;
+                if (nch & 1) e.dma |= SPLIT_DMA_BUF;
+                next_rounds |= rmask;
+            }
+        }
+    }
+    split_plan_finish<C>(out, next_rounds);
+}
+
+template <class C>
 void split_make_plan(const SplitPlanKey& k, std::vector<SplitStep>& out) {
+    if constexpr (C::KYRUN) {
+        split_make_plan_kyrun<C>(k, out);
+        return;
+    }
     const bool vol = k.vol != 0;
     const bool folded = C::CONT && C::SPS == 1 && k.fold_cells > 0;
     const int vcells = (folded ? k.cells_in1 : k.cells_in) * (vol ? k.KZ : 1);
@@ -247,18 +341,7 @@
             next_rounds |= rmask;
         }
     }
-    if (next_rounds == (1u << C::NR) - 1u) out[0].dma |= SPLIT_DMA_NEXT;
-    const size_t n = out.size();
-    out.resize(2 * n);
-    for (size_t i = 0; i < n; ++i) {
-        SplitStep e = out[i];
-        for (int l4 = 0; l4 < 4; ++l4) {
-            const int off = e.bofs[l4] * 16;
-            e.bofs[l4] = (uint16_t)((off >= C::IN_BUF ? off - C::IN_BUF : off + C::IN_BUF) / 16);
-        }
-        if (e.dma & SPLIT_DMA_ANY) e.dma ^= SPLIT_DMA_BUF;
-        out[n + i] = e;
-    }
+    split_plan_finish<C>(out, next_rounds);
 }
 
 enum { EPI_PLAIN_F32 = 5, EPI_POOL = 6 };
@@ -271,6 +354,7 @@
     static_assert(!UNI2 || (HAS2 && VOLM), "MODE 11 = two sources, plane-stacked, chunk-uniform");
     constexpr bool PERSIST = (MODE & 4) != 0;
     static_assert(!PERSIST || (MODE == 4 && EPI != EPI_HEAD), "persistent tiles: plain single-source layers");
+    static_assert(!C::KYRUN || ((MODE == 0 || MODE == 4) && (EPI == EPI_PLAIN || EPI == EPI_PLAIN_F32)), "ky runs: plain single-source 2-D layers");
     const uint4* const in2 = HAS2 ? a.in2 : nullptr;
     const int fold_cells = HAS2 ? a.fold_cells : 0;
     extern __shared__ __attribute__((aligned(16))) unsigned char lds[];
@@ -498,7 +582,7 @@
             }
     };
 
-    const unsigned b_lane = (unsigned)(((wave * C::RPW) * C::ITW + l15) * 16);
+    const unsigned b_lane = (unsigned)((((wave / C::WCOLS) * C::RPW) * C::ITW + (wave % C::WCOLS) * 16 + l15) * 16);
     const unsigned a_lane = (unsigned)(C::OFF_W + lane * 16);
     auto b_frag_base = [&](const StepW& P, int l4) -> const unsigned char* {
         const unsigned w = (l4 & 2) ? P[1] : P[0];
@@ -512,7 +596,7 @@
 
     const bool folded = C::CONT && C::SPS == 1 && fold_cells > 0;
     const int vcells = (folded ? a.cells_in1 : a.cells_in) * (vol ? a.KZ : 1);
-    const int n_stages_a = C::CONT ? C::cont_stages(vcells) : a.n_chunks * C::NSTEP;
+    const int n_stages_a = C::KYRUN ? C::kyrun_stages(vcells) : C::CONT ? C::cont_stages(vcells) : a.n_chunks * C::NSTEP;
     const int n_stages = n_stages_a + (folded ? fold_cells / C::CC : 0);
     const size_t w_cog_bytes = (size_t)n_stages * C::W_STEP_BYTES;
 
@@ -560,7 +644,8 @@
             __syncthreads();
         }
 
-        f16x8 bh[NW], bo[NW], ah[2], ao[2];
+        constexpr int NB = C::KYRUN ? NW + C::K - 1 : NW;
+        f16x8 bh[NB], bo[NB], ah[2], ao[2];
         auto b_off = [&](int n) { return ((n / NFC) * C::ITW + (n % NFC) * 16) * 16; };
         {
             const unsigned char* bl = b_frag_base(P, l4_p);
@@ -578,8 +663,12 @@
         if constexpr ((ABL & 2048) != 0) probe_t1 = __builtin_readcyclecounter();
         if constexpr ((ABL & 524288) != 0) { if (C::WAVES == 8 && wave >= 4) __builtin_amdgcn_s_setprio(1); }
         if constexpr ((ABL & 1048576) != 0) { if (C::WAVES == 8 && wave < 4) __builtin_amdgcn_s_setprio(1); }
-#pragma unroll 1
-        for (int s = 0; s < n_stages; ++s) {
+        auto do_step = [&](const int s, auto kyc) {
+            constexpr int KY = decltype(kyc)::value;
+            constexpr int RB = KY < 0 ? 0 : KY;
+            constexpr bool RUN_END = KY < 0 || KY == C::K - 1;
+            constexpr int NLD = RUN_END ? NW : 1;
+            constexpr int LD_N = RUN_END ? 0 : NW - 1, LD_R = RUN_END ? 0 : KY + NW;
             const int stage = s / C::SPS, sub = s - stage * C::SPS;
             const bool stage_end = sub == C::SPS - 1 || s == n_stages - 1;
             const StepW Pn = plan[1 + (s + 1 < n_stages ? s + 1 : s)];
@@ -669,28 +758,28 @@
                 if constexpr (!(ABL & 16)) {
 #pragma unroll
                     for (int n = 0; n < NW; ++n)
-                        acc[m][n] = __builtin_amdgcn_mfma_f32_16x16x32_f16(a_hi, bo[n], acc[m][n], 0, 0, 0);
+                        acc[m][n] = __builtin_amdgcn_mfma_f32_16x16x32_f16(a_hi, bo[RB + n], acc[m][n], 0, 0, 0);
                     if (last) {
 #pragma unroll
-                        for (int n = 0; n < NW; ++n) bo[n] = *reinterpret_cast<const f16x8*>(bl_next + b_off(n) + C::PLANE_BYTES);
+                        for (int j = 0; j < NLD; ++j) bo[LD_R + j] = *reinterpret_cast<const f16x8*>(bl_next + b_off(LD_N + j) + C::PLANE_BYTES);
                     }
 #pragma unroll
                     for (int n = 0; n < NW; ++n)
-                        acc[m][n] = __builtin_amdgcn_mfma_f32_16x16x32_f16(a_hi, bh[n], acc[m][n], 0, 0, 0);
+                        acc[m][n] = __builtin_amdgcn_mfma_f32_16x16x32_f16(a_hi, bh[RB + n], acc[m][n], 0, 0, 0);
 #pragma unroll
                     for (int n = 0; n < NW; ++n)
-                        acc[m][n] = __builtin_amdgcn_mfma_f32_16x16x32_f16(a_lo, bh[n], acc[m][n], 0, 0, 0);
+                        acc[m][n] = __builtin_amdgcn_mfma_f32_16x16x32_f16(a_lo, bh[RB + n], acc[m][n], 0, 0, 0);
                 } else {
 #pragma unroll
-                    for (int n = 0; n < NW; ++n) acc[m][n][0] += (float)a_hi[0] * (float)bh[n][0] + (float)a_lo[1] * (float)bo[n][1];
+                    for (int n = 0; n < NW; ++n) acc[m][n][0] += (float)a_hi[0] * (float)bh[RB + n][0] + (float)a_lo[1] * (float)bo[RB + n][1];
                     if (last) {
 #pragma unroll
-                        for (int n = 0; n < NW; ++n) bo[n] = *reinterpret_cast<const f16x8*>(bl_next + b_off(n) + C::PLANE_BYTES);
+                        for (int j = 0; j < NLD; ++j) bo[LD_R + j] = *reinterpret_cast<const f16x8*>(bl_next + b_off(LD_N + j) + C::PLANE_BYTES);
                     }
                 }
                 if (last) {
 #pragma unroll
-                    for (int n = 0; n < NW; ++n) bh[n] = *reinterpret_cast<const f16x8*>(bl_next + b_off(n));
+                    for (int j = 0; j < NLD; ++j) bh[LD_R + j] = *reinterpret_cast<const f16x8*>(bl_next + b_off(LD_N + j));
                     if (!A0_EARLY) {
                         ah[0] = *reinterpret_cast<const f16x8*>(al_next);
                         ao[0] = *reinterpret_cast<const f16x8*>(al_next + MW * 1024);
@@ -698,14 +787,28 @@
                     if constexpr (!(ABL & 16) && !(ABL & 8)) {
                         if (A0_EARLY) __builtin_amdgcn_sched_group_barrier(0x100, 2, 1);
                         __builtin_amdgcn_sched_group_barrier(0x008, NW, 1);
-                        __builtin_amdgcn_sched_group_barrier(0x100, NW, 1);
+                        __builtin_amdgcn_sched_group_barrier(0x100, NLD, 1);
                         __builtin_amdgcn_sched_group_barrier(0x008, 2 * NW, 1);
-                        __builtin_amdgcn_sched_group_barrier(0x100, A0_EARLY ? NW : NW + 2, 1);
+                        __builtin_amdgcn_sched_group_barrier(0x100, A0_EARLY ? NLD : NLD + 2, 1);
                     }
                     __builtin_amdgcn_sched_barrier(0);
                 }
             }
             P = Pn;
+        };
+        if constexpr (C::KYRUN) {
+            static_assert(!C::KYRUN || C::K == 5, "a run is unrolled over its K = 5 steps");
+#pragma unroll 1
+            for (int s = 0; s < n_stages; s += C::K) {
+                do_step(s, std::integral_constant<int, 0>{});
+                do_step(s + 1, std::integral_constant<int, 1>{});
+                do_step(s + 2, std::integral_constant<int, 2>{});
+                do_step(s + 3, std::integral_constant<int, 3>{});
+                do_step(s + 4, std::integral_constant<int, 4>{});
+            }
+        } else {
+#pragma unroll 1
+            for (int s = 0; s < n_stages; ++s) do_step(s, std::integral_constant<int, -1>{});
         }
         if constexpr ((ABL & 2048) != 0) {
             probe_loop += __builtin_readcyclecounter() - probe_t1;
@@ -729,8 +832,8 @@
         if constexpr (EPI != EPI_HEAD) {
 #pragma unroll
             for (int n = 0; n < NW; ++n) {
-                const int oy = y0 + (wave * C::RPW + n / NFC) * D;
-                const int ox = x0 + (n % NFC) * 16 + l15;
+                const int oy = y0 + ((wave / C::WCOLS) * C::RPW + n / NFC) * D;
+                const int ox = x0 + (wave % C::WCOLS) * 16 + (n % NFC) * 16 + l15;
                 okv[n] = oy < a.wy1 && ox < a.wx1;
                 if constexpr ((ABL & 1) != 0 || (ABL & 64) != 0) okv[n] = okv[n] && (a.slope == 12345.f);
                 const int cy = oy < a.Hout ? oy : a.Hout - 1, cx = ox < a.Wout ? ox : a.Wout - 1;
@@ -756,8 +859,8 @@
 #pragma unroll
             for (int q = 0; q < NP; ++q) {
                 const int fr = odd ? (2 * q + 1) / NFC : (2 * q) / NFC, fc = odd ? (2 * q + 1) % NFC : (2 * q) % NFC;
-                const int oy = y0 + (wave * C::RPW + fr) * D;
-                const int ox = x0 + fc * 16 + l15;
+                const int oy = y0 + ((wave / C::WCOLS) * C::RPW + fr) * D;
+                const int ox = x0 + (wave % C::WCOLS) * 16 + fc * 16 + l15;
                 bool ok = oy < a.wy1 && ox < a.wx1;
                 if constexpr ((ABL & 1) != 0 || (ABL & 64) != 0) ok = ok && (a.slope == 12345.f);
                 const int cy = oy < a.Hout ? oy : a.Hout - 1, cx = ox < a.Wout ? ox : a.Wout - 1;
@@ -970,9 +1073,9 @@
         const int wave = __builtin_amdgcn_readfirstlane(tid_e >> 6);
 #pragma unroll
         for (int n = 0; n < NW; ++n) {
-            const int trow = wave * C::RPW + n / NFC;
+            const int trow = (wave / C::WCOLS) * C::RPW + n / NFC;
             const int oy = y0 + trow * D;
-            const int ox = x0 + (n % NFC) * 16 + l15;
+            const int ox = x0 + (wave % C::WCOLS) * 16 + (n % NFC) * 16 + l15;
             float h = hsum[n];
             h += __shfl_xor(h, 16, 64);
             h += __shfl_xor(h, 32, 64);
diff --git a/topaz_amd/csrc/conv_split_inst_h.hip b/topaz_amd/csrc/conv_split_inst_h.hip
--- /dev/null
+++ b/topaz_amd/csrc/conv_split_inst_h.hip
@@ -0,0 +1,5 @@
+#include "conv_split_registry.h"
+TPZ_SPLIT_KYRUN(5, 1, 32,  8, 32, 2, 4, 2, ::tpz::EPI_PLAIN)
+TPZ_SPLIT_KYRUN(5, 1, 32,  8, 32, 2, 4, 2, ::tpz::EPI_PLAIN_F32)
+TPZ_SPLIT_KYRUN(5, 2, 32, 16, 32, 2, 8, 4, ::tpz::EPI_PLAIN)
+TPZ_SPLIT_KYRUN(5, 4, 32, 16, 32, 2, 8, 4, ::tpz::EPI_PLAIN)
diff --git a/topaz_amd/csrc/conv_split_registry.h b/topaz_amd/csrc/conv_split_registry.h
--- a/topaz_amd/csrc/conv_split_registry.h
+++ b/topaz_amd/csrc/conv_split_registry.h
@@ -11,7 +11,12 @@
     int cont, Q;
     SplitSlot (*slot)(int step, int kb);
     SplitSlot (*cont_slot)(int q);
-    int stages(int cells) const { return cont ? ((Q / CC) * cells + 3) / 4 : (cells + CC - 1) / CC * NSTEP; }
+    int kyrun;
+    SplitRunSlot (*kyrun_slot)(int cells, int step, int kb);
+    int (*kyrun_stages)(int cells);
+    int stages(int cells) const {
+        return kyrun ? kyrun_stages(cells) : cont ? ((Q / CC) * cells + 3) / 4 : (cells + CC - 1) / CC * NSTEP;
+    }
     hipError_t (*launch)(const SplitArgs&, dim3 grid, hipStream_t);
     hipError_t (*launch_multi)(const SplitArgs* const* list, int n, hipStream_t);
     void (*make_plan)(const SplitPlanKey&, std::vector<SplitStep>&);
@@ -19,7 +24,7 @@
 };
 
 void register_split(const SplitKernelInfo& info);
-const SplitKernelInfo* find_split(int K, int D, int MT, int epi, int KX = 0, int sps = 0);
+const SplitKernelInfo* find_split(int K, int D, int MT, int epi, int KX = 0, int sps = 0, bool kyrun = false);
 
 template <class C, int EPI>
 hipError_t launch_split_cfg(const SplitArgs& a, dim3 grid, hipStream_t s) {
@@ -68,6 +73,24 @@
     return hipGetLastError();
 }
 
+template <class C, int EPI>
+hipError_t launch_split_kyrun_cfg(const SplitArgs& a, dim3 grid, hipStream_t s) {
+    static bool attr_set = false;
+    if (!attr_set) {
+        hipError_t e = hipFuncSetAttribute(reinterpret_cast<const void*>(&conv_split_kernel<C, EPI, 0, 0>),
+                                           hipFuncAttributeMaxDynamicSharedMemorySize, C::LDS_BYTES);
+        if (e == hipSuccess)
+            e = hipFuncSetAttribute(reinterpret_cast<const void*>(&conv_split_kernel<C, EPI, 0, 4>),
+                                    hipFuncAttributeMaxDynamicSharedMemorySize, C::LDS_BYTES);
+        if (e != hipSuccess) return e;
+        attr_set = true;
+    }
+    if (a.in2 || a.KZ > 1 || a.Din > 1 || a.nphase > 0 || a.subpix_cout > 0) return hipErrorInvalidValue;
+    if (a.n_tiles > 0) hipLaunchKernelGGL((conv_split_kernel<C, EPI, 0, 4>), grid, dim3(C::THREADS), C::LDS_BYTES, s, a);
+    else hipLaunchKernelGGL((conv_split_kernel<C, EPI, 0, 0>), grid, dim3(C::THREADS), C::LDS_BYTES, s, a);
+    return hipGetLastError();
+}
+
 inline int split_mode_of(const SplitArgs& a) {
     if (!a.in2 && a.KZ <= 1 && a.Din <= 1) return 0;
     if (a.KZ <= 1 && a.Din <= 1) return 1;
@@ -114,6 +137,34 @@
     return hipGetLastError();
 }
 
+template <class C, int EPI>
+hipError_t launch_split_multi_kyrun_cfg(const SplitArgs* const* list, int n, hipStream_t s) {
+    static bool attr_set = false;
+    if (!attr_set) {
+        const hipError_t e = hipFuncSetAttribute(reinterpret_cast<const void*>(&conv_split_multi_kernel<C, EPI, 0>),
+                                                 hipFuncAttributeMaxDynamicSharedMemorySize, C::LDS_BYTES);
+        if (e != hipSuccess) return e;
+        attr_set = true;
+    }
+    if (n < 1 || n > SPLIT_MULTI_MAX) return hipErrorInvalidValue;
+    SplitMulti m;
+    m.n = (unsigned)n;
+    unsigned total = 0;
+    for (int i = 0; i < n; ++i) {
+        if (split_mode_of(*list[i]) != 0 || list[i]->n_tiles < 1 || list[i]->nphase > 0 || list[i]->subpix_cout > 0) return hipErrorInvalidValue;
+        m.first[i] = total;
+        m.a[i] = *list[i];
+        total = (total + (unsigned)list[i]->n_tiles + 7u) & ~7u;
+    }
+    for (int i = n; i <= SPLIT_MULTI_MAX; ++i) m.first[i] = total;
+    hipLaunchKernelGGL((conv_split_multi_kernel<C, EPI, 0>), dim3(total, 1, 1), dim3(C::THREADS), C::LDS_BYTES, s, m);
+    return hipGetLastError();
+}
+
+template <class C>
+SplitRunSlot split_kyrun_slot_of(int cells, int step, int kb) { return C::kyrun_slot(cells, step, kb); }
+template <class C>
+int split_kyrun_stages_of(int cells) { return C::kyrun_stages(cells); }
 template <class C>
 SplitSlot split_slot_of(int step, int kb) { return C::slot(step, kb); }
 template <class C>
@@ -130,11 +181,22 @@
         i.slot = &split_slot_of<C>;
         i.cont = C::CONT ? 1 : 0; i.Q = C::Q;
         i.cont_slot = &split_cont_slot_of<C>;
-        i.launch = &launch_split_cfg<C, EPI>;
+        i.kyrun = C::KYRUN ? 1 : 0;
+        i.kyrun_slot = &split_kyrun_slot_of<C>;
+        i.kyrun_stages = &split_kyrun_stages_of<C>;
         i.launch_multi = nullptr;
-        if constexpr (C::WAVES == 4 && EPI != EPI_HEAD) i.launch_multi = &launch_split_multi_cfg<C, EPI>;
+        if constexpr (C::KYRUN) {
+            i.launch = &launch_split_kyrun_cfg<C, EPI>;
+            if constexpr (C::WAVES == 4) i.launch_multi = &launch_split_multi_kyrun_cfg<C, EPI>;
+        } else {
+            i.launch = &launch_split_cfg<C, EPI>;
+            if constexpr (C::WAVES == 4 && EPI != EPI_HEAD) i.launch_multi = &launch_split_multi_cfg<C, EPI>;
+        }
         i.make_plan = &split_make_plan<C>;
-        if (C::SPS == 1)
+        if (C::KYRUN)
+            snprintf(i.name, sizeof i.name, "conv_split_kernel<K=%dx%d,D=%d,MT=%d,TH=%d,TW=%d,CC=%d,W=%d,S=%d,KYRUN,EPI=%d>", i.K,
+                     i.KX, i.D, i.MT, i.TH, i.TW, i.CC, i.WAVES, i.SPS, i.epi);
+        else if (C::SPS == 1)
             snprintf(i.name, sizeof i.name, "conv_split_kernel<K=%dx%d,D=%d,MT=%d,TH=%d,TW=%d,CC=%d,W=%d,EPI=%d>", i.K, i.KX,
                      i.D, i.MT, i.TH, i.TW, i.CC, i.WAVES, i.epi);
         else
@@ -150,6 +212,8 @@
     static ::tpz::SplitRegistrar<::tpz::SplitCfg<K, D, MT, TH, TW, CC, 8, K, S>, EPI> TPZ_CAT(tpz_sreg_, __COUNTER__);
 #define TPZ_SPLIT4_S(K, D, MT, TH, TW, CC, S, EPI) \
     static ::tpz::SplitRegistrar<::tpz::SplitCfg<K, D, MT, TH, TW, CC, 4, K, S>, EPI> TPZ_CAT(tpz_sreg_, __COUNTER__);
+#define TPZ_SPLIT_KYRUN(K, D, MT, TH, TW, CC, W, S, EPI) \
+    static ::tpz::SplitRegistrar<::tpz::SplitCfg<K, D, MT, TH, TW, CC, W, K, S, true>, EPI> TPZ_CAT(tpz_sreg_, __COUNTER__);
 #define TPZ_SPLIT4_COL(K, D, MT, TH, TW, CC, EPI) \
     static ::tpz::SplitRegistrar<::tpz::SplitCfg<K, D, MT, TH, TW, CC, 4, 1>, EPI> TPZ_CAT(tpz_sreg_, __COUNTER__);
 #define TPZ_SPLIT4(K, D, MT, TH, TW, CC, EPI) \
diff --git a/topaz_amd/csrc/rt_core.hip b/topaz_amd/csrc/rt_core.hip
--- a/topaz_amd/csrc/rt_core.hip
+++ b/topaz_amd/csrc/rt_core.hip
@@ -18,11 +18,14 @@
     return nullptr;
 }
 void register_split(const SplitKernelInfo& info) { split_registry().push_back(info); }
-const SplitKernelInfo* find_split(int K, int D, int MT, int epi, int KX, int sps) {
+const SplitKernelInfo* find_split(int K, int D, int MT, int epi, int KX, int sps, bool kyrun) {
     if (KX <= 0) KX = K;
+    if (kyrun && sps <= 0)
+        for (const auto& k : split_registry())
+            if (k.kyrun && k.K == K && k.KX == KX && k.D == D && k.MT == MT && k.epi == epi) return &k;
     const SplitKernelInfo* best = nullptr;
     for (const auto& k : split_registry())
-        if (k.K == K && k.KX == KX && k.D == D && k.MT == MT && k.epi == epi && (sps <= 0 || k.SPS == sps) &&
+        if (!k.kyrun && k.K == K && k.KX == KX && k.D == D && k.MT == MT && k.epi == epi && (sps <= 0 || k.SPS == sps) &&
             (!best || k.SPS > best->SPS)) best = &k;
     return best;
 }
@@ -59,6 +62,7 @@
     d.no_pool3d = flag("TPZ_NO_POOL3D");
     d.no_fold = flag("TPZ_NO_FOLD");
     d.no_widen = flag("TPZ_NO_WIDEN");
+    d.no_kyrun = flag("TPZ_NO_KYRUN");
     if (flag("TPZ_NO_BATCH")) d.batch = 0;
     else if (const char* e = getenv("TPZ_BATCH")) {
         const int n = atoi(e);
@@ -328,7 +332,8 @@
     add(d.no_phase, "no_phase"); add(d.exact_fp32, "exact_fp32"); add(d.no_issuer, "no_issuer"); add(d.no_lanes, "no_lanes");
     add(d.no_roi, "no_roi"); add(d.no_persist, "no_persist"); add(d.trace_host, "trace_host"); add(d.no_range, "no_range");
     add(d.no_raster, "no_raster"); add(d.no_srcmajor, "no_srcmajor"); add(d.no_valu_last, "no_valu_last"); add(d.no_rw, "no_rw");
-    add(d.no_pool3d, "no_pool3d"); add(d.no_fold, "no_fold"); add(d.no_widen, "no_widen"); add(d.batch >= 0, "batch");
+    add(d.no_pool3d, "no_pool3d"); add(d.no_fold, "no_fold"); add(d.no_widen, "no_widen"); add(d.no_kyrun, "no_kyrun");
+    add(d.batch >= 0, "batch");
     add(d.lanes != 0, "lanes");
     if (buf && buf_len > 0) snprintf(buf, (size_t)buf_len, "%s", s.c_str());
     return n;
diff --git a/topaz_amd/csrc/rt_forward.hip b/topaz_amd/csrc/rt_forward.hip
--- a/topaz_amd/csrc/rt_forward.hip
+++ b/topaz_amd/csrc/rt_forward.hip
@@ -211,7 +211,7 @@
     memset(&L, 0, sizeof L);
     L.op = TPZ_OP_CONV; L.dims = 2; L.cin = cin; L.cout = cout; L.k = k; L.dil = dil; L.pad = pad; L.slope = slope;
     L.res = d_res ? 1 : -1; L.res_crop = res_crop; L.head = h_head_w ? 1 : 0; L.src2 = -1;
-    rt.ks = pick_split(k, dil, cout, epi);
+    rt.ks = pick_split(k, dil, cout, epi, 0, !ctx->dbg.no_kyrun);
     if (!rt.ks) return fail(ctx, "tpz_conv_split_2d: no 2xf16 kernel for k=%d dil=%d cout=%d epi=%d", k, dil, cout, epi);
     const int span = dil * (k - 1);
     const int Ho = H + 2 * pad - span, Wo = W + 2 * pad - span;
diff --git a/topaz_amd/csrc/rt_internal.h b/topaz_amd/csrc/rt_internal.h
--- a/topaz_amd/csrc/rt_internal.h
+++ b/topaz_amd/csrc/rt_internal.h
@@ -13,6 +13,7 @@
 #include "../../include/topaz_hip.h"
 #include "conv_registry.h"
 #include "conv_split_registry.h"
+#include "split_pack.h"
 #include "conv_rw.h"
 #include "kernels_misc.h"
 
@@ -35,6 +36,7 @@
     bool no_pool3d = false;
     bool no_fold = false;
     bool no_widen = false;
+    bool no_kyrun = false;
     int batch = -1;
     int lanes = 0;
 };
@@ -342,10 +344,7 @@
 int upload(tpz_ctx* ctx, tpz_model* m, const float* h, size_t n, float** out);
 int upload_chan(tpz_ctx* ctx, tpz_model* m, const float* h, size_t n, float** out);
 int upload_halfs(tpz_ctx* ctx, tpz_model* m, const std::vector<uint16_t>& h, void** out);
-void pack_weights_split(const SplitKernelInfo& ki, const float* w, int cout, int cin, int n_cog, int n_chunks,
-                        std::vector<uint16_t>& out, std::vector<float>& wscale_inv, const float* wp = nullptr, int cin_b = 0,
-                        const float* mul = nullptr);
-const SplitKernelInfo* pick_split(int k, int dil, int cout, int epi, int kx = 0);
+const SplitKernelInfo* pick_split(int k, int dil, int cout, int epi, int kx = 0, bool kyrun = false);
 int model_load(tpz_ctx* ctx, const tpz_layer* layers, int n_layers, const float* h_blob, size_t n_floats,
                const std::vector<int>& preset_chan, tpz_model** out);
 unsigned split_forms(const tpz_model* m, int i);
diff --git a/topaz_amd/csrc/rt_load.hip b/topaz_amd/csrc/rt_load.hip
--- a/topaz_amd/csrc/rt_load.hip
+++ b/topaz_amd/csrc/rt_load.hip
@@ -190,90 +190,8 @@
 
 }
 
-void pack_weights_split(const SplitKernelInfo& ki, const float* w, int cout, int cin, int n_cog, int n_chunks,
-                        std::vector<uint16_t>& out, std::vector<float>& wscale_inv, const float* wp, int cin_b, const float* mul) {
-    const int K = ki.K, KX = ki.KX, MW = ki.MT / 16;
-    const size_t taps = (size_t)K * KX;
-    std::vector<float> scale(cout, 1.f);
-    wscale_inv.assign(cout, 1.f);
-    for (int co = 0; co < cout; ++co) {
-        float mx = 0.f;
-        const float f = mul ? std::fabs(mul[co]) : 1.f;
-        for (size_t i = 0; i < (size_t)cin * taps; ++i) mx = std::max(mx, f * std::fabs(w[(size_t)co * cin * taps + i]));
-        for (int i = 0; wp && i < cin_b; ++i) mx = std::max(mx, f * std::fabs(wp[(size_t)co * cin_b + i]));
-        int e = 0;
-        if (mx > 0.f && std::isfinite(mx)) e = std::min(60, std::max(-60, (int)std::floor(std::log2(16384.0 / mx))));
-        scale[co] = std::ldexp(1.f, e);
-        wscale_inv[co] = std::ldexp(1.f, -e);
-    }
-    const size_t step_halfs = (size_t)ki.W_STEP_BYTES / 2;
-    const int cells = (int)split_cells(cin);
-    const int n_stages_a = ki.stages(cells);
-    const int n_stages = n_stages_a + (wp ? (int)split_cells(cin_b) / ki.CC : 0);
-    const int n_full = cells / ki.CC, n_rem = cells - n_full * ki.CC, taps_n = ki.cont ? ki.Q / ki.CC : 0;
-    out.assign((size_t)n_cog * n_stages * step_halfs, 0);
-    auto put = [&](uint16_t* blk, int m, int kb, int i, int j, float v) {
-        const _Float16 hi = (_Float16)v;
-        const _Float16 lo = (_Float16)(v - (float)hi);
-        uint16_t hb, lb;
-        memcpy(&hb, &hi, 2);
-        memcpy(&lb, &lo, 2);
-        const size_t lane = (size_t)kb * 16 + i;
-        blk[((size_t)(0 * MW + m) * 64 + lane) * 8 + j] = hb;
-        blk[((size_t)(1 * MW + m) * 64 + lane) * 8 + j] = lb;
-    };
-    for (int cog = 0; cog < n_cog; ++cog)
-        for (int st = 0; st < n_stages; ++st) {
-            uint16_t* blk = out.data() + ((size_t)cog * n_stages + st) * step_halfs;
-            if (st >= n_stages_a) {
-                const int cb = st - n_stages_a;
-                for (int kb = 0; kb < ki.CC; ++kb)
-                    for (int m = 0; m < MW; ++m)
-                        for (int i = 0; i < 16; ++i) {
-                            const int co = cog * ki.MT + m * 16 + i;
-                            if (co >= cout) continue;
-                            for (int j = 0; j < 8; ++j) {
-                                const int ci = (cb * ki.CC + kb) * 8 + j;
-                                if (ci < cin_b) put(blk, m, kb, i, j, wp[(size_t)co * cin_b + ci] * scale[co] * (mul ? mul[co] : 1.f));
-                            }
-                        }
-                continue;
-            }
-            for (int kb = 0; kb < 4; ++kb) {
-                int ch;
-                SplitSlot sl;
-                if (ki.cont) {
-                    const int G = 4 * st + kb;
-                    ch = G / ki.Q;
-                    if (ch < n_full) {
-                        sl = ki.cont_slot(G % ki.Q);
-                    } else {
-                        const int q2 = G - n_full * ki.Q;
-                        if (n_rem == 0 || q2 >= taps_n * n_rem) continue;
-                        ch = n_full;
-                        sl = ki.cont_slot((q2 / n_rem) * ki.CC + (q2 % n_rem));
-                    }
-                } else {
-                    ch = st / ki.NSTEP;
-                    sl = ki.slot(st % ki.NSTEP, kb);
-                    if (sl.ky < 0) continue;
-                }
-                for (int m = 0; m < MW; ++m)
-                    for (int i = 0; i < 16; ++i) {
-                        const int co = cog * ki.MT + m * 16 + i;
-                        if (co >= cout) continue;
-                        for (int j = 0; j < 8; ++j) {
-                            const int ci = (ch * ki.CC + sl.c) * 8 + j;
-                            if (ci >= cin) continue;
-                            put(blk, m, kb, i, j, w[((size_t)co * cin + ci) * taps + (size_t)sl.ky * KX + sl.kx] * scale[co] * (mul ? mul[co] : 1.f));
-                        }
-                    }
-            }
-        }
-}
-
-const SplitKernelInfo* pick_split(int k, int dil, int cout, int epi, int kx) {
-    return pick_by_padded_width(cout, [&](int mt) { return find_split(k, dil, mt, epi, kx); });
+const SplitKernelInfo* pick_split(int k, int dil, int cout, int epi, int kx, bool kyrun) {
+    return pick_by_padded_width(cout, [&](int mt) { return find_split(k, dil, mt, epi, kx, 0, kyrun); });
 }
 
 int upload_halfs(tpz_ctx* ctx, tpz_model* m, const std::vector<uint16_t>& h, void** out) {
@@ -444,8 +362,9 @@
             reads[i] = (rt.sphase.valid || rt.ks) ? 1 : 0;
             continue;
         }
-        rt.ks = pick_split(L.k, L.dil, L.cout, rt.ki->epi);
-        if (!rt.ks && rt.ki->epi == EPI_PLAIN) rt.ks = pick_split(L.k, L.dil, L.cout, EPI_PLAIN_F32);
+        const bool kyrun = L.dims == 2 && !m->dbg.no_kyrun;
+        rt.ks = pick_split(L.k, L.dil, L.cout, rt.ki->epi, 0, kyrun);
+        if (!rt.ks && rt.ki->epi == EPI_PLAIN) rt.ks = pick_split(L.k, L.dil, L.cout, EPI_PLAIN_F32, 0, kyrun);
         reads[i] = rt.ks ? 1 : 0;
     }
     std::function<bool(int)> slot_read_split = [&](int slot) {
@@ -514,8 +433,9 @@
         }
         if (rt.ks) {
             if (!L.head && !wanted && rt.ks->epi == EPI_PLAIN && L.src2 < 0) {
-                const SplitKernelInfo* f = find_split(L.k, L.dil, rt.ks->MT, EPI_PLAIN_F32);
-                if (!f) f = pick_split(L.k, L.dil, L.cout, EPI_PLAIN_F32);
+                const bool kyrun = L.dims == 2 && !m->dbg.no_kyrun;
+                const SplitKernelInfo* f = find_split(L.k, L.dil, rt.ks->MT, EPI_PLAIN_F32, 0, 0, kyrun);
+                if (!f) f = pick_split(L.k, L.dil, L.cout, EPI_PLAIN_F32, 0, kyrun);
                 if (f) rt.ks = f;
             }
             if (i == nl - 1 && !L.head && rt.ks->epi != EPI_PLAIN_F32) rt.ks = nullptr;
@@ -552,7 +472,8 @@
         }
         if (readers != 1 || pool != i + 1) continue;
         const SplitKernelInfo* pk = find_split(base->K, base->D, base->MT, EPI_POOL, base->KX);
-        if (pk && pk->CC == base->CC && pk->NSTEP == base->NSTEP && pk->cont == base->cont && pk->W_STEP_BYTES == base->W_STEP_BYTES) rt.ks_pool = pk;
+        if (pk && pk->CC == base->CC && pk->NSTEP == base->NSTEP && pk->cont == base->cont && pk->kyrun == base->kyrun &&
+            pk->W_STEP_BYTES == base->W_STEP_BYTES) rt.ks_pool = pk;
     }
     const bool no_fold = m->dbg.no_fold;
     for (int i = 0; i < nl && !no_fold; ++i) {
diff --git a/topaz_amd/csrc/split_pack.h b/topaz_amd/csrc/split_pack.h
--- /dev/null
+++ b/topaz_amd/csrc/split_pack.h
@@ -0,0 +1,99 @@
+#pragma once
+#include <algorithm>
+#include <cmath>
+#include <cstring>
+#include <vector>
+
+#include "conv_split_registry.h"
+
+namespace tpz::rt {
+
+inline void pack_weights_split(const SplitKernelInfo& ki, const float* w, int cout, int cin, int n_cog, int n_chunks,
+                               std::vector<uint16_t>& out, std::vector<float>& wscale_inv, const float* wp = nullptr, int cin_b = 0,
+                               const float* mul = nullptr) {
+    const int K = ki.K, KX = ki.KX, MW = ki.MT / 16;
+    const size_t taps = (size_t)K * KX;
+    std::vector<float> scale(cout, 1.f);
+    wscale_inv.assign(cout, 1.f);
+    for (int co = 0; co < cout; ++co) {
+        float mx = 0.f;
+        const float f = mul ? std::fabs(mul[co]) : 1.f;
+        for (size_t i = 0; i < (size_t)cin * taps; ++i) mx = std::max(mx, f * std::fabs(w[(size_t)co * cin * taps + i]));
+        for (int i = 0; wp && i < cin_b; ++i) mx = std::max(mx, f * std::fabs(wp[(size_t)co * cin_b + i]));
+        int e = 0;
+        if (mx > 0.f && std::isfinite(mx)) e = std::min(60, std::max(-60, (int)std::floor(std::log2(16384.0 / mx))));
+        scale[co] = std::ldexp(1.f, e);
+        wscale_inv[co] = std::ldexp(1.f, -e);
+    }
+    const size_t step_halfs = (size_t)ki.W_STEP_BYTES / 2;
+    const int cells = (int)split_cells(cin);
+    const int n_stages_a = ki.stages(cells);
+    const int n_stages = n_stages_a + (wp ? (int)split_cells(cin_b) / ki.CC : 0);
+    const int n_full = cells / ki.CC, n_rem = cells - n_full * ki.CC, taps_n = ki.cont ? ki.Q / ki.CC : 0;
+    out.assign((size_t)n_cog * n_stages * step_halfs, 0);
+    auto put = [&](uint16_t* blk, int m, int kb, int i, int j, float v) {
+        const _Float16 hi = (_Float16)v;
+        const _Float16 lo = (_Float16)(v - (float)hi);
+        uint16_t hb, lb;
+        memcpy(&hb, &hi, 2);
+        memcpy(&lb, &lo, 2);
+        const size_t lane = (size_t)kb * 16 + i;
+        blk[((size_t)(0 * MW + m) * 64 + lane) * 8 + j] = hb;
+        blk[((size_t)(1 * MW + m) * 64 + lane) * 8 + j] = lb;
+    };
+    for (int cog = 0; cog < n_cog; ++cog)
+        for (int st = 0; st < n_stages; ++st) {
+            uint16_t* blk = out.data() + ((size_t)cog * n_stages + st) * step_halfs;
+            if (st >= n_stages_a) {
+                const int cb = st - n_stages_a;
+                for (int kb = 0; kb < ki.CC; ++kb)
+                    for (int m = 0; m < MW; ++m)
+                        for (int i = 0; i < 16; ++i) {
+                            const int co = cog * ki.MT + m * 16 + i;
+                            if (co >= cout) continue;
+                            for (int j = 0; j < 8; ++j) {
+                                const int ci = (cb * ki.CC + kb) * 8 + j;
+                                if (ci < cin_b) put(blk, m, kb, i, j, wp[(size_t)co * cin_b + ci] * scale[co] * (mul ? mul[co] : 1.f));
+                            }
+                        }
+                continue;
+            }
+            for (int kb = 0; kb < 4; ++kb) {
+                int ch;
+                SplitSlot sl;
+                if (ki.kyrun) {
+                    const SplitRunSlot rs = ki.kyrun_slot(cells, st, kb);
+                    if (rs.sl.ky < 0) continue;
+                    ch = rs.chunk;
+                    sl = rs.sl;
+                } else if (ki.cont) {
+                    const int G = 4 * st + kb;
+                    ch = G / ki.Q;
+                    if (ch < n_full) {
+                        sl = ki.cont_slot(G % ki.Q);
+                    } else {
+                        const int q2 = G - n_full * ki.Q;
+                        if (n_rem == 0 || q2 >= taps_n * n_rem) continue;
+                        ch = n_full;
+                        sl = ki.cont_slot((q2 / n_rem) * ki.CC + (q2 % n_rem));
+                    }
+                } else {
+                    ch = st / ki.NSTEP;
+                    sl = ki.slot(st % ki.NSTEP, kb);
+                    if (sl.ky < 0) continue;
+                }
+                for (int m = 0; m < MW; ++m)
+                    for (int i = 0; i < 16; ++i) {
+                        const int co = cog * ki.MT + m * 16 + i;
+                        if (co >= cout) continue;
+                        for (int j = 0; j < 8; ++j) {
+                            const int ci = (ch * ki.CC + sl.c) * 8 + j;
+                            if (ci >= cin) continue;
+                            put(blk, m, kb, i, j, w[((size_t)co * cin + ci) * taps + (size_t)sl.ky * KX + sl.kx] * scale[co] * (mul ? mul[co] : 1.f));
+                        }
+                    }
+            }
+        }
+}
+
+}
```

After: 8.854, median of 2. About the same (-0.1%).
